# DecodeGenetics/BamQC

Hardware: AMD Instinct MI355X
Metric: BAM records/sec (and GB/s vs HBM roofline), 150 bp PE, 1/2/4/8 MI355X (higher is better)
Workload: dtype u8/u32/u64 integer

## Files before the change

### bamqc_amd/csrc/bqc_api.cpp

```cpp
#include <hip/hip_runtime.h>

#include <algorithm>
#include <climits>
#include <cmath>
#include <cstdarg>
#include <cstdio>
#include <cstdlib>
#include <cstring>
#include <string>
#include <chrono>
#include <condition_variable>
#include <mutex>
#include <thread>
#include <vector>

#include "bqc_ctx.h"
#include "../host/parallel.h"

extern "C" {
void bqc_launch_cov_final(const StateLayout&, uint64_t*, const uint32_t* carry, const uint32_t* parity, const uint8_t* started, const uint8_t* sel, uint32_t count_start, hipStream_t);
void bqc_launch_ref_nibbles(const uint8_t* dna5, uint64_t len, uint32_t* out, uint64_t n_dwords, hipStream_t);
uint32_t bqc_long_slots_cap(uint32_t max_read_len, uint32_t n_cu);
hipError_t bqc_long_init();
hipError_t bqc_short_init();
}

static thread_local char g_create_err[512];

int bqc_fail(bqc_ctx* c, int code, const char* fmt, ...)
{
    char buf[512];
    va_list ap;
    va_start(ap, fmt);
    vsnprintf(buf, sizeof buf, fmt, ap);
    va_end(ap);
    if (c) c->err = buf;
    else snprintf(g_create_err, sizeof g_create_err, "%s", buf);
    return code;
}
#define fail bqc_fail

extern "C" int bqc_abi_version(void) { return BQC_ABI_VERSION; }
extern "C" const char* bqc_last_error(const bqc_ctx* c) { return c ? c->err.c_str() : g_create_err; }

static int upload_ref_tables(bqc_ctx* c)
{
    HIPCHK(c, hipMemcpyAsync(c->d_ref_ptrs, c->d_ref.data(), sizeof(uint8_t*) * c->d_ref.size(), hipMemcpyHostToDevice, c->stream));
    HIPCHK(c, hipMemcpyAsync(c->d_ref_len, c->ref_len.data(), sizeof(uint64_t) * c->ref_len.size(), hipMemcpyHostToDevice, c->stream));
    HIPCHK(c, hipMemcpyAsync(c->d_refn_ptrs, c->d_refn.data(), sizeof(uint32_t*) * c->d_refn.size(), hipMemcpyHostToDevice, c->stream));
    HIPCHK(c, hipStreamSynchronize(c->stream));
    return 0;
}

static int reset_stream_records(bqc_ctx* c)
{
    ErrRec e{};
    e.first_key = BQC_ERRKEY_NONE;
    const int32_t cur[2] = {-1, -1};
    HIPCHK(c, hipMemcpyAsync(c->d_err0, &e, sizeof e, hipMemcpyHostToDevice, c->stream));
    HIPCHK(c, hipMemcpyAsync(c->d_cursor, cur, 8, hipMemcpyHostToDevice, c->stream));
    HIPCHK(c, hipStreamSynchronize(c->stream));
    return 0;
}

extern "C" int bqc_create(const bqc_options* opt, bqc_ctx** out)
{
    if (!opt || !out) return fail(nullptr, BQC_ERR_ARG, "bqc_create: null argument");
    if (opt->struct_size != sizeof(bqc_options)) return fail(nullptr, BQC_ERR_ARG, "bqc_create: struct_size mismatch");
    if (opt->n_lanes == 0 || opt->n_lanes > 256) return fail(nullptr, BQC_ERR_ARG, "bqc_create: n_lanes must be 1..256");
    if (opt->isize < 0) return fail(nullptr, BQC_ERR_ARG, "bqc_create: negative insert size");
    if (opt->max_read_len == 0 || opt->hist_cap == 0) return fail(nullptr, BQC_ERR_ARG, "bqc_create: zero capacity");
    if (opt->n_refs && !opt->main_chrom) return fail(nullptr, BQC_ERR_ARG, "bqc_create: main_chrom missing");
    int ndev = 0;
    if (hipGetDeviceCount(&ndev) != hipSuccess || ndev <= 0)
        return fail(nullptr, BQC_ERR_DEVICE, "bqc_create: no HIP device available (this library has no CPU fallback)");
    if (opt->device < 0 || opt->device >= ndev) return fail(nullptr, BQC_ERR_DEVICE, "bqc_create: device %d out of range", opt->device);
    bqc_ctx* c = new bqc_ctx();
    c->opt = *opt;
    c->device = opt->device;
    uint32_t nr = opt->n_refs ? opt->n_refs : 1;
    c->main_chrom.assign(nr, 0);
    if (opt->n_refs) memcpy(c->main_chrom.data(), opt->main_chrom, opt->n_refs);
    if (opt->fasta_index) c->fasta_index.assign(opt->fasta_index, opt->fasta_index + opt->n_refs);
    c->opt.main_chrom = c->main_chrom.data();
    c->opt.fasta_index = c->fasta_index.empty() ? nullptr : c->fasta_index.data();
    c->sl = make_state_layout(opt->n_lanes, opt->max_read_len, opt->hist_cap, (uint32_t)opt->isize + 1);
    c->cov.assign(opt->n_lanes, LaneCov());
    c->shard.tail = opt->shard_tail != 0;
    c->shard.pending.assign(opt->n_lanes, c->shard.tail ? 1 : 0);
    c->shard.has_prev.assign(opt->n_lanes, 0);
    c->shard.prev_rid.assign(opt->n_lanes, 0);
    c->shard.prev_bp.assign(opt->n_lanes, 0);
    c->d_ref.assign(nr, nullptr);
    c->d_refn.assign(nr, nullptr);
    c->ref_len.assign(nr, 0);
    const char* v = getenv("BQC_NO_FAST");
    c->no_fast = v && v[0] == '1';
#define CCHK(call)                                                                                            \
    do {                                                                                                      \
        hipError_t e_ = (call);                                                                               \
        if (e_ != hipSuccess) {                                                                               \
            fail(nullptr, BQC_ERR_DEVICE, "bqc_create: %s failed: %s", #call, hipGetErrorString(e_));         \
            bqc_destroy(c);                                                                                   \
            return BQC_ERR_DEVICE;                                                                            \
        }                                                                                                     \
    } while (0)
    const bool ctiming = getenv("BQC_TIMING") && getenv("BQC_TIMING")[0] == '1';
    const auto ct0 = std::chrono::steady_clock::now();
    double cts[10] = {0, 0, 0, 0, 0, 0, 0, 0, 0, 0};
    auto cstamp = [&](int k) { cts[k] = std::chrono::duration<double>(std::chrono::steady_clock::now() - ct0).count() * 1e3; };
    CCHK(hipSetDevice(c->device));
    hipDeviceProp_t prop;
    CCHK(hipGetDeviceProperties(&prop, c->device));
    c->n_cu = prop.multiProcessorCount > 0 ? (uint32_t)prop.multiProcessorCount : 256;
    cstamp(0);
    c->stream = bqc_pool_stream(c->device, 0);
    if (!c->stream) { fail(nullptr, BQC_ERR_DEVICE, "bqc_create: hipStreamCreate failed"); bqc_destroy(c); return BQC_ERR_DEVICE; }
    cstamp(1);
    CCHK(hipMalloc(&c->d_state, c->sl.words * 8));
    CCHK(hipMalloc(&c->d_err0, sizeof(ErrRec)));
    CCHK(hipMalloc(&c->d_cursor, 8));
    cstamp(6);
    if (!c->fasta_index.empty()) {
        CCHK(hipMalloc(&c->d_fasta_index, 4 * c->fasta_index.size()));
        CCHK(hipMemcpy(c->d_fasta_index, c->fasta_index.data(), 4 * c->fasta_index.size(), hipMemcpyHostToDevice));
    }
    cstamp(7);
    c->kl_slots_cap = bqc_long_slots_cap(opt->max_read_len, c->n_cu);
    c->t8_slots_cap = std::max(std::max(1024u, 4u * c->n_cu), c->kl_slots_cap);
    CCHK(hipMalloc(&c->d_t8rows, (size_t)c->t8_slots_cap * BQC_T8_SPW * 65536));
    CCHK(hipMalloc(&c->d_t8used, (size_t)c->t8_slots_cap * BQC_T8_USED * 4));
    cstamp(8);
    CCHK(hipMalloc(&c->d_kl_cyc, (size_t)c->kl_slots_cap * 2 * 6 * 1024 * 4));
    CCHK(hipMalloc(&c->d_kl_cyc_used, (size_t)c->kl_slots_cap * 4));
    CCHK(hipMalloc(&c->d_carry, (size_t)opt->n_lanes * 2 * 2000 * 4));
    CCHK(hipMalloc(&c->d_parity, ((size_t)opt->n_lanes + 1) * 4));
    CCHK(hipMalloc(&c->d_started, opt->n_lanes));
    CCHK(hipMalloc(&c->d_ref_ptrs, sizeof(uint8_t*) * nr));
    CCHK(hipMalloc(&c->d_ref_len, sizeof(uint64_t) * nr));
    CCHK(hipMalloc(&c->d_refn_ptrs, sizeof(uint32_t*) * nr));
    CCHK(hipMalloc(&c->d_main, nr));
    cstamp(9);
    CCHK(hipMemcpy(c->d_main, c->main_chrom.data(), nr, hipMemcpyHostToDevice));
    cstamp(2);
    CCHK(hipMemsetAsync(c->d_state, 0, c->sl.words * 8, c->stream));
    if (reset_stream_records(c)) { snprintf(g_create_err, sizeof g_create_err, "%s", c->err.c_str()); bqc_destroy(c); return BQC_ERR_DEVICE; }
    CCHK(hipMemsetAsync(c->d_carry, 0, (size_t)opt->n_lanes * 2 * 2000 * 4, c->stream));
    CCHK(hipMemsetAsync(c->d_parity, 0, ((size_t)opt->n_lanes + 1) * 4, c->stream));
    CCHK(hipMemsetAsync(c->d_started, 0, opt->n_lanes, c->stream));
    CCHK(hipStreamSynchronize(c->stream));
    if (upload_ref_tables(c)) { snprintf(g_create_err, sizeof g_create_err, "%s", c->err.c_str()); bqc_destroy(c); return BQC_ERR_DEVICE; }
    cstamp(3);
    if (opt->sketch.n_k && opt->sketch.n_q) {
        std::string e;
        c->sketch = sketch_create(opt->sketch, opt->n_lanes, c->stream, e);
        if (!c->sketch) { fail(nullptr, BQC_ERR_ARG, "bqc_create: sketch: %s", e.c_str()); bqc_destroy(c); return BQC_ERR_ARG; }
    }
    cstamp(4);
    for (int i = 0; i < 16; ++i) {
        hipEvent_t e;
        CCHK(hipEventCreate(&e));
        c->ev.push_back(e);
    }
    cstamp(5);
    if (ctiming) fprintf(stderr, "[timing] bqc_create: kernel attributes (code object load) at %.1f ms, compute stream %.1f, allocations %.1f (first three %.1f, FASTA index copied %.1f, 8-mer rows %.1f, the rest %.1f, then a copy), memsets + tables %.1f, sketch %.1f, events %.1f\n", cts[0], cts[1], cts[2], cts[6], cts[7], cts[8], cts[9], cts[3], cts[4], cts[5]);
    *out = c;
    return 0;
}

namespace {
struct StreamPool {
    std::mutex m;
    std::condition_variable cv;
    static const int kAhead = 4;
    hipStream_t made[kAhead] = {nullptr, nullptr, nullptr, nullptr};
    bool taken[kAhead] = {false, false, false, false};
    int device = -1;
    int n_made = 0;
    bool making = false;
};
StreamPool g_streams;
}
hipStream_t bqc_pool_stream(int device, int rank)
{
    {
        std::unique_lock<std::mutex> lk(g_streams.m);
        if (g_streams.device == device && rank >= 0 && rank < StreamPool::kAhead) {
            g_streams.cv.wait(lk, [&] { return g_streams.n_made > rank || !g_streams.making; });
            if (g_streams.n_made > rank && !g_streams.taken[rank]) { g_streams.taken[rank] = true; return g_streams.made[rank]; }
        }
    }
    hipStream_t s = nullptr;
    if (hipStreamCreateWithFlags(&s, hipStreamNonBlocking) != hipSuccess) { (void)hipGetLastError(); return nullptr; }
    return s;
}

extern "C" int bqc_warmup(int32_t device)
{
    {
        std::lock_guard<std::mutex> lk(g_streams.m);
        if (g_streams.device != -1) return g_streams.device == device ? 0 : BQC_ERR_ARG;
        g_streams.device = device;
        g_streams.making = true;
    }
    auto done = [](int rc) { { std::lock_guard<std::mutex> lk(g_streams.m); g_streams.making = false; } g_streams.cv.notify_all(); return rc; };
    if (hipSetDevice(device) != hipSuccess || hipFree(nullptr) != hipSuccess) return done(BQC_ERR_DEVICE);
    for (int k = 0; k < StreamPool::kAhead; ++k) {
        hipStream_t s = nullptr;
        if (hipStreamCreateWithFlags(&s, hipStreamNonBlocking) != hipSuccess) { (void)hipGetLastError(); return done(BQC_ERR_DEVICE); }
        { std::lock_guard<std::mutex> lk(g_streams.m); g_streams.made[k] = s; g_streams.n_made = k + 1; }
        g_streams.cv.notify_all();
    }
    return done(0);
}

extern "C" int bqc_set_fasta_index(bqc_ctx* c, const int32_t* idx)
{
    if (!c || !idx) return BQC_ERR_ARG;
    if (c->upload_counter) return bqc_fail(c, BQC_ERR_STATE, "bqc_set_fasta_index after the first batch");
    HIPCHK(c, hipSetDevice(c->device));
    const size_t n = c->opt.n_refs ? c->opt.n_refs : 1;
    c->fasta_index.assign(n, -1);
    for (uint32_t r = 0; r < c->opt.n_refs; ++r) c->fasta_index[r] = idx[r];
    c->opt.fasta_index = c->fasta_index.data();
    if (!c->d_fasta_index) HIPCHK(c, hipMalloc(&c->d_fasta_index, 4 * n));
    HIPCHK(c, hipMemcpy(c->d_fasta_index, c->fasta_index.data(), 4 * n, hipMemcpyHostToDevice));
    return 0;
}

extern "C" void bqc_destroy(bqc_ctx* c)
{
    if (!c) return;
    (void)hipSetDevice(c->device);
    if (c->copy_stream) (void)hipStreamSynchronize(c->copy_stream);
    if (c->stream) (void)hipStreamSynchronize(c->stream);
    bqc_pipeline_destroy(c);
    bqc_anchor_destroy(c);
    auto in_arena = [&](const void* p) { return c->ref_arena && (const uint8_t*)p >= c->ref_arena && (const uint8_t*)p < c->ref_arena + c->ref_arena_cap; };
    for (auto p : c->d_ref) if (p && !in_arena(p)) (void)hipFree(p);
    for (auto p : c->d_refn) if (p && !in_arena(p)) (void)hipFree(p);
    if (c->ref_arena) (void)hipFree(c->ref_arena);

    (void)hipFree(c->d_refn_ptrs);
    if (c->sketch) sketch_destroy(c->sketch);
    (void)hipFree(c->d_state); (void)hipFree(c->d_err0); (void)hipFree(c->d_cursor); (void)hipFree(c->d_fasta_index); (void)hipFree(c->d_t8rows); (void)hipFree(c->d_t8used); (void)hipFree(c->d_kl_cyc); (void)hipFree(c->d_kl_cyc_used); (void)hipFree(c->d_carry); (void)hipFree(c->d_parity);
    (void)hipFree(c->d_started); (void)hipFree(c->d_ref_ptrs); (void)hipFree(c->d_ref_len); (void)hipFree(c->d_main);
    for (auto e : c->ev) (void)hipEventDestroy(e);
    if (c->stream) (void)hipStreamDestroy(c->stream);
    if (c->copy_stream) (void)hipStreamDestroy(c->copy_stream);
    delete c;
}

extern "C" int bqc_reserve_references(bqc_ctx* c, uint64_t total_bases, uint32_t n_contigs)
{
    if (!c) return BQC_ERR_ARG;
    if (c->ref_arena) return 0;
    HIPCHK(c, hipSetDevice(c->device));
    const size_t cap = (size_t)total_bases + (size_t)total_bases / 2 + (size_t)n_contigs * (8 * BQC_FAST_NH + 1024) + 4096;
    if (hipMalloc((void**)&c->ref_arena, cap) != hipSuccess) { (void)hipGetLastError(); c->ref_arena = nullptr; return 0; }
    c->ref_arena_cap = cap;
    c->ref_arena_used = 0;
    return 0;
}

extern "C" int bqc_set_reference(bqc_ctx* c, int32_t rid, const uint8_t* dna5, uint64_t len)
{
    if (!c || rid < 0 || (uint32_t)rid >= c->opt.n_refs || (!dna5 && len)) return fail(c, BQC_ERR_ARG, "bqc_set_reference: bad argument");
    HIPCHK(c, hipSetDevice(c->device));
    auto in_arena = [&](const void* p) { return c->ref_arena && (const uint8_t*)p >= c->ref_arena && (const uint8_t*)p < c->ref_arena + c->ref_arena_cap; };
    if (c->d_ref[rid]) { if (!in_arena(c->d_ref[rid])) HIPCHK(c, hipFree(c->d_ref[rid])); c->d_ref[rid] = nullptr; }
    if (c->d_refn[rid]) { if (!in_arena(c->d_refn[rid])) HIPCHK(c, hipFree(c->d_refn[rid])); c->d_refn[rid] = nullptr; }
    const uint64_t nd8 = (len + 7) / 8;
    const size_t b1 = ((len ? len : 1) + 255) & ~(size_t)255, b2 = ((nd8 + 2 * BQC_FAST_NH) * 4 + 255) & ~(size_t)255;
    uint8_t* p = nullptr;
    uint32_t* pn = nullptr;
    if (c->ref_arena && c->ref_arena_used + b1 + b2 <= c->ref_arena_cap) {
        p = c->ref_arena + c->ref_arena_used;
        pn = (uint32_t*)(p + b1);
        c->ref_arena_used += b1 + b2;
    } else {
        HIPCHK(c, hipMalloc(&p, len ? len : 1));
        HIPCHK(c, hipMalloc(&pn, (nd8 + 2 * BQC_FAST_NH) * 4));
    }
    HIPCHK(c, hipMemcpy(p, dna5, len, hipMemcpyHostToDevice));
    bqc_launch_ref_nibbles(p, len, pn, nd8, c->stream);
    HIPCHK(c, hipStreamSynchronize(c->stream));
    c->d_ref[rid] = p;
    c->d_refn[rid] = pn;
    c->ref_len[rid] = len;
    return upload_ref_tables(c);
}

static int sync_and_check(bqc_ctx* c)
{
    HIPCHK(c, hipSetDevice(c->device));
    if (c->poisoned) return bqc_fail(c, BQC_ERR_STATE, "context is in an error state: %s", c->err.c_str());
    int rc = bqc_drain(c);
    if (rc) return rc;
    ErrRec e;
    HIPCHK(c, hipMemcpyAsync(&e, c->d_err0, sizeof e, hipMemcpyDeviceToHost, c->stream));
    HIPCHK(c, hipStreamSynchronize(c->stream));
    rc = bqc_report_errors(c, e);
    if (rc) { c->poisoned = true; c->poison_code = rc; }
    return rc;
}

extern "C" int bqc_sync(bqc_ctx* c)
{
    if (!c) return BQC_ERR_ARG;
    return sync_and_check(c);
}

extern "C" int bqc_reset(bqc_ctx* c)
{
    if (!c) return BQC_ERR_ARG;
    HIPCHK(c, hipSetDevice(c->device));
    (void)bqc_drain(c);
    bqc_state_ready(c);
    HIPCHK(c, hipMemsetAsync(c->d_state, 0, c->sl.words * 8, c->stream));
    if (reset_stream_records(c)) return BQC_ERR_DEVICE;
    HIPCHK(c, hipMemsetAsync(c->d_carry, 0, (size_t)c->opt.n_lanes * 2 * 2000 * 4, c->stream));
    HIPCHK(c, hipMemsetAsync(c->d_parity, 0, ((size_t)c->opt.n_lanes + 1) * 4, c->stream));
    HIPCHK(c, hipMemsetAsync(c->d_started, 0, c->opt.n_lanes, c->stream));
    if (c->sketch) sketch_reset(c->sketch, c->stream);
    HIPCHK(c, hipStreamSynchronize(c->stream));
    c->cov.assign(c->opt.n_lanes, LaneCov());
    if (c->anchor.d_state) HIPCHK(c, bqc_anchor_fresh_state(c));
    c->anchor.mode = 0;
    c->state_seq = 0;
    c->flushed = false;
    c->poisoned = false;
    c->poison_code = 0;
    return 0;
}

extern "C" int bqc_set_timing(bqc_ctx* c, int enable)
{
    if (!c) return BQC_ERR_ARG;
    c->timing = enable != 0;
    return 0;
}

extern "C" int bqc_last_timing(bqc_ctx* c, uint32_t* n, const char* const** names, const float** ms)
{
    if (!c || !n || !names || !ms) return BQC_ERR_ARG;
    HIPCHK(c, hipStreamSynchronize(c->stream));
    c->tms.assign(c->n_timed, 0.f);
    for (int i = 0; i < c->n_timed; ++i) (void)hipEventElapsedTime(&c->tms[i], c->ev[i], c->ev[i + 1]);
    *n = (uint32_t)c->n_timed;
    *names = c->tnames.data();
    *ms = c->tms.data();
    return 0;
}

extern "C" int bqc_flush(bqc_ctx* c)
{
    if (!c) return BQC_ERR_ARG;
    if (c->poisoned) return fail(c, BQC_ERR_STATE, "context is in an error state: %s", c->err.c_str());
    if (c->flushed) return 0;
    HIPCHK(c, hipSetDevice(c->device));
    int rc = sync_and_check(c);
    if (rc) return rc;
    bqc_state_ready(c);
    bqc_launch_cov_final(c->sl, c->d_state, c->d_carry, c->d_parity, c->d_started, nullptr, 1, c->stream);
    HIPCHK(c, hipGetLastError());
    HIPCHK(c, hipStreamSynchronize(c->stream));
    c->flushed = true;
    return 0;
}

extern "C" uint64_t bqc_state_words(const bqc_ctx* c) { return c ? c->sl.words + (c->sketch ? sketch_state_words(c->sketch) : 0) : 0; }

extern "C" int bqc_state_export(bqc_ctx* c, void* dst)
{
    if (!c || !dst) return BQC_ERR_ARG;
    int rc = bqc_flush(c);
    if (rc) return rc;
    bqc_state_ready(c);
    HIPCHK(c, hipMemcpyAsync(dst, c->d_state, c->sl.words * 8, hipMemcpyDeviceToDevice, c->stream));
    if (c->sketch) sketch_state_export(c->sketch, (uint64_t*)dst + c->sl.words, c->stream);
    HIPCHK(c, hipStreamSynchronize(c->stream));
    return 0;
}
extern "C" int bqc_state_import(bqc_ctx* c, const void* src)
{
    if (!c || !src) return BQC_ERR_ARG;
    HIPCHK(c, hipSetDevice(c->device));
    (void)bqc_drain(c);
    bqc_state_ready(c);
    HIPCHK(c, hipMemcpyAsync(c->d_state, src, c->sl.words * 8, hipMemcpyDeviceToDevice, c->stream));
    if (c->sketch) sketch_state_import(c->sketch, (const uint64_t*)src + c->sl.words, c->stream);
    HIPCHK(c, hipStreamSynchronize(c->stream));
    c->flushed = true;
    return 0;
}
extern "C" int bqc_state_export_host(bqc_ctx* c, uint64_t* dst)
{
    if (!c || !dst) return BQC_ERR_ARG;
    int rc = bqc_flush(c);
    if (rc) return rc;
    bqc_state_ready(c);
    HIPCHK(c, hipStreamSynchronize(c->stream));
    HIPCHK(c, hipMemcpy(dst, c->d_state, c->sl.words * 8, hipMemcpyDeviceToHost));
    if (c->sketch) {
        uint64_t* tmp = nullptr;
        const uint64_t w = sketch_state_words(c->sketch);
        HIPCHK(c, hipMalloc(&tmp, w * 8));
        sketch_state_export(c->sketch, tmp, c->stream);
        HIPCHK(c, hipStreamSynchronize(c->stream));
        HIPCHK(c, hipMemcpy(dst + c->sl.words, tmp, w * 8, hipMemcpyDeviceToHost));
        HIPCHK(c, hipFree(tmp));
    }
    return 0;
}
extern "C" int bqc_state_import_host(bqc_ctx* c, const uint64_t* src)
{
    if (!c || !src) return BQC_ERR_ARG;
    HIPCHK(c, hipSetDevice(c->device));
    (void)bqc_drain(c);
    bqc_state_ready(c);
    HIPCHK(c, hipStreamSynchronize(c->stream));
    HIPCHK(c, hipMemcpy(c->d_state, src, c->sl.words * 8, hipMemcpyHostToDevice));
    if (c->sketch) {
        uint64_t* tmp = nullptr;
        const uint64_t w = sketch_state_words(c->sketch);
        HIPCHK(c, hipMalloc(&tmp, w * 8));
        HIPCHK(c, hipMemcpy(tmp, src + c->sl.words, w * 8, hipMemcpyHostToDevice));
        sketch_state_import(c->sketch, tmp, c->stream);
        HIPCHK(c, hipStreamSynchronize(c->stream));
        HIPCHK(c, hipFree(tmp));
    }
    c->flushed = true;
    return 0;
}

static uint32_t last_nonzero_len(const uint64_t* p, uint32_t n)
{
    while (n > 0 && p[n - 1] == 0) --n;
    return n;
}

extern "C" int bqc_finalize(bqc_ctx* c, const bqc_counts** out)
{
    if (!c || !out) return BQC_ERR_ARG;
    int rc = bqc_flush(c);
    if (rc) return rc;
    const StateLayout& sl = c->sl;
    c->h_state.resize(sl.words);
    HIPCHK(c, hipMemcpy(c->h_state.data(), c->d_state, sl.words * 8, hipMemcpyDeviceToHost));
    c->arrays.clear();
    c->lanes.assign(sl.n_lanes, bqc_lane_counts{});
    c->sk_out.assign(sl.n_lanes, {});
    auto keep = [&](std::vector<uint64_t>&& v) -> const uint64_t* {
        c->arrays.push_back(std::move(v));
        return c->arrays.back().data();
    };
    auto u32copy = [&](const uint64_t* p, uint32_t n) {
        std::vector<uint64_t> v(n ? n : 1);
        for (uint32_t i = 0; i < n; ++i) v[i] = p[i] & 0xFFFFFFFFull;
        return v;
    };
    c->arrays.reserve(sl.n_lanes * 64);
    for (uint32_t l = 0; l < sl.n_lanes; ++l) {
        const uint64_t* S = c->h_state.data() + sl.lane_base(l);
        bqc_lane_counts& L = c->lanes[l];
        for (int i = 0; i < BQC_N_SCALARS; ++i)
            L.scalars[i] = i == BQC_S_TOTALBPS ? S[sl.o_scalars + i] : (S[sl.o_scalars + i] & 0xFFFFFFFFull);
        for (int i = 0; i <= BQC_COVSIZE; ++i) L.poscov[i] = S[sl.o_poscov + i];
        if (S[sl.o_covstart] == 0) L.poscov[0] += 2 * BQC_VSIZE;
        for (int i = 0; i <= BQC_COVSIZE; ++i) L.poscov[i] &= 0xFFFFFFFFull;
        L.eightmer = S + sl.o_eightmer;
        L.triplet = S + sl.o_triplet;
        for (uint32_t m = 0; m < 2; ++m) {
            const uint64_t* Mq = S + sl.o_mate[m];
            bqc_mate_counts& mc = L.mate[m];
            const uint32_t n_rl = last_nonzero_len(Mq + sl.m_readlen, sl.lcap + 1);
            const uint32_t ncyc = n_rl ? n_rl - 1 : 0;
            mc.n_cycles = ncyc;
            for (int j = 0; j < 5; ++j) mc.dnacount[j] = Mq + sl.m_dnacount + (uint64_t)j * sl.lcap;
            mc.qualcount = Mq + sl.m_qualcount;
            mc.qualcount_readnr = Mq[sl.m_readnr] & 0xFFFFFFFFull;
            {
                std::vector<uint64_t> v(ncyc ? ncyc : 1, 0);
                uint64_t run = 0;
                for (uint32_t j = sl.lcap + 1; j-- > 0;) {
                    if (j < ncyc) v[j] = run & 0xFFFFFFFFull;
                    run += Mq[sl.m_sc5hist + j];
                }
                mc.sc5 = keep(std::move(v));
            }
            {
                std::vector<uint64_t> v(ncyc ? ncyc : 1, 0);
                uint64_t run = 0;
                for (uint32_t j = 0; j < ncyc; ++j) { run += Mq[sl.m_sc3diff + j]; v[j] = run & 0xFFFFFFFFull; }
                mc.sc3 = keep(std::move(v));
            }
            mc.n_Ncount = n_rl; mc.Ncount = keep(u32copy(Mq + sl.m_ncount, n_rl));
            mc.n_GCcount = n_rl; mc.GCcount = Mq + sl.m_gccount;
            mc.n_averageQual = last_nonzero_len(Mq + sl.m_avgceil, 256);
            mc.averageQual = keep(u32copy(Mq + sl.m_avgqual, mc.n_averageQual));
            mc.n_insertSize = sl.icap; mc.insertSize = keep(u32copy(Mq + sl.m_insert, sl.icap));
            mc.n_mapQ = last_nonzero_len(Mq + sl.m_mapq, 256); mc.mapQ = keep(u32copy(Mq + sl.m_mapq, mc.n_mapQ));
            mc.n_readLength = n_rl; mc.readLength = keep(u32copy(Mq + sl.m_readlen, n_rl));
            mc.n_mismatch = last_nonzero_len(Mq + sl.m_mismatch, sl.hcap); mc.mismatch = keep(u32copy(Mq + sl.m_mismatch, mc.n_mismatch));
            mc.n_delhist = last_nonzero_len(Mq + sl.m_delhist, sl.hcap); mc.delhist = keep(u32copy(Mq + sl.m_delhist, mc.n_delhist));
            mc.n_inshist = last_nonzero_len(Mq + sl.m_inshist, sl.hcap); mc.inshist = keep(u32copy(Mq + sl.m_inshist, mc.n_inshist));
        }
        if (c->sketch) {
            std::string e;
            if (!sketch_finalize(c->sketch, l, c->sk_out[l], c->stream, e)) return fail(c, BQC_ERR_DEVICE, "sketch finalize: %s", e.c_str());
            L.n_sketch = (uint32_t)c->sk_out[l].size();
            L.sketch = c->sk_out[l].data();
        }
    }
    c->counts.n_lanes = sl.n_lanes;
    c->counts.lanes = c->lanes.data();
    *out = &c->counts;
    return 0;
}
```

### bamqc_amd/csrc/bqc_ctx.h

```cpp
#pragma once
#include <hip/hip_runtime.h>

#include <atomic>
#include <cstdarg>
#include <cstdio>
#include <deque>
#include <mutex>
#include <string>
#include <vector>

#include "../../include/bamqc.h"
#include "device_types.h"
#include "prep.h"
#include "anchor.h"
#include "sketch.h"
#include "../host/raw_vector.h"

struct LaneCov {
    bool first = true;
    int32_t id = 0;
    uint32_t shift = 0;
    uint64_t win = 0;
    uint64_t batch_base = 0;
};

struct HostPass {
    uint32_t n = 0;
    uint64_t seq_bytes = 0, qual_bytes = 0, cigar_words = 0;
    uint32_t n_slow = 0, max_len_slow = 0;
    uint32_t t8_lane = 0;
    bool multi_lane = false;
    raw_vector<CovEntry> cov;
    raw_vector<uint32_t> order;
    std::vector<SuperWindow> sws;
    std::vector<Stretch> stretches;
    std::vector<CovTile> tiles;
    std::vector<uint8_t> lane_mask, started_after;
    std::vector<uint64_t> add_idx, add_val;
    uint32_t n_pending = 0;
    std::vector<std::vector<uint32_t>> lane_first;
    std::vector<uint64_t> lane_count;
};

struct BatchMem {
    void* dmem = nullptr;
    size_t dcap = 0;
    DevBatch d{};
    PrepArgs prep{};
    uint8_t* d_lane_mask = nullptr;
    uint8_t* d_started_after = nullptr;
    uint64_t* d_add_idx = nullptr;
    uint64_t* d_add_val = nullptr;
    uint32_t n_add = 0;
    uint32_t* d_rsum = nullptr;
    uint32_t* d_order_tmp = nullptr;
    ErrRec* d_err = nullptr;
    uint64_t algo_bytes = 0;
    uint32_t n_slow = 0, max_len_slow = 0, n_chunks_slow_ub = 0, t8_lane = 0;
    uint64_t lane_bits[4] = {0, 0, 0, 0};
    bool processed = false;
    size_t h2d_begin = 0, h2d_end = 0;
    size_t o_col[13] = {0};
    size_t col_bytes[13] = {0};
    size_t o_xr = 0, o_xv = 0, o_cov_in = 0, o_order = 0, o_sws = 0, o_stretch = 0, o_tiles = 0, o_mask = 0, o_started = 0, o_aidx = 0, o_aval = 0;
};

struct PendBatch {
    std::vector<uint8_t> lane;
    std::vector<int32_t> rid;
    std::vector<uint32_t> bp;
    void* dmem = nullptr;
    uint32_t extra_cap = 0;
    uint32_t n() const { return (uint32_t)lane.size(); }
};
struct ShardCtx {
    bool tail = false, resolved = false, exported = false;
    std::vector<uint8_t> pending;
    std::vector<uint8_t> has_prev;
    std::vector<int32_t> prev_rid;
    std::vector<uint32_t> prev_bp;
    std::deque<PendBatch> batches;
};

struct bqc_dbatch {
    BatchMem m;
    std::vector<LaneCov> cov_after;
    uint64_t seq = 0;
};

struct Slot {
    BatchMem m;
    char* hmem = nullptr;
    size_t hcap = 0;
    ErrRec* h_err = nullptr;
    hipEvent_t ev_h2d = nullptr, ev_done = nullptr;
    bool busy = false;
    bool in_place = false;
    uint64_t ticket = 0;
};

struct bqc_anchored {
    AnchorSummary* h_sum = nullptr;
    AnchorLane* h_lanes = nullptr;
    uint32_t* h_bound = nullptr;
    std::vector<uint32_t> rest;
    std::vector<int32_t> pend_rid;
    std::vector<uint32_t> pend_bp;
    std::vector<uint8_t> pend_lane;
    const CovEntry* d_cov = nullptr;
    uint32_t n = 0;
    bool completed = false;
    bool released = false;
    static const uint32_t kInline = 1u << 17;
};
struct AnchorEngine {
    std::atomic<int> mode{0};
    AnchorState* d_state = nullptr;
    AnchorSummary* d_sum = nullptr;
    uint32_t* d_bound = nullptr;
    void* d_scratch = nullptr;
    const uint32_t* d_plog_bp = nullptr; const int32_t* d_plog_rid = nullptr; const uint8_t* d_plog_lane = nullptr;
    size_t cap_n = 0;
    std::mutex m;
    std::vector<bqc_anchored*> free_list, all;
    bqc_anchored* outstanding = nullptr;
    std::string err;
};

struct bqc_ctx {
    bqc_options opt{};
    std::vector<uint8_t> main_chrom;
    std::vector<int32_t> fasta_index;
    StateLayout sl{};
    int device = 0;
    hipStream_t stream = nullptr;
    hipStream_t copy_stream = nullptr;
    uint32_t n_cu = 256;
    uint64_t* d_state = nullptr;
    ErrRec* d_err0 = nullptr;
    int32_t* d_cursor = nullptr;
    int32_t* d_fasta_index = nullptr;
    uint32_t* d_t8rows = nullptr;
    uint32_t* d_t8used = nullptr;
    uint32_t* d_kl_cyc = nullptr;
    uint32_t* d_kl_cyc_used = nullptr;
    uint32_t kl_slots_cap = 0;
    uint32_t t8_slots_used = 0, t8_slots_cap = 0;
    uint64_t t8_lanes[4] = {0, 0, 0, 0};
    std::vector<std::pair<void*, size_t>> pool;
    uint32_t* d_carry = nullptr;
    uint32_t* d_parity = nullptr;
    uint8_t* d_started = nullptr;
    std::vector<uint8_t*> d_ref;
    uint8_t* ref_arena = nullptr;
    size_t ref_arena_cap = 0, ref_arena_used = 0;
    std::vector<uint32_t*> d_refn;
    std::vector<uint64_t> ref_len;
    uint8_t** d_ref_ptrs = nullptr;
    uint32_t** d_refn_ptrs = nullptr;
    bool no_fast = false;
    uint64_t* d_ref_len = nullptr;
    uint8_t* d_main = nullptr;
    std::vector<LaneCov> cov;
    bool flushed = false;
    bool poisoned = false;
    int poison_code = 0;
    uint64_t upload_counter = 0;
    uint64_t state_seq = 0;
    HostPass hp;
    ShardCtx shard;
    static const int kSlots = 3;
    Slot slots[kSlots];
    uint64_t next_ticket = 1;
    uint64_t checked_ticket = 0;
    AnchorEngine anchor;
    SketchDevice* sketch = nullptr;
    bool timing = false;
    std::vector<hipEvent_t> ev;
    std::vector<const char*> tnames;
    std::vector<float> tms;
    int n_timed = 0;
    std::vector<uint64_t> h_state;
    std::vector<std::vector<uint64_t>> arrays;
    std::vector<bqc_lane_counts> lanes;
    std::vector<std::vector<bqc_sketch_counts>> sk_out;
    bqc_counts counts{};
    std::string err;
};

int bqc_fail(bqc_ctx* c, int code, const char* fmt, ...);
#define HIPCHK(c, call)                                                                                         \
    do {                                                                                                        \
        hipError_t e_ = (call);                                                                                 \
        if (e_ != hipSuccess) return bqc_fail(c, BQC_ERR_DEVICE, "%s failed: %s", #call, hipGetErrorString(e_)); \
    } while (0)

hipStream_t bqc_pool_stream(int device, int rank);
int bqc_copy_stream(bqc_ctx* c);
int bqc_report_errors(bqc_ctx* c, const ErrRec& e);
int bqc_drain(bqc_ctx* c);
void bqc_pipeline_destroy(bqc_ctx* c);
hipError_t bqc_anchor_fresh_state(bqc_ctx* c);
void bqc_anchor_destroy(bqc_ctx* c);
void bqc_state_ready(bqc_ctx* c);
```

### bamqc_amd/csrc/bqc_pipeline.cpp

```cpp
#include "bqc_ctx.h"

#include <algorithm>
#include <chrono>
#include <climits>
#include <cstdlib>
#include <cstring>

#include "../host/parallel.h"

extern "C" {
void bqc_launch_reads_chunks(const DevBatch&, const StateLayout&, uint64_t*, const DevRefs&, uint32_t*, uint32_t grid, uint32_t fast_table, hipStream_t);
void bqc_launch_nm_extra(const DevBatch&, const StateLayout&, uint64_t*, const DevRefs&, uint32_t*, hipStream_t);
void bqc_launch_long(const DevBatch&, const StateLayout&, uint64_t*, const DevRefs&, uint32_t*, uint32_t*, uint32_t max_len_ub, uint32_t max_read_len, uint32_t, uint32_t, uint32_t* t8rows, uint32_t* t8_used, uint32_t t8_lane, uint32_t* cyc_tiles, uint32_t* cyc_used, uint32_t slot_cap, hipStream_t);
uint32_t bqc_long_slots(uint32_t max_len_ub, uint32_t max_read_len, uint32_t n_chunks_ub, uint32_t n_cu);
void bqc_launch_cov(const DevBatch&, const StateLayout&, uint64_t*, uint32_t* carry, uint32_t* parity, const uint8_t* lane_mask, uint8_t* started,
                    const uint8_t* started_after, uint32_t n_lanes, hipStream_t);
void bqc_launch_add_words(uint64_t* state, const uint64_t* idx, const uint64_t* val, uint32_t n, hipStream_t);
void bqc_launch_or_bytes(uint8_t* dst, const uint8_t* src, uint32_t n, hipStream_t);
void bqc_launch_short(const DevBatch&, const StateLayout&, uint64_t*, const DevRefs&, uint32_t*, uint32_t grid, uint32_t* t8rows, uint32_t* t8_used, hipStream_t);
uint32_t bqc_short_parts();
void bqc_launch_t8_fold(const uint32_t* t8rows, const uint32_t* t8_used, uint32_t n_slots, const StateLayout&, uint64_t* state, uint32_t lane, hipStream_t);
void bqc_launch_err_merge(ErrRec* dst, const ErrRec* src, hipStream_t);
void bqc_launch_cov_final(const StateLayout&, uint64_t*, const uint32_t* carry, const uint32_t* parity, const uint8_t* started, const uint8_t* sel, uint32_t count_start, hipStream_t);
}

using clk = std::chrono::steady_clock;
static double secs_since(clk::time_point a) { return std::chrono::duration<double>(clk::now() - a).count(); }
static int timing_level()
{
    static const int lv = [] { const char* e = getenv("BQC_TIMING"); return e ? atoi(e) : 0; }();
    return lv;
}

int bqc_copy_stream(bqc_ctx* c)
{
    if (c->copy_stream) return 0;
    c->copy_stream = bqc_pool_stream(c->device, 3);
    return c->copy_stream ? 0 : bqc_fail(c, BQC_ERR_DEVICE, "hipStreamCreate failed");
}

void bqc_state_ready(bqc_ctx* c)
{
    if (!c->t8_slots_used) return;
    for (uint32_t l = 0; l < c->opt.n_lanes; ++l)
        if (c->t8_lanes[l >> 6] >> (l & 63u) & 1ull) bqc_launch_t8_fold(c->d_t8rows, c->d_t8used, c->t8_slots_used, c->sl, c->d_state, l, c->stream);
    c->t8_lanes[0] = c->t8_lanes[1] = c->t8_lanes[2] = c->t8_lanes[3] = 0;
    c->t8_slots_used = 0;
}

namespace {
struct CovPlanner {
    bqc_ctx* c;
    HostPass& H;
    uint32_t n, nl;
    std::vector<uint8_t> started_before;
    std::vector<uint32_t> last_rel;
    CovPlanner(bqc_ctx* c_, HostPass& H_, uint32_t n_) : c(c_), H(H_), n(n_), nl(c_->opt.n_lanes), started_before(nl), last_rel(nl, 0)
    {
        H.lane_mask.assign(nl, 0);
        H.lane_first.resize(nl);
        for (uint32_t l = 0; l < nl; ++l) {
            started_before[l] = !c->cov[l].first;
            c->cov[l].batch_base = c->cov[l].win;
            H.lane_first[l].clear();
        }
    }
    void step(uint32_t i, uint32_t lane, int32_t rid, uint32_t beginpos, uint64_t& rel, uint32_t& pos)
    {
        LaneCov& s = c->cov[lane];
        pos = an_step(s.first, s.id, s.shift, s.win, rid, beginpos);
        rel = s.win - s.batch_base;
        if (rel > 0xFFFFFFF0ull) return;
        std::vector<uint32_t>& first = H.lane_first[lane];
        if (first.size() <= rel) first.resize((size_t)rel + 1, i);
        last_rel[lane] = (uint32_t)rel;
    }
    void finish()
    {
        H.tiles.clear(); H.add_idx.clear(); H.add_val.clear();
        for (uint32_t l = 0; l < nl; ++l) {
            const std::vector<uint32_t>& first = H.lane_first[l];
            if (first.empty()) continue;
            H.lane_mask[l] = 1;
            const uint32_t W1 = last_rel[l];
            auto first_at = [&](uint64_t k) { return k < first.size() ? first[k] : n; };
            uint32_t last_tile = 0xFFFFFFFFu;
            uint64_t covered_final = 0;
            auto push_tile = [&](uint32_t w) {
                const uint32_t t = w / BQC_COV_TILE_WINDOWS;
                if (last_tile != 0xFFFFFFFFu && t <= last_tile) return;
                last_tile = t;
                const uint32_t wlo = t * BQC_COV_TILE_WINDOWS;
                CovTile ct{};
                ct.lane = l; ct.win_lo = wlo; ct.win_final = W1; ct.mixed = H.multi_lane ? 1u : 0u;
                ct.list_begin = first_at(wlo == 0 ? 0 : wlo - 1);
                ct.list_end = first_at((uint64_t)wlo + BQC_COV_TILE_WINDOWS);
                H.tiles.push_back(ct);
                const uint64_t hi = std::min<uint64_t>((uint64_t)wlo + BQC_COV_TILE_WINDOWS, W1);
                if (hi > wlo) covered_final += hi - wlo;
            };
            if (started_before[l]) { push_tile(0); push_tile(1); }
            for (uint64_t w = 0; w < first.size(); ++w) {
                const bool present = w + 1 == first.size() || first[w] != first[w + 1];
                if (present) { push_tile((uint32_t)w); push_tile((uint32_t)w + 1); }
            }
            if (W1 > covered_final) {
                H.add_idx.push_back(c->sl.lane_base(l) + c->sl.o_poscov + 0);
                H.add_val.push_back((uint64_t)(W1 - covered_final) * BQC_VSIZE);
            }
            c->cov[l].batch_base = c->cov[l].win;
        }
        H.started_after.resize(nl);
        for (uint32_t l = 0; l < nl; ++l) H.started_after[l] = !c->cov[l].first;
    }
};
}

static uint64_t plan_read_groups(HostPass& H, uint32_t n, uint32_t nl)
{
    uint32_t lanes_present = 0;
    H.t8_lane = 0;
    for (uint32_t l = 0; l < nl; ++l) {
        if (H.lane_count[l]) ++lanes_present;
        if (H.lane_count[l] > H.lane_count[H.t8_lane]) H.t8_lane = l;
    }
    uint64_t in_lanes = 0;
    for (uint32_t l = 0; l < nl; ++l) in_lanes += H.lane_count[l];
    const uint64_t n_bad = n - in_lanes;
    H.multi_lane = lanes_present > 1 || (n_bad > 0 && in_lanes > 0);
    H.stretches.clear(); H.sws.clear();
    auto add_stretch = [&](uint32_t lane, uint32_t begin, uint32_t count) {
        if (!count) return;
        Stretch S{lane, (uint32_t)H.sws.size(), 0, 0};
        for (uint32_t p = 0; p < count; p += BQC_SW_READS)
            H.sws.push_back(SuperWindow{lane, begin + p, std::min<uint32_t>(BQC_SW_READS, count - p), (uint32_t)H.stretches.size()});
        S.sw_end = (uint32_t)H.sws.size();
        H.stretches.push_back(S);
    };
    if (!H.multi_lane) {
        uint32_t lane = 0;
        for (uint32_t l = 0; l < nl; ++l) if (H.lane_count[l]) lane = l;
        add_stretch(lane, 0, n);
    } else {
        uint64_t at = n_bad;
        for (uint32_t l = 0; l < nl; ++l) { add_stretch(l, (uint32_t)(l == 0 ? 0 : at), (uint32_t)(H.lane_count[l] + (l == 0 ? n_bad : 0))); at += H.lane_count[l]; }
    }
    return n_bad;
}

static int host_pass(bqc_ctx* c, const bqc_batch* b, HostPass& H)
{
    const uint32_t n = b->n_reads, nl = c->opt.n_lanes;
    H.n = n;
    const unsigned nt_max = std::min(16u, bqc_host_threads());
    struct Part { uint64_t s1 = 0, s2 = 0, s3 = 0; uint32_t n_slow = 0, max_slow = 0; std::vector<uint64_t> lanes; };
    std::vector<Part> part(nt_max);
    const unsigned nt = parallel_ranges(n, nt_max, 1 << 17, [&](unsigned t, size_t lo, size_t hi) {
        Part& P = part[t];
        P.lanes.assign(nl, 0);
        uint64_t s1 = 0, s2 = 0, s3 = 0;
        uint32_t ns = 0, ms = 0;
        for (size_t i = lo; i < hi; ++i) {
            const uint32_t L = b->l_seq[i], lane = b->lane[i];
            s1 += (L + 1) / 2; s2 += L; s3 += b->n_cigar[i];
            if (lane < nl) P.lanes[lane]++;
            if (c->no_fast || L > BQC_FAST_MAXLEN) { ++ns; ms = std::max(ms, L); }
        }
        P.s1 = s1; P.s2 = s2; P.s3 = s3; P.n_slow = ns; P.max_slow = ms;
    });
    H.seq_bytes = H.qual_bytes = H.cigar_words = 0;
    H.n_slow = H.max_len_slow = 0;
    H.lane_count.assign(nl, 0);
    for (unsigned t = 0; t < nt; ++t) {
        H.seq_bytes += part[t].s1; H.qual_bytes += part[t].s2; H.cigar_words += part[t].s3;
        H.n_slow += part[t].n_slow; H.max_len_slow = std::max(H.max_len_slow, part[t].max_slow);
        for (uint32_t l = 0; l < nl; ++l) H.lane_count[l] += part[t].lanes[l];
    }
    const uint64_t n_bad = plan_read_groups(H, n, nl);
    if (H.multi_lane) {
        std::vector<uint64_t> w(nl);
        uint64_t at = n_bad, w_bad = 0;
        for (uint32_t l = 0; l < nl; ++l) { w[l] = at; at += H.lane_count[l]; }
        { const size_t cap = H.order.capacity(); H.order.resize(n); if (H.order.capacity() != cap) advise_huge(H.order); }
        for (uint32_t i = 0; i < n; ++i) {
            const uint32_t lane = b->lane[i];
            if (lane < nl) H.order[w[lane]++] = i; else H.order[w_bad++] = i;
        }
    } else H.order.clear();
    { const size_t cap = H.cov.capacity(); H.cov.resize(n); if (H.cov.capacity() != cap) advise_huge(H.cov); }
    CovPlanner plan(c, H, n);
    ShardCtx& sh = c->shard;
    const bool set_aside = sh.tail && !sh.resolved;
    PendBatch* pb = nullptr;
    H.n_pending = 0;
    const uint32_t n_refs = c->opt.n_refs;
    const uint8_t* main_chrom = c->main_chrom.data();
    if (!set_aside) {
        const uint16_t* const flags = b->flag;
        const uint8_t* const lanes = b->lane;
        const int32_t* const rids = b->rid;
        const int32_t* const poss = b->pos;
        CovEntry* const out = H.cov.data();
        LaneCov* const cov = c->cov.data();
        std::vector<uint32_t>* const lane_first = H.lane_first.data();
        uint32_t* const last_rel = plan.last_rel.data();
        LaneCov local = cov[0];
        const bool one = nl == 1;
        bool too_many = false;
        for (uint32_t i = 0; i < n; ++i) {
            const uint32_t flag = flags[i], lane = lanes[i];
            const int32_t rid = rids[i];
            if (!an_is_candidate(flag, rid, n_refs, main_chrom, lane, nl)) { out[i] = CovEntry{BQC_COV_NONE, 0}; continue; }
            LaneCov& st = one ? local : cov[lane];
            const uint32_t pos = an_step(st.first, st.id, st.shift, st.win, rid, (uint32_t)poss[i]);
            const uint64_t rel = st.win - st.batch_base;
            if (rel > 0xFFFFFFF0ull) { too_many = true; break; }
            std::vector<uint32_t>& first = lane_first[lane];
            if (first.size() <= rel) first.resize((size_t)rel + 1, i);
            last_rel[lane] = (uint32_t)rel;
            out[i] = CovEntry{(uint32_t)rel, pos};
        }
        if (one) cov[0] = local;
        if (too_many) return bqc_fail(c, BQC_ERR_ARG, "batch spans too many coverage windows (split the batch)");
    } else
    for (uint32_t i = 0; i < n; ++i) {
        const uint32_t flag = b->flag[i], lane = b->lane[i];
        const int32_t rid = b->rid[i];
        if (!an_is_candidate(flag, rid, n_refs, main_chrom, lane, nl)) { H.cov[i] = CovEntry{BQC_COV_NONE, 0}; continue; }
        const uint32_t beginpos = (uint32_t)b->pos[i];
        if (set_aside && sh.pending[lane]) {
            const uint32_t d = beginpos - sh.prev_bp[lane];
            const bool certain = sh.has_prev[lane] && (rid != sh.prev_rid[lane] || (d > 2u * BQC_VSIZE && d <= 0xFFFFFFFFu - 2u * BQC_VSIZE));
            sh.has_prev[lane] = 1; sh.prev_rid[lane] = rid; sh.prev_bp[lane] = beginpos;
            if (!certain) {
                if (!pb) { sh.batches.emplace_back(); pb = &sh.batches.back(); }
                H.cov[i] = CovEntry{BQC_COV_PENDING, pb->n()};
                pb->lane.push_back((uint8_t)lane); pb->rid.push_back(rid); pb->bp.push_back(beginpos);
                continue;
            }
            sh.pending[lane] = 0;
        }
        uint64_t rel;
        uint32_t pos;
        plan.step(i, lane, rid, beginpos, rel, pos);
        if (rel > 0xFFFFFFF0ull) return bqc_fail(c, BQC_ERR_ARG, "batch spans too many coverage windows (split the batch)");
        H.cov[i] = CovEntry{(uint32_t)rel, pos};
    }
    H.n_pending = pb ? pb->n() : 0;
    plan.finish();
    for (uint32_t e = 0; e < b->n_nm_extra; ++e)
        if (b->nm_extra_read[e] >= n) return bqc_fail(c, BQC_ERR_ARG, "nm_extra_read out of range");
    return 0;
}

extern "C" void bqc_anchor_rule(uint32_t n, const uint16_t* flag, const int32_t* rid, const int32_t* pos, const uint8_t* lane, uint32_t n_refs,
                                const uint8_t* main_chrom, uint32_t n_lanes, AnchorState* states, uint64_t* win, uint32_t* off)
{
    for (uint32_t i = 0; i < n; ++i) {
        win[i] = ~0ull; off[i] = 0;
        if (!an_is_candidate(flag[i], rid[i], n_refs, main_chrom, lane[i], n_lanes)) continue;
        AnchorState& s = states[lane[i]];
        bool first = s.first != 0;
        off[i] = an_step(first, s.id, s.shift, s.win, rid[i], (uint32_t)pos[i]);
        s.first = first;
        win[i] = s.win;
    }
}

static int first_from_table(bqc_ctx* c, const bqc_anchored* a, size_t off, size_t total, std::vector<uint32_t>& first)
{
    if (off + total > bqc_anchored::kInline + a->rest.size()) return bqc_fail(c, BQC_ERR_DEVICE, "internal error: the anchors' window table is shorter than the last window");
    first.assign(total, AN_NO_READ);
    uint32_t cur = AN_NO_READ;
    for (size_t k = total; k-- > 0;) {
        const size_t at = off + k;
        const uint32_t v = at < bqc_anchored::kInline ? a->h_bound[at] : a->rest[at - bqc_anchored::kInline];
        if (v != AN_NO_READ) cur = v;
        first[k] = cur;
    }
    if (first[total - 1] == AN_NO_READ) return bqc_fail(c, BQC_ERR_DEVICE, "internal error: the anchors' window table does not end at the last window");
    return 0;
}

static bool lane_anchored(const AnchorLane* AL, uint32_t l) { return AL[l].n_cand > AL[l].n_pending; }
static void load_state(LaneCov& lc, const AnchorState& s) { lc.first = s.first != 0; lc.id = s.id; lc.shift = s.shift; lc.win = s.win; }

static int host_pass_anchored(bqc_ctx* c, uint32_t n, const bqc_anchored* a, HostPass& H)
{
    const AnchorSummary& S = *a->h_sum;
    const AnchorLane* AL = a->h_lanes;
    const uint32_t nl = c->opt.n_lanes;
    H.n = n;
    H.seq_bytes = S.seq_bytes; H.qual_bytes = S.qual_bytes; H.cigar_words = S.cigar_words;
    H.n_slow = S.n_slow; H.max_len_slow = S.max_len_slow;
    H.lane_count.assign(nl, 0);
    for (uint32_t l = 0; l < nl; ++l) H.lane_count[l] = AL[l].n_reads;
    if (plan_read_groups(H, n, nl) != S.n_bad) return bqc_fail(c, BQC_ERR_DEVICE, "internal error: the anchors' read counts do not add up");
    H.order.clear();
    H.n_pending = 0;
    if (S.n_pending) {
        ShardCtx& sh = c->shard;
        sh.batches.emplace_back();
        PendBatch& pb = sh.batches.back();
        if (nl > 1) pb.lane = a->pend_lane; else pb.lane.assign(S.n_pending, 0);
        pb.rid = a->pend_rid;
        pb.bp = a->pend_bp;
        H.n_pending = S.n_pending;
    }
    if (c->shard.tail)
        for (uint32_t l = 0; l < nl; ++l) {
            const AnchorState& A = AL[l].after;
            c->shard.pending[l] = A.pending ? 1 : 0; c->shard.has_prev[l] = A.has_prev ? 1 : 0; c->shard.prev_rid[l] = A.prev_rid; c->shard.prev_bp[l] = A.prev_bp;
        }
    for (uint32_t l = 0; l < nl; ++l) load_state(c->cov[l], AL[l].before);
    CovPlanner plan(c, H, n);
    for (uint32_t l = 0; l < nl; ++l) {
        if (!lane_anchored(AL, l)) continue;
        const int rc = first_from_table(c, a, AL[l].first_off, (size_t)AL[l].last_rel + 1, H.lane_first[l]);
        if (rc) return rc;
        plan.last_rel[l] = AL[l].last_rel;
    }
    for (uint32_t l = 0; l < nl; ++l) load_state(c->cov[l], AL[l].after);
    plan.finish();
    return 0;
}

namespace {
struct Carver {
    size_t off = 0;
    size_t take(size_t bytes) { size_t o = off; off += (bytes + 255) & ~(size_t)255; return o; }
};
}

static int layout_batch(bqc_ctx* c, BatchMem& m, const bqc_batch* b, const HostPass& H, bool from_pool, const CovEntry* in_place = nullptr, bool order_on_device = false)
{
    const uint64_t n = H.n;
    const uint32_t nl = c->opt.n_lanes;
    Carver cv;
    cv.take(256);
    m.h2d_begin = cv.off;
    const size_t cb[13] = {2 * n, n, n, 4 * n, 4 * n, 4 * n, 4 * n, 4 * n, 4 * n, 2 * n, H.seq_bytes, H.qual_bytes, 4 * H.cigar_words};
    for (int k = 0; k < 13; ++k) { m.col_bytes[k] = in_place ? 0 : cb[k]; m.o_col[k] = cv.take(in_place ? 0 : cb[k] + (k >= 10 ? 512 : 0)); }
    m.o_xr = cv.take(4ull * b->n_nm_extra); m.o_xv = cv.take(4ull * b->n_nm_extra);
    m.o_cov_in = cv.take(in_place ? 0 : sizeof(CovEntry) * n);
    m.o_order = cv.take(H.multi_lane ? 4 * n : 0);
    m.o_sws = cv.take(sizeof(SuperWindow) * H.sws.size());
    m.o_stretch = cv.take(sizeof(Stretch) * H.stretches.size());
    m.o_tiles = cv.take(sizeof(CovTile) * H.tiles.size());
    m.o_mask = cv.take(nl); m.o_started = cv.take(nl);
    m.o_aidx = cv.take(8 * H.add_idx.size()); m.o_aval = cv.take(8 * H.add_val.size());
    m.h2d_end = cv.off;
    const uint64_t nblk = (n + 1023) / 1024, n_sw = H.sws.size(), n_st = H.stretches.size();
    const uint64_t perm_cap = 3 * n + H.cigar_words + 128 * (n_sw + n_st + 1);
    const uint64_t cf_cap = (2 * n + 128 * n_sw) / 256 + H.cigar_words / 256 + 4 * n_st + 16;
    const uint64_t cs_cap = H.n_slow / BQC_CHUNK_READS + n_st + 4;
    const uint64_t cx_cap = H.cigar_words / 2 + 1;
    if (perm_cap > 0xFFFFFFF0ull) return bqc_fail(c, BQC_ERR_ARG, "batch too large (split the batch)");
    const size_t o_flag2 = cv.take(2 * n), o_soff = cv.take(4 * n), o_qoff = cv.take(4 * n), o_cgoff = cv.take(4 * n), o_cov = cv.take(sizeof(CovEntry) * n),
                 o_covx = cv.take(sizeof(CovExtra) * cx_cap), o_cls = cv.take(2 * n), o_segs = cv.take(sizeof(TripSeg) * (H.cigar_words + 1)),
                 o_perm = cv.take(4 * perm_cap), o_cf = cv.take(sizeof(Chunk) * cf_cap), o_cs = cv.take(sizeof(Chunk) * cs_cap),
                 o_desc = cv.take(sizeof(BatchDesc)), o_err = cv.take(sizeof(ErrRec)), o_cursave = cv.take(8), o_bsz = cv.take(24 * nblk), o_btgt = cv.take(8 * nblk),
                 o_bmf = cv.take(8 * nblk), o_swc = cv.take(sizeof(SwCounts) * n_sw), o_swp = cv.take(sizeof(SwPlan) * n_sw),
                 o_rsum = cv.take(H.n_slow ? 12 * n : 0), o_otmp = cv.take(order_on_device && H.multi_lane ? 4 * lane_order_tmp_words((uint32_t)n, nl) : 0);
    const size_t need = cv.off + 256;
    if (m.dcap < need) {
        if (m.dmem) { (void)hipFree(m.dmem); m.dmem = nullptr; m.dcap = 0; }
        if (from_pool)
            for (size_t k = 0; k < c->pool.size(); ++k)
                if (c->pool[k].second >= need && c->pool[k].second <= 2 * need + (64u << 20)) {
                    m.dmem = c->pool[k].first; m.dcap = c->pool[k].second;
                    c->pool.erase(c->pool.begin() + k);
                    break;
                }
        if (!m.dmem) {
            const size_t cap = need + need / 8;
            const hipError_t he = hipMalloc(&m.dmem, cap);
            if (he != hipSuccess) { m.dmem = nullptr; return bqc_fail(c, BQC_ERR_DEVICE, "hipMalloc(%zu) failed: %s", cap, hipGetErrorString(he)); }
            m.dcap = cap;
        }
    }
    char* base = (char*)m.dmem;
    DevBatch& d = m.d;
    d = DevBatch{};
    d.n_reads = (uint32_t)n;
    d.flag = (const uint16_t*)(base + o_flag2);
    d.mapq = (const uint8_t*)(base + m.o_col[1]); d.lane = (const uint8_t*)(base + m.o_col[2]);
    d.rid = (const int32_t*)(base + m.o_col[3]); d.pos = (const int32_t*)(base + m.o_col[4]); d.tlen = (const int32_t*)(base + m.o_col[5]);
    d.nm = (const int32_t*)(base + m.o_col[6]); d.as_ = (const int32_t*)(base + m.o_col[7]); d.l_seq = (const uint32_t*)(base + m.o_col[8]);
    d.n_cigar = (const uint16_t*)(base + m.o_col[9]);
    d.seq = (const uint8_t*)(base + m.o_col[10]); d.qual = (const uint8_t*)(base + m.o_col[11]); d.cigar = (const uint32_t*)(base + m.o_col[12]);
    d.seq_off = (const uint32_t*)(base + o_soff); d.qual_off = (const uint32_t*)(base + o_qoff); d.cigar_off = (const uint32_t*)(base + o_cgoff);
    d.order = H.multi_lane ? (const uint32_t*)(base + m.o_order) : nullptr;
    d.perm = (const uint32_t*)(base + o_perm);
    d.chunks = (const Chunk*)(base + o_cs); d.chunks_fast = (const Chunk*)(base + o_cf);
    d.desc = (const BatchDesc*)(base + o_desc);
    d.nm_extra_read = (const uint32_t*)(base + m.o_xr); d.nm_extra_val = (const int32_t*)(base + m.o_xv); d.n_nm_extra = b->n_nm_extra;
    d.cov = (const CovEntry*)(base + o_cov); d.cov_extra = (const CovExtra*)(base + o_covx);
    d.cov_tiles = (const CovTile*)(base + m.o_tiles); d.n_cov_tiles = (uint32_t)H.tiles.size();
    d.segs = (const TripSeg*)(base + o_segs);
    PrepArgs& p = m.prep;
    p = PrepArgs{};
    p.n = (uint32_t)n; p.n_lanes = nl; p.max_read_len = c->opt.max_read_len; p.no_fast = c->no_fast ? 1u : 0u; p.replay = 0;
    p.flag_in = (const uint16_t*)(base + m.o_col[0]); p.mapq = d.mapq; p.lane = d.lane; p.rid = d.rid; p.pos = d.pos; p.as_ = d.as_;
    p.l_seq = d.l_seq; p.n_cigar = d.n_cigar; p.qual = d.qual; p.cigar = d.cigar;
    p.cov_in = (const CovEntry*)(base + m.o_cov_in); p.order = d.order;
    p.sws = (const SuperWindow*)(base + m.o_sws); p.n_sw = (uint32_t)n_sw;
    p.stretches = (const Stretch*)(base + m.o_stretch); p.n_stretch = (uint32_t)n_st;
    p.fasta_index = c->d_fasta_index;
    p.flag_out = (uint16_t*)(base + o_flag2); p.seq_off = (uint32_t*)(base + o_soff); p.qual_off = (uint32_t*)(base + o_qoff);
    p.cigar_off = (uint32_t*)(base + o_cgoff); p.cov_out = (CovEntry*)(base + o_cov); p.cov_extra = (CovExtra*)(base + o_covx);
    p.cov_extra_cap = (uint32_t)std::min<uint64_t>(cx_cap, 0xFFFFFFFFull); p.cls = (uint16_t*)(base + o_cls); p.segs = (TripSeg*)(base + o_segs);
    p.perm = (uint32_t*)(base + o_perm); p.perm_cap = (uint32_t)perm_cap;
    p.chunks_fast = (Chunk*)(base + o_cf); p.chunks_fast_cap = (uint32_t)cf_cap;
    p.chunks_slow = (Chunk*)(base + o_cs); p.chunks_slow_cap = (uint32_t)cs_cap;
    p.desc = (BatchDesc*)(base + o_desc); p.err = (ErrRec*)(base + o_err);
    p.cursor = c->d_cursor; p.cursor_save = (int32_t*)(base + o_cursave);
    p.blk_sizes = (unsigned long long*)(base + o_bsz); p.blk_tgt = (uint32_t*)(base + o_btgt); p.blk_maxfast = (uint32_t*)(base + o_bmf);
    p.sw_counts = (SwCounts*)(base + o_swc); p.sw_plan = (SwPlan*)(base + o_swp);
    m.d_lane_mask = (uint8_t*)(base + m.o_mask); m.d_started_after = (uint8_t*)(base + m.o_started);
    m.d_add_idx = (uint64_t*)(base + m.o_aidx); m.d_add_val = (uint64_t*)(base + m.o_aval); m.n_add = (uint32_t)H.add_idx.size();
    m.d_rsum = H.n_slow ? (uint32_t*)(base + o_rsum) : nullptr;
    m.d_order_tmp = order_on_device && H.multi_lane ? (uint32_t*)(base + o_otmp) : nullptr;
    m.d_err = p.err;
    m.algo_bytes = 48ull * n + H.seq_bytes + H.qual_bytes + 4 * H.cigar_words;
    m.n_slow = H.n_slow; m.max_len_slow = H.max_len_slow; m.n_chunks_slow_ub = (uint32_t)cs_cap; m.t8_lane = H.t8_lane;
    m.lane_bits[0] = m.lane_bits[1] = m.lane_bits[2] = m.lane_bits[3] = 0;
    for (size_t l = 0; l < H.lane_count.size() && l < 256; ++l) if (H.lane_count[l]) m.lane_bits[l >> 6] |= 1ull << (l & 63);
    if (in_place) {
        d.mapq = b->mapq; d.lane = b->lane; d.rid = b->rid; d.pos = b->pos; d.tlen = b->tlen; d.nm = b->nm; d.as_ = b->as; d.l_seq = b->l_seq; d.n_cigar = b->n_cigar;
        d.seq = b->seq; d.qual = b->qual; d.cigar = b->cigar;
        p.flag_in = b->flag; p.mapq = d.mapq; p.lane = d.lane; p.rid = d.rid; p.pos = d.pos; p.as_ = d.as_; p.l_seq = d.l_seq; p.n_cigar = d.n_cigar; p.qual = d.qual; p.cigar = d.cigar;
        p.cov_in = in_place;
    }
    m.processed = false;
    return 0;
}

static void fill_tables(const BatchMem& m, const bqc_batch* b, const HostPass& H, char* img, size_t img_begin , bool anchors_on_device = false)
{
    auto at = [&](size_t off) { return img + (off - img_begin); };
    if (b->n_nm_extra) { memcpy(at(m.o_xr), b->nm_extra_read, 4ull * b->n_nm_extra); memcpy(at(m.o_xv), b->nm_extra_val, 4ull * b->n_nm_extra); }
    if (!anchors_on_device) memcpy(at(m.o_cov_in), H.cov.data(), sizeof(CovEntry) * (size_t)H.n);
    if (H.multi_lane && !anchors_on_device) memcpy(at(m.o_order), H.order.data(), 4ull * H.n);
    memcpy(at(m.o_sws), H.sws.data(), sizeof(SuperWindow) * H.sws.size());
    memcpy(at(m.o_stretch), H.stretches.data(), sizeof(Stretch) * H.stretches.size());
    if (!H.tiles.empty()) memcpy(at(m.o_tiles), H.tiles.data(), sizeof(CovTile) * H.tiles.size());
    memcpy(at(m.o_mask), H.lane_mask.data(), H.lane_mask.size());
    memcpy(at(m.o_started), H.started_after.data(), H.started_after.size());
    if (!H.add_idx.empty()) { memcpy(at(m.o_aidx), H.add_idx.data(), 8 * H.add_idx.size()); memcpy(at(m.o_aval), H.add_val.data(), 8 * H.add_val.size()); }
}

static const void* column_ptr(const bqc_batch* b, int k)
{
    switch (k) {
    case 0: return b->flag; case 1: return b->mapq; case 2: return b->lane; case 3: return b->rid; case 4: return b->pos; case 5: return b->tlen;
    case 6: return b->nm; case 7: return b->as; case 8: return b->l_seq; case 9: return b->n_cigar; case 10: return b->seq; case 11: return b->qual;
    default: return b->cigar;
    }
}

static void tick(bqc_ctx* c, const char* name)
{
    if (!c->timing || c->n_timed + 1 >= (int)c->ev.size()) return;
    (void)hipEventRecord(c->ev[c->n_timed + 1], c->stream);
    c->tnames.push_back(name);
    c->n_timed++;
}

static int enqueue_kernels(bqc_ctx* c, BatchMem& m)
{
    DevRefs refs{(const uint8_t* const*)c->d_ref_ptrs, c->d_ref_len, c->d_main, c->opt.n_refs, (const uint32_t* const*)c->d_refn_ptrs};
    uint32_t* err = &m.d_err->flags;
    const DevBatch& d = m.d;
    if (d.n_reads == 0) { if (c->timing) { c->n_timed = 0; c->tnames.clear(); } return 0; }
    if (c->timing) { c->n_timed = 0; c->tnames.clear(); (void)hipEventRecord(c->ev[0], c->stream); }
    m.prep.replay = m.processed ? 1u : 0u;
    bqc_launch_prep(m.prep, refs, c->stream);
    m.processed = true;
    tick(c, "k_prep");
    if (!d.n_cov_tiles) bqc_launch_or_bytes(c->d_started, m.d_started_after, c->opt.n_lanes, c->stream);
    if (d.n_reads > m.n_slow) {
        const uint32_t grid = c->n_cu;
        if (!(bqc_short_parts() & 8u)) {
            bqc_launch_reads_chunks(d, c->sl, c->d_state, refs, err, c->n_cu * 8, 1, c->stream);
            tick(c, "k_reads");
        }
        if (c->t8_slots_used + grid > c->t8_slots_cap) bqc_state_ready(c);
        for (int k = 0; k < 4; ++k) c->t8_lanes[k] |= m.lane_bits[k];
        bqc_launch_short(d, c->sl, c->d_state, refs, err, grid, c->d_t8rows + (size_t)c->t8_slots_used * BQC_T8_SPW * 16384u,
                         c->d_t8used + (size_t)c->t8_slots_used * BQC_T8_USED, c->stream);
        c->t8_slots_used += grid;
        tick(c, "k_short");
    }
    if (m.n_slow) {
        bqc_launch_reads_chunks(d, c->sl, c->d_state, refs, err, std::min(m.n_chunks_slow_ub, c->n_cu * 8), 0, c->stream);
        tick(c, "k_reads(generic)");
        HIPCHK(c, hipMemsetAsync(m.d_rsum, 0, 12ull * d.n_reads, c->stream));
        const uint32_t slots = bqc_long_slots(m.max_len_slow, c->opt.max_read_len, m.n_chunks_slow_ub, c->n_cu);
        if (slots > c->kl_slots_cap || slots > c->t8_slots_cap)
            return bqc_fail(c, BQC_ERR_DEVICE, "internal error: k_long needs %u scratch slots, the context has %u / %u", slots, c->kl_slots_cap, c->t8_slots_cap);
        if (c->t8_slots_used + slots > c->t8_slots_cap) bqc_state_ready(c);
        for (int k = 0; k < 4; ++k) c->t8_lanes[k] |= m.lane_bits[k];
        bqc_launch_long(d, c->sl, c->d_state, refs, err, m.d_rsum, m.max_len_slow, c->opt.max_read_len, m.n_chunks_slow_ub, c->n_cu,
                        c->d_t8rows + (size_t)c->t8_slots_used * BQC_T8_SPW * 16384u, c->d_t8used + (size_t)c->t8_slots_used * BQC_T8_USED, m.t8_lane, c->d_kl_cyc,
                        c->d_kl_cyc_used, std::min(c->kl_slots_cap, c->t8_slots_cap - c->t8_slots_used), c->stream);
        c->t8_slots_used += slots;
        tick(c, "k_long");
    }
    if (d.n_nm_extra) bqc_launch_nm_extra(d, c->sl, c->d_state, refs, err, c->stream);
    if (d.n_cov_tiles) bqc_launch_cov(d, c->sl, c->d_state, c->d_carry, c->d_parity, m.d_lane_mask, c->d_started, m.d_started_after, c->opt.n_lanes, c->stream);
    bqc_launch_add_words(c->d_state, m.d_add_idx, m.d_add_val, m.n_add, c->stream);
    tick(c, "k_cov");
    if (c->sketch) { sketch_process(c->sketch, d, c->stream); tick(c, "k_sketch"); }
    bqc_launch_err_merge(c->d_err0, m.d_err, c->stream);
    HIPCHK(c, hipGetLastError());
    return 0;
}

int bqc_report_errors(bqc_ctx* c, const ErrRec& e)
{
    if (e.first_key != BQC_ERRKEY_NONE) {
        const uint32_t i = (uint32_t)(e.first_key >> 3), order = (uint32_t)(e.first_key & 7u);
        switch (order) {
        case 1: return bqc_fail(c, BQC_ERR_RANGE, "read %u is %u bases long; max_read_len is %u", i, e.aux0, c->opt.max_read_len);
        case 2: return bqc_fail(c, BQC_ERR_ARG, "read %u: lane %u out of range", i, e.aux0);
        case 3: return bqc_fail(c, BQC_ERR_ARG, "batch too large: payload offsets exceed 32 bits (split the batch)");
        case 4: return bqc_fail(c, BQC_ERR_AS_TAG, "ERROR: read %u has no usable AS tag.", i);
        case 5: return bqc_fail(c, BQC_ERR_FASTA, "ERROR: Could not read fasta record for reference id %d (read %u)", (int32_t)e.aux0, i);
        default: return bqc_fail(c, BQC_ERR_NO_MATE_FLAG, "ERROR: No first or second flag in read %u", i);
        }
    }
    if (!e.flags) return 0;
    if (e.flags & BQC_DEVERR_INTERNAL) return bqc_fail(c, BQC_ERR_DEVICE, "internal error: kernel layout assumption violated");
    if (e.flags & BQC_DEVERR_MATE) return bqc_fail(c, BQC_ERR_NO_MATE_FLAG, "ERROR: No first or second flag in read");
    if (e.flags & BQC_DEVERR_RANGE) return bqc_fail(c, BQC_ERR_RANGE, "mismatch/deletion/insertion count exceeds hist_cap (or NM < D+I)");
    return bqc_fail(c, BQC_ERR_RANGE, "base quality above 222 cannot be represented by the reference (q+33 wraps)");
}
static int poison(bqc_ctx* c, int code) { c->poisoned = true; c->poison_code = code; return code; }

extern "C" void bqc_dbatch_free(bqc_ctx* c, bqc_dbatch* db)
{
    if (!db) return;
    if (c) { (void)hipSetDevice(c->device); (void)hipStreamSynchronize(c->stream); }
    if (c && db->m.dmem && c->pool.size() < 3) c->pool.emplace_back(db->m.dmem, db->m.dcap);
    else (void)hipFree(db->m.dmem);
    delete db;
}
extern "C" uint64_t bqc_dbatch_bytes(const bqc_dbatch* db) { return db ? db->m.algo_bytes : 0; }

static int check_batch_args(bqc_ctx* c, const bqc_batch* b, const char* who)
{
    if (!c || !b) return bqc_fail(c, BQC_ERR_ARG, "%s: null argument", who);
    if (c->poisoned) return bqc_fail(c, BQC_ERR_STATE, "context is in an error state: %s", c->err.c_str());
    if (c->flushed) return bqc_fail(c, BQC_ERR_STATE, "%s after bqc_flush/bqc_finalize (call bqc_reset first)", who);
    if (b->n_reads && (!b->flag || !b->mapq || !b->lane || !b->rid || !b->pos || !b->tlen || !b->nm || !b->as || !b->l_seq || !b->n_cigar))
        return bqc_fail(c, BQC_ERR_ARG, "%s: null column", who);
    if (b->n_nm_extra && (!b->nm_extra_read || !b->nm_extra_val)) return bqc_fail(c, BQC_ERR_ARG, "%s: null nm_extra column", who);
    return 0;
}

extern "C" int bqc_upload(bqc_ctx* c, const bqc_batch* b, bqc_dbatch** out)
{
    if (!out) return bqc_fail(c, BQC_ERR_ARG, "bqc_upload: null argument");
    int rc = check_batch_args(c, b, "bqc_upload");
    if (rc) return rc;
    if (c->shard.tail && !c->shard.resolved) return bqc_fail(c, BQC_ERR_STATE, "bqc_upload: resident batches are not available to a shard_tail context (use bqc_submit)");
    HIPCHK(c, hipSetDevice(c->device));
    c->anchor.mode = 2;
    const auto t0 = clk::now();
    HostPass& H = c->hp;
    if ((rc = host_pass(c, b, H))) return poison(c, rc);
    const double t_pass = secs_since(t0);
    bqc_dbatch* db = new bqc_dbatch();
    if ((rc = layout_batch(c, db->m, b, H, true))) { delete db; return poison(c, rc); }
    BatchMem& m = db->m;
    char* base = (char*)m.dmem;
    std::vector<char> img(m.h2d_end - m.o_xr);
    fill_tables(m, b, H, img.data(), m.o_xr);
    hipError_t he = hipSuccess;
    for (int k = 0; k < 13 && he == hipSuccess; ++k)
        if (m.col_bytes[k]) he = hipMemcpyAsync(base + m.o_col[k], column_ptr(b, k), m.col_bytes[k], hipMemcpyHostToDevice, c->stream);
    if (he == hipSuccess) he = hipMemcpyAsync(base + m.o_xr, img.data(), img.size(), hipMemcpyHostToDevice, c->stream);
    if (he == hipSuccess) he = hipStreamSynchronize(c->stream);
    if (he != hipSuccess) { bqc_dbatch_free(c, db); poison(c, BQC_ERR_DEVICE); return bqc_fail(c, BQC_ERR_DEVICE, "upload failed: %s", hipGetErrorString(he)); }
    if (timing_level() == 2)
        fprintf(stderr, "[timing] upload of %u reads: host pass %.4f s, H2D %.4f s (%.1f MB)\n", b->n_reads, t_pass, secs_since(t0) - t_pass, (m.h2d_end - m.h2d_begin) / 1e6);
    db->cov_after = c->cov;
    db->seq = ++c->upload_counter;
    c->state_seq = db->seq;
    *out = db;
    return 0;
}

extern "C" int bqc_process(bqc_ctx* c, bqc_dbatch* db)
{
    if (!c || !db) return bqc_fail(c, BQC_ERR_ARG, "bqc_process: null argument");
    if (c->poisoned) return bqc_fail(c, BQC_ERR_STATE, "context is in an error state: %s", c->err.c_str());
    if (c->flushed) return bqc_fail(c, BQC_ERR_STATE, "bqc_process after bqc_flush (call bqc_reset first)");
    HIPCHK(c, hipSetDevice(c->device));
    if (db->seq > c->state_seq) {
        c->cov = db->cov_after;
        c->state_seq = db->seq;
    }
    return enqueue_kernels(c, db->m);
}

static int retire_slot(bqc_ctx* c, Slot& s)
{
    if (!s.busy) return 0;
    HIPCHK(c, hipEventSynchronize(s.ev_done));
    s.busy = false;
    if (s.ticket > c->checked_ticket) c->checked_ticket = s.ticket;
    const int rc = bqc_report_errors(c, *s.h_err);
    return rc ? poison(c, rc) : 0;
}

int bqc_drain(bqc_ctx* c)
{
    int first = 0;
    for (uint64_t t = c->checked_ticket + 1; t < c->next_ticket; ++t) {
        Slot& s = c->slots[t % bqc_ctx::kSlots];
        if (!s.busy || s.ticket != t) continue;
        if (first) { (void)hipEventSynchronize(s.ev_done); s.busy = false; continue; }
        const int rc = retire_slot(c, s);
        if (rc) first = rc;
    }
    if (c->next_ticket) c->checked_ticket = c->next_ticket - 1;
    return first;
}

void bqc_pipeline_destroy(bqc_ctx* c)
{
    for (Slot& s : c->slots) {
        if (s.busy && s.ev_done) (void)hipEventSynchronize(s.ev_done);
        if (s.m.dmem) (void)hipFree(s.m.dmem);
        if (s.hmem) (void)hipHostFree(s.hmem);
        if (s.h_err) (void)hipHostFree(s.h_err);
        if (s.ev_h2d) (void)hipEventDestroy(s.ev_h2d);
        if (s.ev_done) (void)hipEventDestroy(s.ev_done);
        s = Slot();
    }
    for (auto& pb : c->pool) (void)hipFree(pb.first);
    c->pool.clear();
    for (PendBatch& pb : c->shard.batches) if (pb.dmem) (void)hipFree(pb.dmem);
    c->shard.batches.clear();
}

static int submit_impl(bqc_ctx* c, const bqc_batch* b, bool pinned_columns, uint64_t* ticket_out, const bqc_anchored* anchored = nullptr)
{
    int rc = check_batch_args(c, b, "bqc_submit");
    if (rc) return rc;
    HIPCHK(c, hipSetDevice(c->device));
    if (ticket_out) *ticket_out = 0;
    if (!anchored) c->anchor.mode = 2;
    if (b->n_reads == 0) return 0;
    if ((rc = bqc_copy_stream(c))) return rc;
    const uint64_t ticket = c->next_ticket;
    Slot& s = c->slots[ticket % bqc_ctx::kSlots];
    const auto t0 = clk::now();
    if ((rc = retire_slot(c, s))) return rc;
    const double t_wait = secs_since(t0);
    if (!s.ev_done) {
        HIPCHK(c, hipEventCreateWithFlags(&s.ev_h2d, hipEventDisableTiming));
        HIPCHK(c, hipEventCreateWithFlags(&s.ev_done, hipEventDisableTiming));
        HIPCHK(c, hipHostMalloc((void**)&s.h_err, sizeof(ErrRec), hipHostMallocDefault));
    }
    HostPass& H = c->hp;
    if ((rc = anchored ? host_pass_anchored(c, b->n_reads, anchored, H) : host_pass(c, b, H))) return poison(c, rc);
    const double t_pass = secs_since(t0) - t_wait;
    static const bool copy_anyway = getenv("BQC_ANCHORED_COPY") && getenv("BQC_ANCHORED_COPY")[0] == '1';
    const bool in_place = anchored && !copy_anyway;
    if ((rc = layout_batch(c, s.m, b, H, false, in_place ? anchored->d_cov : nullptr, anchored != nullptr))) return poison(c, rc);
    s.in_place = in_place;
    BatchMem& m = s.m;
    if (H.n_pending) {
        PendBatch& pb = c->shard.batches.back();
        pb.extra_cap = (uint32_t)std::min<uint64_t>(H.cigar_words / 2 + 1, 0xFFFFFFF0ull);
        const size_t bytes = sizeof(PendRun) * (size_t)pb.n() + 256 + sizeof(PendExtra) * (size_t)pb.extra_cap;
        const hipError_t he = hipMalloc(&pb.dmem, bytes);
        if (he != hipSuccess) { poison(c, BQC_ERR_DEVICE); return bqc_fail(c, BQC_ERR_DEVICE, "hipMalloc(%zu) failed: %s", bytes, hipGetErrorString(he)); }
        m.prep.pend = (PendRun*)pb.dmem;
        m.prep.pend_extra_n = (uint32_t*)((char*)pb.dmem + sizeof(PendRun) * (size_t)pb.n());
        m.prep.pend_extra = (PendExtra*)((char*)m.prep.pend_extra_n + 256);
        m.prep.pend_extra_cap = pb.extra_cap;
    }
    const size_t img_begin = pinned_columns ? m.o_xr : m.h2d_begin, img_bytes = m.h2d_end - img_begin;
    if (s.hcap < img_bytes) {
        if (s.hmem) (void)hipHostFree(s.hmem);
        s.hmem = nullptr; s.hcap = 0;
        const size_t cap = img_bytes + img_bytes / 8 + 4096;
        const hipError_t he = hipHostMalloc((void**)&s.hmem, cap, hipHostMallocDefault);
        if (he != hipSuccess) { poison(c, BQC_ERR_DEVICE); return bqc_fail(c, BQC_ERR_DEVICE, "hipHostMalloc(%zu) failed: %s", cap, hipGetErrorString(he)); }
        s.hcap = cap;
    }
    fill_tables(m, b, H, s.hmem, img_begin, anchored != nullptr);
    char* base = (char*)m.dmem;
    hipError_t he = hipSuccess;
    if (pinned_columns) {
        for (int k = 0; k < 13 && he == hipSuccess; ++k)
            if (m.col_bytes[k]) he = hipMemcpyAsync(base + m.o_col[k], column_ptr(b, k), m.col_bytes[k], hipMemcpyDefault, c->copy_stream);
    } else {
        struct Piece { char* dst; const char* src; size_t n; };
        Piece pc[13];
        size_t total = 0;
        for (int k = 0; k < 13; ++k) { pc[k] = Piece{s.hmem + (m.o_col[k] - m.h2d_begin), (const char*)column_ptr(b, k), m.col_bytes[k]}; total += m.col_bytes[k]; }
        parallel_ranges(total, std::min(8u, bqc_host_threads()), 16u << 20, [&](unsigned, size_t lo, size_t hi) {
            size_t at = 0;
            for (int k = 0; k < 13; ++k) {
                const size_t a = std::max(lo, at), z = std::min(hi, at + pc[k].n);
                if (a < z) memcpy(pc[k].dst + (a - at), pc[k].src + (a - at), z - a);
                at += pc[k].n;
            }
        });
    }
    if (anchored && !in_place) {
        const size_t n_cov = sizeof(CovEntry) * (size_t)b->n_reads, o_behind = m.o_cov_in + ((n_cov + 255) & ~(size_t)255);
        if (he == hipSuccess && m.o_cov_in > img_begin) he = hipMemcpyAsync(base + img_begin, s.hmem, m.o_cov_in - img_begin, hipMemcpyHostToDevice, c->copy_stream);
        if (he == hipSuccess && n_cov) he = hipMemcpyAsync(base + m.o_cov_in, anchored->d_cov, n_cov, hipMemcpyDeviceToDevice, c->copy_stream);
        if (he == hipSuccess && m.h2d_end > o_behind) he = hipMemcpyAsync(base + o_behind, s.hmem + (o_behind - img_begin), m.h2d_end - o_behind, hipMemcpyHostToDevice, c->copy_stream);
    } else
    if (he == hipSuccess) he = hipMemcpyAsync(base + img_begin, s.hmem, img_bytes, hipMemcpyHostToDevice, c->copy_stream);
    if (he == hipSuccess) he = hipEventRecord(s.ev_h2d, c->copy_stream);
    if (he == hipSuccess) he = hipStreamWaitEvent(c->stream, s.ev_h2d, 0);
    if (he != hipSuccess) { poison(c, BQC_ERR_DEVICE); return bqc_fail(c, BQC_ERR_DEVICE, "upload failed: %s", hipGetErrorString(he)); }
    if (m.d_order_tmp) bqc_launch_lane_order(m.d.lane, b->n_reads, c->opt.n_lanes, (uint32_t*)((char*)m.dmem + m.o_order), m.d_order_tmp, c->stream);
    if ((rc = enqueue_kernels(c, m))) return poison(c, rc);
    HIPCHK(c, hipMemcpyAsync(s.h_err, m.d_err, sizeof(ErrRec), hipMemcpyDeviceToHost, c->stream));
    HIPCHK(c, hipEventRecord(s.ev_done, c->stream));
    s.busy = true;
    s.ticket = ticket;
    c->next_ticket = ticket + 1;
    c->state_seq = ++c->upload_counter;
    if (ticket_out) *ticket_out = ticket;
    if (timing_level() == 2)
        fprintf(stderr, "[timing] submit of %u reads: waited %.4f s for the slot, host pass %.4f s, staging + enqueue %.4f s (%.1f MB to the device)\n", b->n_reads, t_wait,
                t_pass, secs_since(t0) - t_wait - t_pass, (m.h2d_end - m.h2d_begin) / 1e6);
    return 0;
}

static bool lives_on_device(const void* p)
{
    if (!p) return false;
    hipPointerAttribute_t a;
    if (hipPointerGetAttributes(&a, p) != hipSuccess) { (void)hipGetLastError(); return false; }
    return a.type == hipMemoryTypeDevice;
}
extern "C" int bqc_submit(bqc_ctx* c, const bqc_batch* b)
{
    if (c && b && b->n_reads && (lives_on_device(b->seq) || lives_on_device(b->qual) || lives_on_device(b->cigar)))
        return bqc_fail(c, BQC_ERR_ARG, "bqc_submit: payload columns in device memory need bqc_submit_async");
    return submit_impl(c, b, false, nullptr);
}
extern "C" int bqc_submit_async(bqc_ctx* c, const bqc_batch* b, uint64_t* ticket) { return submit_impl(c, b, true, ticket); }

static int anchor_fail(bqc_ctx* c, const char* what) { c->anchor.err = what; return -BQC_ERR_DEVICE; }
static void anchor_release_locked(AnchorEngine& E, bqc_anchored* a)
{
    if (E.outstanding == a) E.outstanding = nullptr;
    if (a->released) return;
    a->released = true;
    E.free_list.push_back(a);
}
static void anchor_release(AnchorEngine& E, bqc_anchored* a) { std::lock_guard<std::mutex> lk(E.m); anchor_release_locked(E, a); }
extern "C" const char* bqc_anchor_error(const bqc_ctx* c) { return c ? c->anchor.err.c_str() : ""; }

hipError_t bqc_anchor_fresh_state(bqc_ctx* c)
{
    AnchorState s0{};
    s0.first = 1;
    s0.pending = c->shard.tail && !c->shard.resolved ? 1u : 0u;
    const std::vector<AnchorState> s0s(c->opt.n_lanes, s0);
    return hipMemcpy(c->anchor.d_state, s0s.data(), sizeof(AnchorState) * s0s.size(), hipMemcpyHostToDevice);
}
static size_t anchor_first_extra(uint32_t nl) { return 2 * (size_t)nl + 16; }

extern "C" int bqc_anchor_enqueue(bqc_ctx* c, const bqc_batch* b, void* d_cov, void* stream, bqc_anchored** out)
{
    if (!c || !b || !out || (b->n_reads && !d_cov)) return -BQC_ERR_ARG;
    *out = nullptr;
    AnchorEngine& E = c->anchor;
    const uint32_t nl = c->opt.n_lanes;
    if ((c->shard.tail && c->shard.resolved) || E.mode.load() == 2) return 1;
    const bool log_groups = c->shard.tail && nl > 1;
    {
        std::lock_guard<std::mutex> lk(E.m);
        if (E.outstanding) { E.err = "bqc_anchor_enqueue: the batch enqueued before has not been completed or discarded"; return -BQC_ERR_STATE; }
    }
    if (hipSetDevice(c->device) != hipSuccess) return anchor_fail(c, "hipSetDevice failed");
    hipStream_t st = (hipStream_t)stream;
    const size_t n = b->n_reads;
    const size_t sum_bytes = sizeof(AnchorSummary) + sizeof(AnchorLane) * nl;
    if (!E.d_state) {
        if (hipMalloc((void**)&E.d_state, sizeof(AnchorState) * nl) != hipSuccess || hipMalloc((void**)&E.d_sum, sum_bytes) != hipSuccess) return anchor_fail(c, "out of device memory");
        if (bqc_anchor_fresh_state(c) != hipSuccess) return anchor_fail(c, "copy failed");
    }
    const size_t first_extra = anchor_first_extra(nl);
    if (E.cap_n < n) {
        if (hipStreamSynchronize(st) != hipSuccess) return anchor_fail(c, "stream failed");
        if (E.d_scratch) (void)hipFree(E.d_scratch);
        E.d_scratch = nullptr; E.cap_n = 0;
        const size_t cap = std::max<size_t>(n + n / 8, 1u << 20), nbk = cap / 1024 + 4;
        const size_t bytes = cap * 24 + 4 * first_extra + 64 + AN_MAX_BREAKS * (4 + sizeof(AnchorRun)) + nbk * (2 * 4 + sizeof(AnchorPart)) + 4096 +
                             (nl > 1 ? 4 * nbk * (2 * (size_t)nl + 1) + cap + 1024 : 0) + (log_groups ? 4 * (size_t)nl + 9 * cap + 1024 : 0);
        if (hipMalloc(&E.d_scratch, bytes) != hipSuccess) return anchor_fail(c, "out of device memory");
        E.cap_n = cap;
    }
    bqc_anchored* a = nullptr;
    {
        std::lock_guard<std::mutex> lk(E.m);
        if (!E.free_list.empty()) { a = E.free_list.back(); E.free_list.pop_back(); a->released = false; }
    }
    if (!a) {
        a = new bqc_anchored();
        if (hipHostMalloc((void**)&a->h_sum, sum_bytes, hipHostMallocDefault) != hipSuccess ||
            hipHostMalloc((void**)&a->h_bound, sizeof(uint32_t) * bqc_anchored::kInline, hipHostMallocDefault) != hipSuccess) {
            if (a->h_sum) (void)hipHostFree(a->h_sum);
            delete a;
            return anchor_fail(c, "out of page-locked memory");
        }
        a->h_lanes = (AnchorLane*)(a->h_sum + 1);
        std::lock_guard<std::mutex> lk(E.m);
        E.all.push_back(a);
    }
    a->rest.clear(); a->pend_rid.clear(); a->pend_bp.clear(); a->pend_lane.clear(); a->completed = false; a->n = (uint32_t)n; a->d_cov = (const CovEntry*)d_cov;
    AnchorArgs A{};
    A.n = (uint32_t)n; A.n_refs = c->opt.n_refs; A.n_lanes = nl; A.no_fast = c->no_fast ? 1u : 0u;
    A.flag = b->flag; A.lane = b->lane; A.rid = b->rid; A.pos = b->pos; A.l_seq = b->l_seq; A.n_cigar = b->n_cigar;
    A.main_chrom = c->d_main;
    A.cov_out = (CovEntry*)d_cov; A.state = E.d_state; A.sum = E.d_sum; A.lanes = (AnchorLane*)(E.d_sum + 1);
    char* q = (char*)E.d_scratch;
    const size_t cap = E.cap_n, nbk = cap / 1024 + 4;
    A.cpos = (uint32_t*)q; q += 4 * cap; A.crid = (int32_t*)q; q += 4 * cap; A.cidx = (uint32_t*)q; q += 4 * cap; A.crun = (uint32_t*)q; q += 4 * cap;
    A.first_of = (uint32_t*)q; q += 8 * cap + 4 * first_extra + 64; A.first_cap = (uint32_t)std::min<size_t>(2 * cap + first_extra, 0xFFFFFFFFu);
    A.bj = (uint32_t*)q; q += 4 * AN_MAX_BREAKS; A.runs = (AnchorRun*)q; q += sizeof(AnchorRun) * AN_MAX_BREAKS;
    q = (char*)(((uintptr_t)q + 255) & ~(uintptr_t)255);
    A.blk_a = (uint32_t*)q; q += 4 * (cap / 1024 + 4); A.blk_b = (uint32_t*)q; q += 4 * (cap / 1024 + 4);
    q = (char*)(((uintptr_t)q + 255) & ~(uintptr_t)255);
    A.parts = (AnchorPart*)q;
    if (nl > 1) {
        q += sizeof(AnchorPart) * nbk;
        q = (char*)(((uintptr_t)q + 255) & ~(uintptr_t)255);
        A.blk_c = (uint32_t*)q; q += 4 * nbk * nl; A.blk_r = (uint32_t*)q; q += 4 * nbk * ((size_t)nl + 1); A.clane = (uint8_t*)q;
    }
    E.d_plog_bp = A.cpos; E.d_plog_rid = A.crid; E.d_plog_lane = nullptr;
    if (log_groups) {
        q += cap;
        q = (char*)(((uintptr_t)q + 255) & ~(uintptr_t)255);
        A.set_aside = 1;
        A.lane_fc = (uint32_t*)q; q += 4 * (size_t)nl;
        q = (char*)(((uintptr_t)q + 255) & ~(uintptr_t)255);
        A.plog_bp = (uint32_t*)q; q += 4 * cap; A.plog_rid = (int32_t*)q; q += 4 * cap; A.plog_lane = (uint8_t*)q;
        E.d_plog_bp = A.plog_bp; E.d_plog_rid = A.plog_rid; E.d_plog_lane = A.plog_lane;
    }
    E.d_bound = A.first_of;
    const size_t n_first = std::min<size_t>(2 * n + first_extra, A.first_cap);
    if (hipMemsetAsync(A.first_of, 0xFF, 4 * n_first, st) != hipSuccess) { anchor_release(E, a); return anchor_fail(c, "memset failed"); }
    bqc_launch_anchor(A, st);
    if (hipMemcpyAsync(a->h_sum, E.d_sum, sum_bytes, hipMemcpyDeviceToHost, st) != hipSuccess ||
        hipMemcpyAsync(a->h_bound, A.first_of, sizeof(uint32_t) * std::min<size_t>(bqc_anchored::kInline, n_first), hipMemcpyDeviceToHost, st) != hipSuccess) {
        anchor_release(E, a);
        return anchor_fail(c, "copy failed");
    }
    {
        std::lock_guard<std::mutex> lk(E.m);
        E.outstanding = a;
    }
    E.mode = 1;
    *out = a;
    return 0;
}

extern "C" int bqc_anchor_complete(bqc_ctx* c, bqc_anchored* a, bqc_anchor_info* info)
{
    if (!c || !a) return -BQC_ERR_ARG;
    AnchorEngine& E = c->anchor;
    {
        std::lock_guard<std::mutex> lk(E.m);
        if (E.outstanding == a) E.outstanding = nullptr;
    }
    const AnchorSummary& S = *a->h_sum;
    if (info) { info->n_noqual = S.n_noqual; info->rid_min = S.rid_min; info->rid_max = S.rid_max; }
    if (S.flags & AN_FLAG_BOUND_OVERFLOW) return anchor_fail(c, "internal error: boundary list overflow");
    if (S.flags & AN_FLAG_TOO_MANY_BREAKS) {
        E.mode = 2;
        anchor_release(E, a);
        return 1;
    }
    const uint32_t nl = c->opt.n_lanes;
    const size_t K = bqc_anchored::kInline;
    size_t end = 0;
    for (uint32_t l = 0; l < nl; ++l)
        if (lane_anchored(a->h_lanes, l)) end = std::max(end, (size_t)a->h_lanes[l].first_off + a->h_lanes[l].last_rel + 1);
    if (end > 2 * E.cap_n + anchor_first_extra(nl)) return anchor_fail(c, "internal error: a window table lies outside the anchors' scratch");
    if (end > K) {
        a->rest.resize(end - K);
        if (hipSetDevice(c->device) != hipSuccess ||
            hipMemcpy(a->rest.data(), E.d_bound + K, sizeof(uint32_t) * a->rest.size(), hipMemcpyDeviceToHost) != hipSuccess) return anchor_fail(c, "copy failed");
    }
    if (S.n_pending) {
        if (S.n_pending > a->n) return anchor_fail(c, "internal error: more reads set aside than the batch holds");
        a->pend_rid.resize(S.n_pending); a->pend_bp.resize(S.n_pending);
        if (E.d_plog_lane) a->pend_lane.resize(S.n_pending);
        if (hipSetDevice(c->device) != hipSuccess || hipMemcpy(a->pend_bp.data(), E.d_plog_bp, 4ull * S.n_pending, hipMemcpyDeviceToHost) != hipSuccess ||
            hipMemcpy(a->pend_rid.data(), E.d_plog_rid, 4ull * S.n_pending, hipMemcpyDeviceToHost) != hipSuccess ||
            (E.d_plog_lane && hipMemcpy(a->pend_lane.data(), E.d_plog_lane, S.n_pending, hipMemcpyDeviceToHost) != hipSuccess)) return anchor_fail(c, "copy failed");
    }
    a->completed = true;
    return 0;
}

extern "C" void bqc_anchor_discard(bqc_ctx* c, bqc_anchored* a)
{
    if (!c || !a) return;
    c->anchor.mode = 2;
    anchor_release(c->anchor, a);
}

extern "C" int bqc_submit_anchored(bqc_ctx* c, const bqc_batch* b, bqc_anchored* a, uint64_t* ticket)
{
    if (!c || !b || !a || !a->completed || a->n != b->n_reads) return bqc_fail(c, BQC_ERR_ARG, "bqc_submit_anchored: bad argument");
    if (b->n_nm_extra) return bqc_fail(c, BQC_ERR_ARG, "bqc_submit_anchored: further NM values belong to batches decoded on the host");
    const int rc = submit_impl(c, b, true, ticket, a);
    anchor_release(c->anchor, a);
    return rc;
}

void bqc_anchor_destroy(bqc_ctx* c)
{
    AnchorEngine& E = c->anchor;
    for (bqc_anchored* a : E.all) { if (a->h_sum) (void)hipHostFree(a->h_sum); if (a->h_bound) (void)hipHostFree(a->h_bound); delete a; }
    E.all.clear(); E.free_list.clear(); E.outstanding = nullptr;
    if (E.d_state) (void)hipFree(E.d_state);
    if (E.d_sum) (void)hipFree(E.d_sum);
    if (E.d_scratch) (void)hipFree(E.d_scratch);
    E.d_state = nullptr; E.d_sum = nullptr; E.d_scratch = nullptr; E.cap_n = 0;
}

extern "C" int bqc_batch_uploaded(bqc_ctx* c, uint64_t ticket, int wait)
{
    if (!c) return -BQC_ERR_ARG;
    if (ticket == 0 || ticket >= c->next_ticket) return 1;
    Slot& s = c->slots[ticket % bqc_ctx::kSlots];
    if (!s.busy || s.ticket != ticket) return 1;
    hipEvent_t ev = s.in_place ? s.ev_done : s.ev_h2d;
    if (wait) return hipEventSynchronize(ev) == hipSuccess ? 1 : -BQC_ERR_DEVICE;
    const hipError_t q = hipEventQuery(ev);
    return q == hipSuccess ? 1 : q == hipErrorNotReady ? 0 : -BQC_ERR_DEVICE;
}

extern "C" int bqc_host_register(void* p, uint64_t bytes)
{
    if (!p || !bytes) return BQC_ERR_ARG;
    return hipHostRegister(p, (size_t)bytes, hipHostRegisterDefault) == hipSuccess ? 0 : BQC_ERR_DEVICE;
}
extern "C" int bqc_host_unregister(void* p) { return p && hipHostUnregister(p) == hipSuccess ? 0 : BQC_ERR_DEVICE; }

namespace {
struct LaneWire { uint8_t first, started, pad0, pad1; int32_t id, shift; };
}
static size_t shard_bytes(const bqc_ctx* c) { return 8 + (size_t)c->opt.n_lanes * (sizeof(LaneWire) + 2 * BQC_VSIZE * 4); }
extern "C" uint64_t bqc_shard_state_bytes(const bqc_ctx* c) { return c ? shard_bytes(c) : 0; }

extern "C" int bqc_shard_fasta_span(bqc_ctx* c, int32_t span[2])
{
    if (!c || !span) return BQC_ERR_ARG;
    HIPCHK(c, hipSetDevice(c->device));
    const int rc = c->poisoned ? 0 : bqc_sync(c);
    if (rc) return rc;
    int32_t cur[2];
    HIPCHK(c, hipMemcpy(cur, c->d_cursor, 8, hipMemcpyDeviceToHost));
    span[0] = cur[1]; span[1] = cur[0];
    return 0;
}

extern "C" int bqc_shard_export(bqc_ctx* c, void* out)
{
    if (!c || !out) return bqc_fail(c, BQC_ERR_ARG, "bqc_shard_export: null argument");
    if (c->poisoned) return bqc_fail(c, BQC_ERR_STATE, "context is in an error state: %s", c->err.c_str());
    if (c->shard.tail && !c->shard.resolved) return bqc_fail(c, BQC_ERR_STATE, "bqc_shard_export before bqc_shard_resolve");
    if (c->flushed && !c->shard.exported) return bqc_fail(c, BQC_ERR_STATE, "bqc_shard_export after bqc_flush");
    HIPCHK(c, hipSetDevice(c->device));
    int rc = bqc_sync(c);
    if (rc) return rc;
    const uint32_t nl = c->opt.n_lanes;
    std::vector<uint32_t> parity(nl + 1);
    std::vector<uint8_t> started(nl);
    int32_t cur[2];
    HIPCHK(c, hipMemcpy(parity.data(), c->d_parity, 4 * (size_t)nl, hipMemcpyDeviceToHost));
    HIPCHK(c, hipMemcpy(started.data(), c->d_started, nl, hipMemcpyDeviceToHost));
    HIPCHK(c, hipMemcpy(cur, c->d_cursor, 8, hipMemcpyDeviceToHost));
    char* w = (char*)out;
    const int32_t head[2] = {cur[1], cur[0]};
    memcpy(w, head, 8); w += 8;
    for (uint32_t l = 0; l < nl; ++l) {
        const LaneCov& s = c->cov[l];
        const LaneWire lw{(uint8_t)s.first, started[l], 0, 0, s.id, (int32_t)s.shift};
        memcpy(w, &lw, sizeof lw); w += sizeof lw;
        HIPCHK(c, hipMemcpy(w, c->d_carry + ((size_t)l * 2 + (parity[l] & 1u)) * 2 * BQC_VSIZE, 2 * BQC_VSIZE * 4, hipMemcpyDeviceToHost));
        w += 2 * BQC_VSIZE * 4;
    }
    c->shard.exported = true;
    c->flushed = true;
    return 0;
}

extern "C" int bqc_shard_resolve(bqc_ctx* c, const void* pred)
{
    if (!c || !pred) return bqc_fail(c, BQC_ERR_ARG, "bqc_shard_resolve: null argument");
    if (c->poisoned) return bqc_fail(c, BQC_ERR_STATE, "context is in an error state: %s", c->err.c_str());
    ShardCtx& sh = c->shard;
    if (!sh.tail || sh.resolved) return bqc_fail(c, BQC_ERR_STATE, "bqc_shard_resolve: not a shard_tail context, or resolved already");
    if (c->flushed) return bqc_fail(c, BQC_ERR_STATE, "bqc_shard_resolve after bqc_flush");
    HIPCHK(c, hipSetDevice(c->device));
    int rc = bqc_sync(c);
    if (rc) return rc;
    const uint32_t nl = c->opt.n_lanes;
    const size_t carry_lane = 2 * 2 * BQC_VSIZE;
    const std::vector<LaneCov> main_cov = c->cov;
    uint32_t* d_save = nullptr;
    const size_t save_bytes = carry_lane * 4 * nl + 4 * ((size_t)nl + 1) + nl;
    HIPCHK(c, hipMalloc(&d_save, save_bytes + 256));
    uint32_t* d_save_par = d_save + carry_lane * nl;
    uint8_t* d_save_started = (uint8_t*)(d_save_par + nl + 1);
    HIPCHK(c, hipMemcpyAsync(d_save, c->d_carry, carry_lane * 4 * nl, hipMemcpyDeviceToDevice, c->stream));
    HIPCHK(c, hipMemcpyAsync(d_save_par, c->d_parity, 4 * ((size_t)nl + 1), hipMemcpyDeviceToDevice, c->stream));
    HIPCHK(c, hipMemcpyAsync(d_save_started, c->d_started, nl, hipMemcpyDeviceToDevice, c->stream));
    const char* r = (const char*)pred + 8;
    std::vector<uint32_t> carry_in(carry_lane * nl, 0);
    std::vector<uint8_t> started_in(nl);
    for (uint32_t l = 0; l < nl; ++l) {
        LaneWire lw;
        memcpy(&lw, r, sizeof lw); r += sizeof lw;
        LaneCov s;
        s.first = lw.first != 0; s.id = lw.id; s.shift = (uint32_t)lw.shift; s.win = 0; s.batch_base = 0;
        c->cov[l] = s;
        started_in[l] = lw.started;
        memcpy(carry_in.data() + carry_lane * l, r, 2 * BQC_VSIZE * 4); r += 2 * BQC_VSIZE * 4;
    }
    HIPCHK(c, hipMemcpyAsync(c->d_carry, carry_in.data(), carry_lane * 4 * nl, hipMemcpyHostToDevice, c->stream));
    HIPCHK(c, hipMemsetAsync(c->d_parity, 0, 4 * ((size_t)nl + 1), c->stream));
    HIPCHK(c, hipMemcpyAsync(c->d_started, started_in.data(), nl, hipMemcpyHostToDevice, c->stream));
    HIPCHK(c, hipStreamSynchronize(c->stream));
    HostPass& H = c->hp;
    void* d_work = nullptr;
    size_t work_cap = 0;
    for (PendBatch& pb : sh.batches) {
        const uint32_t n = pb.n();
        H.n = n; H.multi_lane = nl > 1;
        H.cov.resize(n);
        CovPlanner plan(c, H, n);
        for (uint32_t i = 0; i < n; ++i) {
            uint64_t rel;
            uint32_t pos;
            plan.step(i, pb.lane[i], pb.rid[i], pb.bp[i], rel, pos);
            if (rel > 0xFFFFFFF0ull) { (void)hipFree(d_save); (void)hipFree(d_work); return poison(c, bqc_fail(c, BQC_ERR_ARG, "shard spans too many coverage windows")); }
            H.cov[i] = CovEntry{(uint32_t)rel, pos};
        }
        plan.finish();
        Carver cv;
        const size_t o_cin = cv.take(sizeof(CovEntry) * (size_t)n), o_lane = cv.take(n), o_tiles = cv.take(sizeof(CovTile) * H.tiles.size()), o_mask = cv.take(nl),
                     o_started = cv.take(nl), o_aidx = cv.take(8 * H.add_idx.size()), o_aval = cv.take(8 * H.add_val.size()), o_h2d_end = cv.off,
                     o_cov = cv.take(sizeof(CovEntry) * (size_t)n), o_covx = cv.take(sizeof(CovExtra) * ((size_t)pb.extra_cap + 1)), o_desc = cv.take(sizeof(BatchDesc));
        if (work_cap < cv.off) {
            if (d_work) (void)hipFree(d_work);
            d_work = nullptr;
            const hipError_t he = hipMalloc(&d_work, cv.off + cv.off / 4);
            if (he != hipSuccess) { (void)hipFree(d_save); return poison(c, bqc_fail(c, BQC_ERR_DEVICE, "hipMalloc failed: %s", hipGetErrorString(he))); }
            work_cap = cv.off + cv.off / 4;
        }
        std::vector<char> img(o_h2d_end);
        memcpy(img.data() + o_cin, H.cov.data(), sizeof(CovEntry) * (size_t)n);
        memcpy(img.data() + o_lane, pb.lane.data(), n);
        if (!H.tiles.empty()) memcpy(img.data() + o_tiles, H.tiles.data(), sizeof(CovTile) * H.tiles.size());
        memcpy(img.data() + o_mask, H.lane_mask.data(), nl);
        memcpy(img.data() + o_started, H.started_after.data(), nl);
        if (!H.add_idx.empty()) { memcpy(img.data() + o_aidx, H.add_idx.data(), 8 * H.add_idx.size()); memcpy(img.data() + o_aval, H.add_val.data(), 8 * H.add_val.size()); }
        char* base = (char*)d_work;
        HIPCHK(c, hipMemcpyAsync(base, img.data(), o_h2d_end, hipMemcpyHostToDevice, c->stream));
        const PendRun* pend = (const PendRun*)pb.dmem;
        const uint32_t* extra_n = (const uint32_t*)((const char*)pb.dmem + sizeof(PendRun) * (size_t)n);
        const PendExtra* extra = (const PendExtra*)((const char*)extra_n + 256);
        bqc_launch_pend_cov(n, (const CovEntry*)(base + o_cin), pend, extra, extra_n, pb.extra_cap, (const uint8_t*)(base + o_lane), (CovEntry*)(base + o_cov),
                            (CovExtra*)(base + o_covx), (BatchDesc*)(base + o_desc), c->stream);
        DevBatch d{};
        d.n_reads = n; d.lane = (const uint8_t*)(base + o_lane); d.cov = (const CovEntry*)(base + o_cov); d.cov_extra = (const CovExtra*)(base + o_covx);
        d.desc = (const BatchDesc*)(base + o_desc); d.cov_tiles = (const CovTile*)(base + o_tiles); d.n_cov_tiles = (uint32_t)H.tiles.size();
        if (!d.n_cov_tiles) bqc_launch_or_bytes(c->d_started, (const uint8_t*)(base + o_started), nl, c->stream);
        else bqc_launch_cov(d, c->sl, c->d_state, c->d_carry, c->d_parity, (const uint8_t*)(base + o_mask), c->d_started, (const uint8_t*)(base + o_started), nl, c->stream);
        bqc_launch_add_words(c->d_state, (const uint64_t*)(base + o_aidx), (const uint64_t*)(base + o_aval), (uint32_t)H.add_idx.size(), c->stream);
        HIPCHK(c, hipStreamSynchronize(c->stream));
        (void)hipFree(pb.dmem);
        pb.dmem = nullptr;
    }
    sh.batches.clear();
    std::vector<uint8_t> sel(nl, 0);
    bool any = false;
    for (uint32_t l = 0; l < nl; ++l) { sel[l] = sh.pending[l] ? 0 : 1; any |= sel[l] != 0; }
    if (any) {
        uint8_t* d_sel = (uint8_t*)d_save + save_bytes;
        HIPCHK(c, hipMemcpyAsync(d_sel, sel.data(), nl, hipMemcpyHostToDevice, c->stream));
        bqc_launch_cov_final(c->sl, c->d_state, c->d_carry, c->d_parity, c->d_started, d_sel, 0, c->stream);
        for (uint32_t l = 0; l < nl; ++l)
            if (sel[l]) {
                c->cov[l] = main_cov[l];
                HIPCHK(c, hipMemcpyAsync(c->d_carry + carry_lane * l, d_save + carry_lane * l, carry_lane * 4, hipMemcpyDeviceToDevice, c->stream));
                HIPCHK(c, hipMemcpyAsync(c->d_parity + l, d_save_par + l, 4, hipMemcpyDeviceToDevice, c->stream));
                HIPCHK(c, hipMemcpyAsync(c->d_started + l, d_save_started + l, 1, hipMemcpyDeviceToDevice, c->stream));
            }
    }
    HIPCHK(c, hipStreamSynchronize(c->stream));
    (void)hipFree(d_save);
    if (d_work) (void)hipFree(d_work);
    for (uint32_t l = 0; l < nl; ++l) sh.pending[l] = 0;
    sh.resolved = true;
    return 0;
}
```

### bamqc_amd/csrc/k_cov.hip

```cpp
#include "kernels_common.h"

#define KC_AT(p) ((p) + (((p) >> 6) << 2))
__global__ __launch_bounds__(256) void k_cov(DevBatch b, StateLayout sl, uint64_t* __restrict__ state,
                                                uint32_t* __restrict__ carry , uint32_t* parity ,
                                                const uint8_t* __restrict__ lane_mask, uint8_t* __restrict__ started,
                                                const uint8_t* __restrict__ started_after, uint32_t n_lanes)
{
    __shared__ __attribute__((aligned(16))) int32_t diff[4096 + 256];
    __shared__ uint32_t hist[BQC_COVSIZE + 1];
    __shared__ uint32_t wsum[4];
    for (uint32_t i = threadIdx.x; i <= BQC_COVSIZE; i += blockDim.x) hist[i] = 0;
    for (uint32_t i = threadIdx.x; i < 4096 + 256; i += blockDim.x) diff[i] = 0;
    uint32_t cur_lane = 0xFFFFFFFFu;
    CovTile t{};
    t.lane = 0xFFFFFFFFu;
    CovEntry e0{0, 0}, e1{0, 0};
    auto load = [&](const CovTile& tt, uint32_t i) {
        CovEntry e = b.cov[i];
        if (tt.mixed && b.lane[i] != tt.lane) e.off_len = 0;
        return e;
    };
    if (blockIdx.x < b.n_cov_tiles) {
        t = b.cov_tiles[blockIdx.x];
        const uint32_t i0 = t.list_begin + threadIdx.x, i1 = i0 + blockDim.x;
        if (i0 < t.list_end) e0 = load(t, i0);
        if (i1 < t.list_end) e1 = load(t, i1);
    }
    const uint32_t n_extra = b.desc->n_cov_extra;
    for (uint32_t ti = blockIdx.x;; ti += gridDim.x) {
        const bool done = ti >= b.n_cov_tiles;
        if (done) t.lane = 0xFFFFFFFFu;
        if (t.lane != cur_lane) {
            block_sync();
            if (cur_lane != 0xFFFFFFFFu)
                for (uint32_t i = threadIdx.x; i <= BQC_COVSIZE; i += blockDim.x)
                    if (hist[i]) { gadd(state + sl.lane_base(cur_lane) + sl.o_poscov + i, hist[i]); hist[i] = 0; }
            cur_lane = t.lane;
        }
        if (done) break;
        block_sync();
        const int64_t lo = (int64_t)t.win_lo * BQC_VSIZE;
        auto add = [&](const CovEntry& e) {
            const uint32_t len = e.off_len >> 16;
            if (!len) return;
            int64_t a = (int64_t)e.win * BQC_VSIZE + (e.off_len & 0xFFFFu) - lo, z = a + len;
            if (a < 0) a = 0;
            if (z > BQC_COV_TILE) z = BQC_COV_TILE;
            if (a < z) { atomicAdd(&diff[KC_AT((uint32_t)a)], 1); atomicAdd(&diff[KC_AT((uint32_t)z)], -1); }
        };
        add(e0); add(e1);
        for (uint32_t e = t.list_begin + 2 * blockDim.x + threadIdx.x; e < t.list_end; e += blockDim.x) add(load(t, e));
        for (uint32_t e = threadIdx.x; e < n_extra; e += blockDim.x) {
            const CovExtra x = b.cov_extra[e];
            if (x.lane == t.lane) add(CovEntry{x.win, x.off_len});
        }
        const CovTile tc = t;
        {
            const uint32_t tn = ti + gridDim.x;
            e0 = CovEntry{0, 0}; e1 = CovEntry{0, 0};
            if (tn < b.n_cov_tiles) {
                t = b.cov_tiles[tn];
                const uint32_t i0 = t.list_begin + threadIdx.x, i1 = i0 + blockDim.x;
                if (i0 < t.list_end) e0 = load(t, i0);
                if (i1 < t.list_end) e1 = load(t, i1);
            }
        }
        block_sync();
        const uint32_t s0 = threadIdx.x * 16u;
        int32_t d[16];
#pragma unroll
        for (int q = 0; q < 4; ++q) {
            const int4 v = *(const int4*)&diff[KC_AT(s0) + 4 * q];
            d[4 * q] = v.x; d[4 * q + 1] = v.y; d[4 * q + 2] = v.z; d[4 * q + 3] = v.w;
        }
        int32_t loc = 0;
#pragma unroll
        for (int j = 0; j < 16; ++j) loc += (s0 + j < BQC_COV_TILE) ? d[j] : 0;
        const int32_t inc = (int32_t)wave_scan_incl((uint32_t)loc);
        if (lane_id() == WAVE - 1) wsum[threadIdx.x >> 6] = (uint32_t)inc;
        block_sync();
#pragma unroll
        for (int q = 0; q < 4; ++q) *(int4*)&diff[KC_AT(s0) + 4 * q] = make_int4(0, 0, 0, 0);
        int32_t off = inc - loc;
        for (uint32_t w = 0; w < (threadIdx.x >> 6); ++w) off += (int32_t)wsum[w];
        const uint32_t par = parity[tc.lane] & 1u;
        const uint32_t* cin = carry + ((uint64_t)tc.lane * 2 + par) * 2000;
        uint32_t* cout = carry + ((uint64_t)tc.lane * 2 + (par ^ 1u)) * 2000;
        int32_t run = off;
        uint32_t run_bin = 0xFFFFFFFFu, run_n = 0;
        if (lo >= 2 * BQC_VSIZE && tc.win_lo + BQC_COV_TILE_WINDOWS <= tc.win_final) {
#pragma unroll
            for (int j = 0; j < 16; ++j) {
                if (s0 + j >= BQC_COV_TILE) continue;
                run += d[j];
                const uint32_t bin = min((uint32_t)run, (uint32_t)BQC_COVSIZE);
                if (bin == run_bin) ++run_n;
                else { if (run_n) atomicAdd(&hist[run_bin], run_n); run_bin = bin; run_n = 1; }
            }
        } else
#pragma unroll
        for (int j = 0; j < 16; ++j) {
            const uint32_t p = s0 + j;
            if (p >= BQC_COV_TILE) continue;
            run += d[j];
            const int64_t vp = lo + p;
            uint32_t depth = (uint32_t)run;
            if (vp < 2 * BQC_VSIZE) depth += cin[vp];
            const uint32_t win = tc.win_lo + p / BQC_VSIZE;
            if (win < tc.win_final) {
                const uint32_t bin = depth > BQC_COVSIZE ? BQC_COVSIZE : depth;
                if (bin == run_bin) ++run_n;
                else { if (run_n) atomicAdd(&hist[run_bin], run_n); run_bin = bin; run_n = 1; }
            } else if (win < tc.win_final + 2) cout[(win - tc.win_final) * BQC_VSIZE + p % BQC_VSIZE] = depth;
        }
        if (run_n) atomicAdd(&hist[run_bin], run_n);
    }
    block_sync();
    if (threadIdx.x == 0) wsum[0] = atomicAdd(parity + n_lanes, 1u) == gridDim.x - 1u ? 1u : 0u;
    block_sync();
    if (wsum[0]) {
        for (uint32_t l = threadIdx.x; l < n_lanes; l += blockDim.x) {
            if (lane_mask[l]) parity[l] ^= 1u;
            if (started_after[l]) started[l] = 1;
        }
        if (threadIdx.x == 0) parity[n_lanes] = 0u;
    }
}

__global__ __launch_bounds__(256) void k_cov_final(StateLayout sl, uint64_t* __restrict__ state, const uint32_t* __restrict__ carry,
                                                      const uint32_t* __restrict__ parity, const uint8_t* __restrict__ started, const uint8_t* __restrict__ sel,
                                                      uint32_t count_start)
{
    __shared__ uint32_t hist[BQC_COVSIZE + 1];
    const uint32_t lane = blockIdx.x;
    if (!started[lane] || (sel && !sel[lane])) return;
    for (uint32_t i = threadIdx.x; i <= BQC_COVSIZE; i += blockDim.x) hist[i] = 0;
    block_sync();
    const uint32_t* c = carry + ((uint64_t)lane * 2 + (parity[lane] & 1u)) * 2000;
    for (uint32_t i = threadIdx.x; i < 2000; i += blockDim.x) {
        const uint32_t d = c[i];
        atomicAdd(&hist[d > BQC_COVSIZE ? BQC_COVSIZE : d], 1u);
    }
    block_sync();
    for (uint32_t i = threadIdx.x; i <= BQC_COVSIZE; i += blockDim.x)
        if (hist[i]) gadd(state + sl.lane_base(lane) + sl.o_poscov + i, hist[i]);
    if (threadIdx.x == 0 && count_start) gadd(state + sl.lane_base(lane) + sl.o_covstart, 1);
}

__global__ void k_or_bytes(uint8_t* __restrict__ dst, const uint8_t* __restrict__ src, uint32_t n)
{
    const uint32_t i = blockIdx.x * blockDim.x + threadIdx.x;
    if (i < n && src[i]) dst[i] = 1;
}

__global__ void k_add_words(uint64_t* __restrict__ state, const uint64_t* __restrict__ idx, const uint64_t* __restrict__ val, uint32_t n)
{
    const uint32_t i = blockIdx.x * blockDim.x + threadIdx.x;
    if (i < n) gadd(state + idx[i], val[i]);
}

__global__ void k_err_merge(ErrRec* __restrict__ dst, const ErrRec* __restrict__ src)
{
    if (dst->first_key == BQC_ERRKEY_NONE && dst->flags == 0 && (src->first_key != BQC_ERRKEY_NONE || src->flags != 0)) *dst = *src;
}
extern "C" void bqc_launch_err_merge(ErrRec* dst, const ErrRec* src, hipStream_t s) { hipLaunchKernelGGL(k_err_merge, dim3(1), dim3(1), 0, s, dst, src); }

extern "C" void bqc_launch_cov(const DevBatch& b, const StateLayout& sl, uint64_t* state, uint32_t* carry, uint32_t* parity, const uint8_t* lane_mask,
                               uint8_t* started, const uint8_t* started_after, uint32_t n_lanes, hipStream_t s)
{
    if (b.n_cov_tiles == 0) return;
    const uint32_t grid = b.n_cov_tiles < 2048u ? b.n_cov_tiles : 2048u;
    hipLaunchKernelGGL(k_cov, dim3(grid), dim3(256), 0, s, b, sl, state, carry, parity, lane_mask, started, started_after, n_lanes);
}

extern "C" void bqc_launch_cov_final(const StateLayout& sl, uint64_t* state, const uint32_t* carry, const uint32_t* parity,
                                     const uint8_t* started, const uint8_t* sel, uint32_t count_start, hipStream_t s)
{
    hipLaunchKernelGGL(k_cov_final, dim3(sl.n_lanes), dim3(256), 0, s, sl, state, carry, parity, started, sel, count_start);
}

extern "C" void bqc_launch_add_words(uint64_t* state, const uint64_t* idx, const uint64_t* val, uint32_t n, hipStream_t s)
{
    if (n) hipLaunchKernelGGL(k_add_words, dim3((n + 255) / 256), dim3(256), 0, s, state, idx, val, n);
}

extern "C" void bqc_launch_or_bytes(uint8_t* dst, const uint8_t* src, uint32_t n, hipStream_t s)
{
    if (n) hipLaunchKernelGGL(k_or_bytes, dim3((n + 255) / 256), dim3(256), 0, s, dst, src, n);
}

__global__ void k_calib_read4(const uint32_t* __restrict__ p, uint64_t n_dwords, uint32_t* __restrict__ out)
{
    uint32_t acc = 0;
    for (uint64_t i = (uint64_t)blockIdx.x * blockDim.x + threadIdx.x; i < n_dwords; i += (uint64_t)gridDim.x * blockDim.x) acc ^= p[i];
    if (acc == 0x12345678u) out[0] = acc;
}
__global__ void k_calib_read8(const uint2* __restrict__ p, uint64_t n, uint32_t* __restrict__ out)
{
    uint32_t acc = 0;
    for (uint64_t i = (uint64_t)blockIdx.x * blockDim.x + threadIdx.x; i < n; i += (uint64_t)gridDim.x * blockDim.x) { const uint2 v = p[i]; acc ^= v.x ^ v.y; }
    if (acc == 0x12345678u) out[0] = acc;
}
extern "C" int bqc_calib_read4(uint64_t bytes, int repeat)
{
    uint32_t* p = nullptr;
    uint32_t* o = nullptr;
    if (hipMalloc(&p, bytes) != hipSuccess || hipMalloc(&o, 64) != hipSuccess) return 2;
    (void)hipMemset(p, 1, bytes);
    for (int r = 0; r < repeat; ++r) hipLaunchKernelGGL(k_calib_read4, dim3(256 * 8), dim3(256), 0, 0, p, bytes / 4, o);
    for (int r = 0; r < repeat; ++r) hipLaunchKernelGGL(k_calib_read8, dim3(256 * 8), dim3(256), 0, 0, (const uint2*)p, bytes / 8, o);
    (void)hipDeviceSynchronize();
    (void)hipFree(p); (void)hipFree(o);
    return 0;
}
```

### bamqc_amd/csrc/k_prep.hip

```cpp
#include <algorithm>
#include "kernels_common.h"
#include "prep.h"

#define PR_THREADS 256
#define PR_PER_THREAD 4
#define PR_BLOCK (PR_THREADS * PR_PER_THREAD)

__device__ __forceinline__ uint32_t wave_scan_incl_max(uint32_t v)
{
    v = max(v, (uint32_t)__builtin_amdgcn_update_dpp(0, (int)v, 0x111, 0xF, 0xF, true));
    v = max(v, (uint32_t)__builtin_amdgcn_update_dpp(0, (int)v, 0x112, 0xF, 0xF, true));
    v = max(v, (uint32_t)__builtin_amdgcn_update_dpp(0, (int)v, 0x114, 0xF, 0xF, true));
    v = max(v, (uint32_t)__builtin_amdgcn_update_dpp(0, (int)v, 0x118, 0xF, 0xF, true));
    v = max(v, (uint32_t)__builtin_amdgcn_update_dpp(0, (int)v, 0x142, 0xA, 0xF, false));
    v = max(v, (uint32_t)__builtin_amdgcn_update_dpp(0, (int)v, 0x143, 0xC, 0xF, false));
    return v;
}
__device__ __forceinline__ uint32_t block_scan_excl(uint32_t v, uint32_t* sh, uint32_t* total)
{
    const uint32_t inc = wave_scan_incl(v), w = threadIdx.x >> 6, nw = blockDim.x >> 6;
    block_sync();
    if (lane_id() == WAVE - 1) sh[w] = inc;
    block_sync();
    uint32_t base = 0, tot = 0;
    for (uint32_t k = 0; k < nw; ++k) { const uint32_t x = sh[k]; if (k < w) base += x; tot += x; }
    *total = tot;
    return base + inc - v;
}
__device__ __forceinline__ uint32_t block_scan_excl_max(uint32_t v, uint32_t* sh, uint32_t* total)
{
    const uint32_t inc = wave_scan_incl_max(v), w = threadIdx.x >> 6, nw = blockDim.x >> 6;
    block_sync();
    if (lane_id() == WAVE - 1) sh[w] = inc;
    block_sync();
    uint32_t base = 0, tot = 0;
    for (uint32_t k = 0; k < nw; ++k) { const uint32_t x = sh[k]; if (k < w) base = max(base, x); tot = max(tot, x); }
    *total = tot;
    const uint32_t prev = (uint32_t)__builtin_amdgcn_update_dpp(0, (int)inc, 0x138 , 0xF, 0xF, true);
    return max(base, prev);
}
__device__ __forceinline__ void err_key(ErrRec* e, uint32_t read, uint32_t order)
{
    atomicMin(&e->first_key, ((unsigned long long)read << 3) | order);
}

__global__ __launch_bounds__(PR_THREADS) void k_prep_sizes(PrepArgs a)
{
    __shared__ unsigned long long sh[3 * (PR_THREADS / 64)];
    if (blockIdx.x == 0 && threadIdx.x == 0) {
        a.err->first_key = BQC_ERRKEY_NONE; a.err->flags = 0; a.err->aux0 = a.err->aux1 = 0;
        a.desc->n_cov_extra = 0;
        if (a.pend_extra_n) *a.pend_extra_n = 0;
        if (a.replay) *a.cursor = *a.cursor_save; else *a.cursor_save = *a.cursor;
    }
    for (uint32_t k = blockIdx.x * PR_THREADS + threadIdx.x; k < a.n_sw; k += gridDim.x * PR_THREADS) a.sw_counts[k] = SwCounts{0, 0, 0, 0};
    const uint32_t b0 = blockIdx.x * PR_BLOCK;
    unsigned long long s1 = 0, s2 = 0, s3 = 0;
#pragma unroll
    for (int j = 0; j < PR_PER_THREAD; ++j) {
        const uint32_t i = b0 + j * PR_THREADS + threadIdx.x;
        if (i < a.n) { const uint32_t L = a.l_seq[i]; s1 += (L + 1) / 2; s2 += L; s3 += a.n_cigar[i]; }
    }
#pragma unroll
    for (int o = 32; o > 0; o >>= 1) { s1 += __shfl_xor(s1, o); s2 += __shfl_xor(s2, o); s3 += __shfl_xor(s3, o); }
    if (lane_id() == 0) { const uint32_t w = threadIdx.x >> 6; sh[3 * w] = s1; sh[3 * w + 1] = s2; sh[3 * w + 2] = s3; }
    block_sync();
    if (threadIdx.x < 3) {
        unsigned long long t = 0;
        for (uint32_t w = 0; w < PR_THREADS / 64; ++w) t += sh[3 * w + threadIdx.x];
        a.blk_sizes[3ull * blockIdx.x + threadIdx.x] = t;
    }
}

__global__ __launch_bounds__(1024) void k_prep_scan(PrepArgs a)
{
    __shared__ unsigned long long sh[3 * 1024];
    const uint32_t nblk = (a.n + PR_BLOCK - 1) / PR_BLOCK;
    const uint32_t per = (nblk + blockDim.x - 1) / blockDim.x;
    const uint32_t lo = min(nblk, threadIdx.x * per), hi = min(nblk, lo + per);
    unsigned long long t[3] = {0, 0, 0};
    for (uint32_t b = lo; b < hi; ++b)
        for (int k = 0; k < 3; ++k) t[k] += a.blk_sizes[3ull * b + k];
    for (int k = 0; k < 3; ++k) sh[3 * threadIdx.x + k] = t[k];
    block_sync();
    for (uint32_t d = 1; d < blockDim.x; d <<= 1) {
        unsigned long long v[3] = {0, 0, 0};
        if (threadIdx.x >= d) for (int k = 0; k < 3; ++k) v[k] = sh[3 * (threadIdx.x - d) + k];
        block_sync();
        for (int k = 0; k < 3; ++k) sh[3 * threadIdx.x + k] += v[k];
        block_sync();
    }
    unsigned long long run[3];
    for (int k = 0; k < 3; ++k) run[k] = sh[3 * threadIdx.x + k] - t[k];
    for (uint32_t b = lo; b < hi; ++b) {
        bool over = false;
        for (int k = 0; k < 3; ++k) {
            const unsigned long long s = a.blk_sizes[3ull * b + k];
            a.blk_sizes[3ull * b + k] = run[k];
            run[k] += s;
            over |= run[k] > 0xFFFFFFFFull;
        }
        if (over) err_key(a.err, b * PR_BLOCK, 3);
    }
}

struct CigarView {
    uint32_t w[4];
    const uint32_t* cg;
    __device__ __forceinline__ uint32_t at(uint32_t k) const
    {
        if (k < 4u) return k == 0u ? w[0] : k == 1u ? w[1] : k == 2u ? w[2] : w[3];
        return cg[k];
    }
};
__device__ __forceinline__ int triplet_eligible(uint32_t flag, uint32_t mapq, int32_t as, const CigarView& cv, uint32_t ncig)
{
    if (!(flag & 0x1) || !(flag & 0x2) || (flag & 0x4) || (flag & 0x8) || (flag & 0x100)) return 0;
    if (mapq < 60) return 0;
    if (as == BQC_AS_ABSENT || as < 0) return -1;
    if (as < 50) return 0;
    uint32_t clipped = 0;
    for (uint32_t k = 0; k < ncig; ++k) {
        const uint32_t wd = cv.at(k), op = wd & 15u;
        if (op == 4u || op == 5u) clipped += wd >> 4;
    }
    return clipped > 0 ? 0 : 1;
}

struct ReadIn { uint32_t L, nc, flag, lane, mapq; int32_t rid, pos, as; CovEntry ce; };
struct ReadOut { uint32_t flag, cls, tgt1; CovEntry ce; };
__device__ __forceinline__ ReadOut prep_one(const PrepArgs& a, const DevRefs& refs, uint32_t i, const ReadIn& in, uint32_t co, bool offsets_ok,
                                            const CigarView& cv, bool ref_loaded , int32_t target_in )
{
    ReadOut o;
    uint32_t flag = in.flag & (0x0FFFu | BQC_FLAG_MATE_MAIN | BQC_FLAG_NO_QUAL);
    const uint32_t L = in.L, lane = in.lane;
    uint32_t nc = in.nc;
    o.tgt1 = 0;
    if (L > a.max_read_len) err_key(a.err, i, 1);
    else if (lane >= a.n_lanes) err_key(a.err, i, 2);
    if (!offsets_ok) nc = 0;
    const bool fast = !a.no_fast && L <= BQC_FAST_MAXLEN;
    uint32_t nseg = 0;
    CovEntry ce = in.ce;
    if (!(flag & 0x900u)) {
        const bool dup = flag & 0x400u, qcf = flag & 0x200u;
        if (!dup && !qcf) {
            const int e = triplet_eligible(flag, in.mapq, in.as, cv, nc);
            if (e < 0) err_key(a.err, i, 4);
            if (e > 0) {
                const int32_t target = target_in;
                if (target < 0 || !ref_loaded) err_key(a.err, i, 5);
                else { o.tgt1 = (uint32_t)target + 1u; flag |= BQC_FLAG_TRIPLET; }
            }
        }
        if (!(flag & 0xC0u)) err_key(a.err, i, 6);
    }
    if (ce.win != BQC_COV_NONE) {
        flag |= BQC_FLAG_COV;
        const bool rc = flag & 0x10u;
        const bool pending = ce.win == BQC_COV_PENDING;
        const uint32_t pend_idx = ce.off_len;
        const int64_t pos = pending ? 0 : (int64_t)ce.off_len;
        uint32_t cc = 0;
        int64_t run_a = -1, run_z = -1;
        bool first = true;
        ce.off_len = 0;
        auto emit = [&](int64_t lo, int64_t hi) {
            if (pending) {
                if (lo < 0 || lo >= 2 * BQC_VSIZE || lo >= hi) return;
                const uint32_t len = (uint32_t)(hi - lo < 2 * BQC_VSIZE ? hi - lo : 2 * BQC_VSIZE);
                if (first) { a.pend[pend_idx] = PendRun{(uint32_t)lo, len}; first = false; return; }
                const uint32_t k = atomicAdd(a.pend_extra_n, 1u);
                if (k < a.pend_extra_cap) a.pend_extra[k] = PendExtra{pend_idx, (uint32_t)lo, len, 0};
                else atomicOr(&a.err->flags, BQC_DEVERR_INTERNAL);
                return;
            }
            hi = hi < 2 * BQC_VSIZE ? hi : 2 * BQC_VSIZE;
            if (lo < 0 || lo >= hi) return;
            const uint32_t v = (uint32_t)lo | ((uint32_t)(hi - lo) << 16);
            if (first) { ce.off_len = v; first = false; return; }
            const uint32_t k = atomicAdd(&a.desc->n_cov_extra, 1u);
            if (k < a.cov_extra_cap) a.cov_extra[k] = CovExtra{ce.win, v, lane, 0};
            else atomicOr(&a.err->flags, BQC_DEVERR_INTERNAL);
        };
        if (nc == 1u) {
            const uint32_t w = cv.w[0], op = w & 15u, nn = w >> 4;
            if (op == 0u || op == 2u) emit(pos, pos + nn);
        } else {
            for (uint32_t k = 0; k < nc; ++k) {
                const uint32_t w = cv.at(rc ? nc - 1 - k : k), op = w & 15u, nn = w >> 4;
                if (op == 4u) cc += nn;
                if (op == 0u || op == 2u) {
                    const int64_t lo = pos + (int64_t)cc, hi = lo + nn;
                    if (run_z == lo) run_z = hi;
                    else { if (run_a >= 0) emit(run_a, run_z); run_a = lo; run_z = hi; }
                    cc += nn;
                }
            }
            if (run_a >= 0) emit(run_a, run_z);
        }
        if (pending) { if (first) a.pend[pend_idx] = PendRun{0, 0}; ce = CovEntry{BQC_COV_NONE, 0}; }
    } else ce.off_len = 0;
    if (fast && (flag & BQC_FLAG_TRIPLET) && nc > 1 && L >= 3) {
        const uint32_t n0 = cv.w[0] >> 4;
        if (n0 != 0) {
            uint64_t rp = n0;
            int64_t cpos = (int64_t)in.pos + n0;
            for (uint32_t k2 = 1; k2 < nc && rp < L; ++k2) {
                const uint32_t wk = cv.at(k2), op = wk & 15u, nn = wk >> 4;
                if (op == 2u || op == 3u || op == 5u || op == 6u) cpos += nn;
                else if (op == 4u || op == 1u) rp += nn;
                else {
                    const uint64_t ia = rp > 1 ? rp : 1, ib = rp + nn < (uint64_t)L - 1 ? rp + nn : (uint64_t)L - 1;
                    const int64_t posv = cpos - (int64_t)rp;
                    if (ia < ib && posv > INT32_MIN / 2 && posv < INT32_MAX / 2) {
                        a.segs[co + nseg] = TripSeg{i, (int32_t)posv, (uint32_t)ia | ((uint32_t)ib << 8), 0};
                        ++nseg;
                    }
                    rp += nn; cpos += nn;
                }
            }
        }
    }
    o.flag = flag;
    o.ce = ce;
    o.cls = ((fast ? ((flag & 0x40u) ? 0u : 1u) : 2u) << 8) | nseg;
    return o;
}

#ifndef PR_WAVES_PER_EU
#define PR_WAVES_PER_EU 4
#endif
__global__ __launch_bounds__(PR_THREADS) __attribute__((amdgpu_waves_per_eu(PR_WAVES_PER_EU, PR_WAVES_PER_EU))) void k_prep_reads(PrepArgs a, DevRefs refs)
{
    __shared__ uint32_t sh[2 * (PR_THREADS / 64)];
    __shared__ uint32_t red[8];
    const uint32_t i0 = blockIdx.x * PR_BLOCK + 4u * threadIdx.x;
    const unsigned long long gs = a.blk_sizes[3ull * blockIdx.x], gq = a.blk_sizes[3ull * blockIdx.x + 1], gc = a.blk_sizes[3ull * blockIdx.x + 2];
    if (threadIdx.x < 8) red[threadIdx.x] = threadIdx.x == 0 ? 0xFFFFFFFFu : 0u;
    ReadIn in[4];
    const uint32_t nlive = i0 >= a.n ? 0u : min(4u, a.n - i0);
    if (nlive == 4u) {
        const uint4 vl = *(const uint4*)(a.l_seq + i0);
        const uint2 vc = *(const uint2*)(a.n_cigar + i0), vf = *(const uint2*)(a.flag_in + i0);
        const uint32_t vlane = *(const uint32_t*)(a.lane + i0), vmq = *(const uint32_t*)(a.mapq + i0);
        const int4 vr = *(const int4*)(a.rid + i0), vp = *(const int4*)(a.pos + i0), va = *(const int4*)(a.as_ + i0);
        const uint4 c01 = *(const uint4*)(a.cov_in + i0), c23 = *(const uint4*)(a.cov_in + i0 + 2);
        const uint32_t Ls[4] = {vl.x, vl.y, vl.z, vl.w}, ncs[4] = {vc.x & 0xFFFFu, vc.x >> 16, vc.y & 0xFFFFu, vc.y >> 16};
        const uint32_t fs[4] = {vf.x & 0xFFFFu, vf.x >> 16, vf.y & 0xFFFFu, vf.y >> 16};
        const int32_t rs[4] = {vr.x, vr.y, vr.z, vr.w}, ps[4] = {vp.x, vp.y, vp.z, vp.w}, as[4] = {va.x, va.y, va.z, va.w};
        const CovEntry cs[4] = {{c01.x, c01.y}, {c01.z, c01.w}, {c23.x, c23.y}, {c23.z, c23.w}};
#pragma unroll
        for (int j = 0; j < 4; ++j) in[j] = ReadIn{Ls[j], ncs[j], fs[j], (vlane >> (8 * j)) & 0xFFu, (vmq >> (8 * j)) & 0xFFu, rs[j], ps[j], as[j], cs[j]};
    } else {
#pragma unroll
        for (int j = 0; j < 4; ++j) {
            in[j] = ReadIn{0, 0, 0x900u, 0, 0, -1, 0, 0, CovEntry{BQC_COV_NONE, 0}};
            if ((uint32_t)j < nlive) { const uint32_t i = i0 + j; in[j] = ReadIn{a.l_seq[i], a.n_cigar[i], a.flag_in[i], a.lane[i], a.mapq[i], a.rid[i], a.pos[i], a.as_[i], a.cov_in[i]}; }
        }
    }
    uint32_t ls[4], lq[4], lc[4], ts = 0, tq = 0, tc = 0;
#pragma unroll
    for (int j = 0; j < 4; ++j) { ls[j] = ts; lq[j] = tq; lc[j] = tc; ts += (in[j].L + 1) / 2; tq += in[j].L; tc += in[j].nc; }
    uint32_t tot;
    const unsigned long long bs = gs + block_scan_excl(ts, sh, &tot), bq = gq + block_scan_excl(tq, sh, &tot), bc = gc + block_scan_excl(tc, sh, &tot);
    ReadOut out[4];
    CigarView cv[4];
    bool ref_loaded[4];
    int32_t target[4];
    unsigned long long cos[4];
    bool oks[4];
#pragma unroll
    for (int j = 0; j < 4; ++j) {
        const unsigned long long so = bs + ls[j], qo = bq + lq[j], co = bc + lc[j];
        cos[j] = co;
        oks[j] = so + (in[j].L + 1) / 2 <= 0xFFFFFFFFull && qo + in[j].L <= 0xFFFFFFFFull && co + in[j].nc <= 0xFFFFFFFFull;
        const bool live = (uint32_t)j < nlive && oks[j];
        cv[j].cg = a.cigar + (uint32_t)co;
#pragma unroll
        for (uint32_t k = 0; k < 4u; ++k) cv[j].w[k] = live && k < in[j].nc ? cv[j].cg[k] : 0u;
        const int32_t rid = in[j].rid;
        const bool rid_ok = (uint32_t)j < nlive && rid >= 0 && (uint32_t)rid < refs.n_refs;
        ref_loaded[j] = rid_ok && refs.ref[rid] != nullptr;
        target[j] = rid_ok ? (a.fasta_index ? a.fasta_index[rid] : rid) : -1;
    }
    uint32_t tmax = 0, tmin = 0xFFFFFFFFu, maxfast = 0, maxlong = 0, cnt[4] = {0, 0, 0, 0};
    bool local_bad[4] = {false, false, false, false};
#pragma unroll
    for (int j = 0; j < 4; ++j) {
        out[j] = ReadOut{0x900u, 2u << 8, 0, CovEntry{BQC_COV_NONE, 0}};
        if ((uint32_t)j >= nlive) continue;
        out[j] = prep_one(a, refs, i0 + j, in[j], (uint32_t)cos[j], oks[j], cv[j], ref_loaded[j], target[j]);
        if (out[j].tgt1) { local_bad[j] = out[j].tgt1 < tmax; tmax = max(tmax, out[j].tgt1); tmin = min(tmin, out[j].tgt1); }
        const uint32_t cl = out[j].cls >> 8;
        if (cl == 2u) maxlong = max(maxlong, in[j].L); else maxfast = max(maxfast, in[j].L);
        cnt[cl] += 1; cnt[3] += out[j].cls & 0xFFu;
    }
    if (nlive == 4u) {
        *(uint4*)(a.seq_off + i0) = make_uint4((uint32_t)bs + ls[0], (uint32_t)bs + ls[1], (uint32_t)bs + ls[2], (uint32_t)bs + ls[3]);
        *(uint4*)(a.qual_off + i0) = make_uint4((uint32_t)bq + lq[0], (uint32_t)bq + lq[1], (uint32_t)bq + lq[2], (uint32_t)bq + lq[3]);
        *(uint4*)(a.cigar_off + i0) = make_uint4((uint32_t)bc + lc[0], (uint32_t)bc + lc[1], (uint32_t)bc + lc[2], (uint32_t)bc + lc[3]);
        *(uint2*)(a.flag_out + i0) = make_uint2(out[0].flag | (out[1].flag << 16), out[2].flag | (out[3].flag << 16));
        *(uint2*)(a.cls + i0) = make_uint2(out[0].cls | (out[1].cls << 16), out[2].cls | (out[3].cls << 16));
        *(uint4*)(a.cov_out + i0) = make_uint4(out[0].ce.win, out[0].ce.off_len, out[1].ce.win, out[1].ce.off_len);
        *(uint4*)(a.cov_out + i0 + 2) = make_uint4(out[2].ce.win, out[2].ce.off_len, out[3].ce.win, out[3].ce.off_len);
    } else {
        for (uint32_t j = 0; j < nlive; ++j) {
            const uint32_t i = i0 + j;
            a.seq_off[i] = (uint32_t)bs + ls[j]; a.qual_off[i] = (uint32_t)bq + lq[j]; a.cigar_off[i] = (uint32_t)bc + lc[j];
            a.flag_out[i] = (uint16_t)out[j].flag; a.cls[i] = (uint16_t)out[j].cls; a.cov_out[i] = out[j].ce;
        }
    }
    uint32_t blk_max;
    const uint32_t before = block_scan_excl_max(tmax, sh, &blk_max);
#pragma unroll
    for (int j = 0; j < 4; ++j)
        if (out[j].tgt1 && (local_bad[j] || out[j].tgt1 < before)) err_key(a.err, i0 + j, 5);
    if (tmin != 0xFFFFFFFFu) atomicMin(&red[0], tmin);
    if (maxfast) atomicMax(&red[1], maxfast);
    if (maxlong) atomicMax(&red[2], maxlong);
    if (!a.order) {
#pragma unroll
        for (int k = 0; k < 4; ++k) { const uint32_t v = wave_sum(cnt[k]); if (lane_id() == 0 && v) atomicAdd(&red[4 + k], v); }
    }
    block_sync();
    if (threadIdx.x == 0) {
        a.blk_tgt[2ull * blockIdx.x] = blk_max;
        a.blk_tgt[2ull * blockIdx.x + 1] = red[0];
        a.blk_maxfast[2ull * blockIdx.x] = red[1];
        a.blk_maxfast[2ull * blockIdx.x + 1] = red[2];
    }
    if (!a.order && threadIdx.x < 4 && red[4 + threadIdx.x])
        atomicAdd((uint32_t*)&a.sw_counts[blockIdx.x / (BQC_SW_READS / PR_BLOCK)] + threadIdx.x, red[4 + threadIdx.x]);
}

__device__ __forceinline__ uint32_t read_class(const PrepArgs& a, uint32_t r, uint32_t* nseg)
{
    const uint32_t v = a.cls[r];
    *nseg = v & 0xFFu;
    return v >> 8;
}

__global__ __launch_bounds__(PR_THREADS) void k_build_count(PrepArgs a)
{
    __shared__ uint32_t sh[4 * (PR_THREADS / 64)];
    const SuperWindow sw = a.sws[blockIdx.x];
    uint32_t c[4] = {0, 0, 0, 0};
    for (uint32_t p = threadIdx.x; p < sw.count; p += PR_THREADS) {
        const uint32_t r = a.order ? a.order[sw.begin + p] : sw.begin + p;
        uint32_t ns;
        const uint32_t cl = read_class(a, r, &ns);
        c[cl] += 1;
        c[3] += ns;
    }
    for (int k = 0; k < 4; ++k) c[k] = wave_sum(c[k]);
    if (lane_id() == 0) for (int k = 0; k < 4; ++k) sh[4 * (threadIdx.x >> 6) + k] = c[k];
    block_sync();
    if (threadIdx.x < 4) {
        uint32_t t = 0;
        for (uint32_t w = 0; w < PR_THREADS / 64; ++w) t += sh[4 * w + threadIdx.x];
        ((uint32_t*)&a.sw_counts[blockIdx.x])[threadIdx.x] = t;
    }
}

__global__ __launch_bounds__(1024) void k_build_plan(PrepArgs a)
{
    __shared__ uint32_t sh[2 * 16 + 8];
    __shared__ uint32_t s_fast_w, s_first_bad, s_gmin;
    const uint32_t nblk = (a.n + PR_BLOCK - 1) / PR_BLOCK;
    {
        uint32_t carry = (uint32_t)(*a.cursor + 1);
        uint32_t mf = 0, gmin = 0xFFFFFFFFu;
        if (threadIdx.x == 0) { s_first_bad = 0xFFFFFFFFu; s_gmin = 0xFFFFFFFFu; }
        for (uint32_t b0 = 0; b0 < nblk; b0 += blockDim.x) {
            const uint32_t b = b0 + threadIdx.x;
            const uint32_t mx = b < nblk ? a.blk_tgt[2ull * b] : 0u, mn = b < nblk ? a.blk_tgt[2ull * b + 1] : 0xFFFFFFFFu;
            if (b < nblk) mf = max(mf, a.blk_maxfast[2ull * b]);
            uint32_t tot;
            const uint32_t before = max(carry, block_scan_excl_max(mx, sh, &tot));
            gmin = min(gmin, mn);
            if (mn < before) atomicMin(&s_first_bad, b);
            carry = max(carry, tot);
        }
        if (gmin != 0xFFFFFFFFu) atomicMin(&s_gmin, gmin);
        block_sync();
        const uint32_t bad = s_first_bad;
        if (bad != 0xFFFFFFFFu) {
            uint32_t before = (uint32_t)(*a.cursor + 1);
            for (uint32_t b = threadIdx.x; b < bad; b += blockDim.x) before = max(before, a.blk_tgt[2ull * b]);
            uint32_t tot;
            (void)block_scan_excl_max(before, sh, &tot);
            for (uint32_t i = bad * PR_BLOCK + threadIdx.x; i < min(a.n, (bad + 1) * PR_BLOCK); i += blockDim.x)
                if (a.flag_out[i] & BQC_FLAG_TRIPLET) {
                    const int32_t rid = a.rid[i];
                    const uint32_t t1 = (uint32_t)(a.fasta_index ? a.fasta_index[rid] : rid) + 1u;
                    if (t1 < tot) err_key(a.err, i, 5);
                }
        }
        for (int o = 32; o > 0; o >>= 1) mf = max(mf, (uint32_t)__shfl_xor((int)mf, o));
        block_sync();
        if (lane_id() == 0) sh[threadIdx.x >> 6] = mf;
        block_sync();
        if (threadIdx.x == 0) {
            uint32_t m = 0;
            for (uint32_t w = 0; w < blockDim.x / 64; ++w) m = max(m, sh[w]);
            s_fast_w = max(1u, (m + 8 * BQC_FAST_NH - 1) / (8 * BQC_FAST_NH));
            *a.cursor = (int32_t)carry - 1;
            if (a.cursor[1] < 0 && s_gmin != 0xFFFFFFFFu) a.cursor[1] = (int32_t)s_gmin - 1;
        }
        block_sync();
    }
    const uint32_t fast_w = s_fast_w, rpw = 64u / fast_w, h0 = (rpw + 1) / 2, h1 = rpw / 2;
    const uint32_t groups_cap = BQC_FAST_WAVES * (64u / rpw);
    const uint32_t seg_cap = groups_cap * rpw;
    uint32_t run_g = 0, run_q = 0, run_s = 0;
    for (uint32_t s0 = 0; s0 < a.n_sw; s0 += blockDim.x) {
        const uint32_t s = s0 + threadIdx.x;
        uint32_t g = 0, q = 0, sl = 0;
        if (s < a.n_sw) {
            const SwCounts c = a.sw_counts[s];
            g = max((c.n0 + h0 - 1) / h0, (c.n1 + h1 - 1) / h1);
            q = c.n_seg; sl = c.n_slow;
        }
        uint32_t tg, tq, ts;
        const uint32_t eg = run_g + block_scan_excl(g, sh, &tg), eq = run_q + block_scan_excl(q, sh, &tq), es = run_s + block_scan_excl(sl, sh, &ts);
        if (s < a.n_sw) a.sw_plan[s] = SwPlan{eg, g, eq, es};
        run_g += tg; run_q += tq; run_s += ts;
    }
    __threadfence_block();
    block_sync();
    __shared__ uint32_t s_pb, s_cf, s_cs, s_g0, s_q0, s_s0, s_ng, s_nq, s_ns, s_lane, s_sw0, s_sw1, s_longest;
    if (threadIdx.x == 0) { s_pb = 0; s_cf = 0; s_cs = 0; }
    block_sync();
    for (uint32_t st = 0; st < a.n_stretch; ++st) {
        if (threadIdx.x == 0) {
            const Stretch S = a.stretches[st];
            const SwPlan p0 = a.sw_plan[S.sw_begin];
            const SwPlan pl = a.sw_plan[S.sw_end - 1];
            const SwCounts cl = a.sw_counts[S.sw_end - 1];
            s_g0 = p0.group_base; s_q0 = p0.seg_base; s_s0 = p0.slow_base;
            s_ng = pl.group_base + pl.n_groups - p0.group_base;
            s_nq = pl.seg_base + cl.n_seg - p0.seg_base;
            s_ns = pl.slow_base + cl.n_slow - p0.slow_base;
            s_lane = S.lane; s_sw0 = S.sw_begin; s_sw1 = S.sw_end;
        }
        block_sync();
        const uint32_t pb = s_pb, ng = s_ng, nq = s_nq, ns = s_ns, lane = s_lane;
        const uint32_t nq_pad = (nq + rpw - 1) / rpw * rpw;
        const uint32_t seg0 = pb + ng * rpw, slow0 = seg0 + nq_pad;
        for (uint32_t s = s_sw0 + threadIdx.x; s < s_sw1; s += blockDim.x) {
            SwPlan p = a.sw_plan[s];
            p.group_base = pb + (p.group_base - s_g0) * rpw;
            p.seg_base = seg0 + (p.seg_base - s_q0);
            p.slow_base = slow0 + (p.slow_base - s_s0);
            a.sw_plan[s] = p;
        }
        for (uint32_t k = nq + threadIdx.x; k < nq_pad; k += blockDim.x) a.perm[seg0 + k] = 0xFFFFFFFFu;
        const uint32_t n_rc = (ng + groups_cap - 1) / groups_cap, n_sc = (nq_pad + seg_cap - 1) / seg_cap, n_lc = (ns + BQC_CHUNK_READS - 1) / BQC_CHUNK_READS;
        const uint32_t cf = s_cf, cs = s_cs;
        for (uint32_t k = threadIdx.x; k < n_rc; k += blockDim.x) {
            const uint32_t g = min(groups_cap, ng - k * groups_cap);
            if (cf + k < a.chunks_fast_cap) a.chunks_fast[cf + k] = Chunk{pb + k * groups_cap * rpw, g * rpw, lane, g * rpw, 0, 0, 0, 0};
        }
        for (uint32_t k = threadIdx.x; k < n_sc; k += blockDim.x) {
            const uint32_t e = min(seg_cap, nq_pad - k * seg_cap);
            if (cf + n_rc + k < a.chunks_fast_cap) a.chunks_fast[cf + n_rc + k] = Chunk{seg0 + k * seg_cap, e, lane, 0, 0, 0, 0, 0};
        }
        for (uint32_t k = threadIdx.x; k < n_lc; k += blockDim.x) {
            const uint32_t e = min((uint32_t)BQC_CHUNK_READS, ns - k * BQC_CHUNK_READS);
            if (cs + k < a.chunks_slow_cap) a.chunks_slow[cs + k] = Chunk{slow0 + k * BQC_CHUNK_READS, e, lane, 0, 0, 0, 0, 0};
        }
        block_sync();
        if (threadIdx.x == 0) { s_pb = slow0 + ns; s_cf = cf + n_rc + n_sc; s_cs = cs + n_lc; }
        block_sync();
    }
    uint32_t longest = 0;
    for (uint32_t b = threadIdx.x; b < nblk; b += blockDim.x) longest = max(longest, a.blk_maxfast[2ull * b + 1]);
    for (int o = 32; o > 0; o >>= 1) longest = max(longest, (uint32_t)__shfl_xor((int)longest, o));
    if (threadIdx.x == 0) s_longest = 0;
    block_sync();
    if (lane_id() == 0) atomicMax(&s_longest, longest);
    block_sync();
    if (threadIdx.x == 0) {
        if (s_pb > a.perm_cap || s_cf > a.chunks_fast_cap || s_cs > a.chunks_slow_cap) atomicOr(&a.err->flags, BQC_DEVERR_INTERNAL);
        const bool fatal = a.err->first_key != BQC_ERRKEY_NONE || (a.err->flags & BQC_DEVERR_INTERNAL);
        a.desc->fatal = fatal ? 1u : 0u;
        a.desc->n_chunks_fast = fatal ? 0u : min(s_cf, a.chunks_fast_cap);
        a.desc->n_chunks_slow = fatal ? 0u : min(s_cs, a.chunks_slow_cap);
        a.desc->fast_w = fast_w;
        a.desc->n_perm = s_pb;
        a.desc->long_max_len = s_longest;
        if (a.desc->n_cov_extra > a.cov_extra_cap) a.desc->n_cov_extra = a.cov_extra_cap;
        const unsigned long long key = a.err->first_key;
        if (key != BQC_ERRKEY_NONE) {
            const uint32_t i = (uint32_t)(key >> 3), order = (uint32_t)key & 7u;
            if (i < a.n) { a.err->aux0 = order == 1 ? a.l_seq[i] : order == 2 ? a.lane[i] : (uint32_t)a.rid[i]; a.err->aux1 = a.lane[i]; }
        }
    }
}

__device__ __forceinline__ void block_scan_excl4(uint32_t v[4], uint32_t* sh, uint32_t tot[4])
{
    const uint32_t w = threadIdx.x >> 6, nw = blockDim.x >> 6;
    uint32_t inc[4];
#pragma unroll
    for (int k = 0; k < 4; ++k) inc[k] = wave_scan_incl(v[k]);
    block_sync();
    if (lane_id() == WAVE - 1) {
#pragma unroll
        for (int k = 0; k < 4; ++k) sh[4 * w + k] = inc[k];
    }
    block_sync();
#pragma unroll
    for (int k = 0; k < 4; ++k) {
        uint32_t base = 0, t = 0;
        for (uint32_t q = 0; q < nw; ++q) { const uint32_t x = sh[4 * q + k]; if (q < w) base += x; t += x; }
        tot[k] = t;
        v[k] = base + inc[k] - v[k];
    }
}

#define SC_PER (BQC_SW_READS / PR_THREADS)
#define SC_ENT (3 * BQC_SW_READS + 128)
__global__ __launch_bounds__(PR_THREADS) void k_build_scatter(PrepArgs a)
{
    __shared__ uint32_t ent[SC_ENT];
    __shared__ uint32_t sh[4 * (PR_THREADS / 64)];
    const SuperWindow sw = a.sws[blockIdx.x];
    const SwPlan pl = a.sw_plan[blockIdx.x];
    const uint32_t fast_w = a.desc->fast_w, rpw = 64u / fast_w, h0 = (rpw + 1) / 2, h1 = rpw / 2;
    const uint32_t n_ent = pl.n_groups * rpw;
    if (n_ent > SC_ENT) { if (threadIdx.x == 0) atomicOr(&a.err->flags, BQC_DEVERR_INTERNAL); return; }
    for (uint32_t k = threadIdx.x; k < n_ent; k += PR_THREADS) ent[k] = 0xFFFFFFFFu;
    uint32_t r[SC_PER], v[SC_PER];
    const uint32_t p0 = SC_PER * threadIdx.x;
    if (!a.order && p0 + SC_PER <= sw.count && ((sw.begin + p0) & 7u) == 0u) {
        const uint4 x = *(const uint4*)(a.cls + sw.begin + p0), y = *(const uint4*)(a.cls + sw.begin + p0 + 8);
        const uint32_t wd[8] = {x.x, x.y, x.z, x.w, y.x, y.y, y.z, y.w};
#pragma unroll
        for (int k = 0; k < SC_PER; ++k) { r[k] = sw.begin + p0 + k; v[k] = (wd[k >> 1] >> (16 * (k & 1))) & 0xFFFFu; }
    } else {
#pragma unroll
        for (int k = 0; k < SC_PER; ++k) { const uint32_t p = p0 + k; r[k] = p < sw.count ? (a.order ? a.order[sw.begin + p] : sw.begin + p) : 0xFFFFFFFFu; }
#pragma unroll
        for (int k = 0; k < SC_PER; ++k) v[k] = r[k] != 0xFFFFFFFFu ? a.cls[r[k]] : 3u << 8;
    }
    uint32_t c[4] = {0, 0, 0, 0};
#pragma unroll
    for (int k = 0; k < SC_PER; ++k) {
        const uint32_t cl = v[k] >> 8;
        c[0] += cl == 0u; c[1] += cl == 1u; c[2] += cl == 2u; c[3] += cl < 3u ? v[k] & 0xFFu : 0u;
    }
    uint32_t co[SC_PER];
#pragma unroll
    for (int k = 0; k < SC_PER; ++k) co[k] = (v[k] >> 8) < 3u && (v[k] & 0xFFu) ? a.cigar_off[r[k]] : 0u;
    uint32_t tot[4];
    block_scan_excl4(c, sh, tot);
    uint32_t k0 = c[0], k1 = c[1], k2 = c[2], k3 = c[3];
#pragma unroll
    for (int k = 0; k < SC_PER; ++k) {
        const uint32_t cl = v[k] >> 8, ns = v[k] & 0xFFu;
        if (cl == 0u) { ent[(k0 / h0) * rpw + k0 % h0] = r[k]; ++k0; }
        else if (cl == 1u) { ent[(k1 / h1) * rpw + h0 + k1 % h1] = r[k]; ++k1; }
        else if (cl == 2u) a.perm[pl.slow_base + k2++] = r[k];
        if (cl < 3u && ns) { for (uint32_t j = 0; j < ns; ++j) a.perm[pl.seg_base + k3 + j] = BQC_ENTRY_SEG | (co[k] + j); k3 += ns; }
    }
    block_sync();
    for (uint32_t k = threadIdx.x; k < n_ent; k += PR_THREADS) a.perm[pl.group_base + k] = ent[k];
}

extern "C" void bqc_launch_prep(const PrepArgs& a, const DevRefs& refs, hipStream_t s)
{
    if (a.n == 0) return;
    const uint32_t nblk = (a.n + PR_BLOCK - 1) / PR_BLOCK;
    hipLaunchKernelGGL(k_prep_sizes, dim3(nblk), dim3(PR_THREADS), 0, s, a);
    hipLaunchKernelGGL(k_prep_scan, dim3(1), dim3(1024), 0, s, a);
    hipLaunchKernelGGL(k_prep_reads, dim3(nblk), dim3(PR_THREADS), 0, s, a, refs);
    if (a.order) hipLaunchKernelGGL(k_build_count, dim3(a.n_sw), dim3(PR_THREADS), 0, s, a);
    hipLaunchKernelGGL(k_build_plan, dim3(1), dim3(1024), 0, s, a);
    hipLaunchKernelGGL(k_build_scatter, dim3(a.n_sw), dim3(PR_THREADS), 0, s, a);
}

__device__ __forceinline__ uint32_t pend_interval(uint32_t pos, uint32_t c0, uint32_t len)
{
    const uint32_t lo = pos + c0;
    if (!len || lo >= 2u * BQC_VSIZE) return 0u;
    const uint32_t hi = min(lo + len, 2u * BQC_VSIZE);
    return lo | ((hi - lo) << 16);
}
__global__ __launch_bounds__(256) void k_pend_cov(uint32_t n, const CovEntry* __restrict__ cov_in, const PendRun* __restrict__ pend, const PendExtra* __restrict__ extra,
                                                     const uint32_t* __restrict__ extra_n, uint32_t extra_cap, const uint8_t* __restrict__ lane,
                                                     CovEntry* __restrict__ cov_out, CovExtra* __restrict__ cov_extra, BatchDesc* __restrict__ desc)
{
    const uint32_t ne = min(*extra_n, extra_cap);
    for (uint32_t i = blockIdx.x * blockDim.x + threadIdx.x; i < n; i += gridDim.x * blockDim.x) {
        const CovEntry ce = cov_in[i];
        const PendRun r = pend[i];
        cov_out[i] = CovEntry{ce.win, pend_interval(ce.off_len, r.c0, r.len)};
    }
    for (uint32_t e = blockIdx.x * blockDim.x + threadIdx.x; e < ne; e += gridDim.x * blockDim.x) {
        const PendExtra x = extra[e];
        const CovEntry ce = cov_in[x.idx];
        cov_extra[e] = CovExtra{ce.win, pend_interval(ce.off_len, x.c0, x.len), lane[x.idx], 0};
    }
    if (blockIdx.x == 0 && threadIdx.x == 0) { desc->n_cov_extra = ne; desc->fatal = 0; }
}
extern "C" void bqc_launch_pend_cov(uint32_t n, const CovEntry* cov_in, const PendRun* pend, const PendExtra* extra, const uint32_t* extra_n, uint32_t extra_cap,
                                    const uint8_t* lane, CovEntry* cov_out, CovExtra* cov_extra, BatchDesc* desc, hipStream_t s)
{
    if (!n) return;
    hipLaunchKernelGGL(k_pend_cov, dim3(std::min<uint32_t>((n + 255) / 256, 4096u)), dim3(256), 0, s, n, cov_in, pend, extra, extra_n, extra_cap, lane, cov_out, cov_extra, desc);
}
```

### bamqc_amd/csrc/prep.h

```cpp
#pragma once
#include <stdint.h>
#include "device_types.h"

struct Stretch {
    uint32_t lane, sw_begin, sw_end, pad;
};

struct PrepArgs {
    uint32_t n;
    uint32_t n_lanes, max_read_len;
    uint32_t no_fast;
    uint32_t replay;
    const uint16_t* flag_in;
    const uint8_t* mapq;
    const uint8_t* lane;
    const int32_t* rid;
    const int32_t* pos;
    const int32_t* as_;
    const uint32_t* l_seq;
    const uint16_t* n_cigar;
    const uint8_t* qual;
    const uint32_t* cigar;
    const CovEntry* cov_in;
    const uint32_t* order;
    const SuperWindow* sws;
    uint32_t n_sw;
    const Stretch* stretches;
    uint32_t n_stretch;
    const int32_t* fasta_index;
    uint16_t* flag_out;
    uint32_t* seq_off;
    uint32_t* qual_off;
    uint32_t* cigar_off;
    CovEntry* cov_out;
    CovExtra* cov_extra;
    uint32_t cov_extra_cap;
    PendRun* pend;
    PendExtra* pend_extra;
    uint32_t* pend_extra_n;
    uint32_t pend_extra_cap;
    uint16_t* cls;
    TripSeg* segs;
    uint32_t* perm;
    uint32_t perm_cap;
    Chunk* chunks_fast;
    uint32_t chunks_fast_cap;
    Chunk* chunks_slow;
    uint32_t chunks_slow_cap;
    BatchDesc* desc;
    ErrRec* err;
    int32_t* cursor;
    int32_t* cursor_save;
    unsigned long long* blk_sizes;
    uint32_t* blk_tgt;
    uint32_t* blk_maxfast;
    SwCounts* sw_counts;
    SwPlan* sw_plan;
};

extern "C" void bqc_launch_prep(const PrepArgs& a, const DevRefs& refs, hipStream_t s);
extern "C" void bqc_launch_pend_cov(uint32_t n, const CovEntry* cov_in, const PendRun* pend, const PendExtra* extra, const uint32_t* extra_n, uint32_t extra_cap,
                                    const uint8_t* lane, CovEntry* cov_out, CovExtra* cov_extra, BatchDesc* desc, hipStream_t s);
```

Before: 4.428 billion.

## Run coverage on low-priority side stream and drop separate prep scan kernel

Coverage and add-words kernels now fork onto a separate low-priority stream right after k_prep_reads, overlapping with the build/short/long kernels, and join back before error merge. The prep size pass is restructured into grouped blocks with vectorised loads, and the single-block scan kernel is removed: each prep_reads block computes its base offsets from per-group totals. This adds cross-stream event sync and relies on coverage not conflicting with concurrent state updates. It also clamps n_cov_extra to its capacity in k_cov.

```diff
diff --git a/bamqc_amd/csrc/bqc_api.cpp b/bamqc_amd/csrc/bqc_api.cpp
--- a/bamqc_amd/csrc/bqc_api.cpp
+++ b/bamqc_amd/csrc/bqc_api.cpp
@@ -96,6 +96,8 @@
     c->ref_len.assign(nr, 0);
     const char* v = getenv("BQC_NO_FAST");
     c->no_fast = v && v[0] == '1';
+    const char* cs = getenv("BQC_COV_STREAM");
+    c->cov_side = !(cs && cs[0] == '0');
 #define CCHK(call)                                                                                            \
     do {                                                                                                      \
         hipError_t e_ = (call);                                                                               \
@@ -191,6 +193,12 @@
         }
     }
     hipStream_t s = nullptr;
+    if (rank == BQC_STREAM_RANK_COV) {
+        int least = 0, greatest = 0;
+        if (hipDeviceGetStreamPriorityRange(&least, &greatest) != hipSuccess) { (void)hipGetLastError(); least = 0; }
+        if (hipStreamCreateWithPriority(&s, hipStreamNonBlocking, least) != hipSuccess) { (void)hipGetLastError(); return nullptr; }
+        return s;
+    }
     if (hipStreamCreateWithFlags(&s, hipStreamNonBlocking) != hipSuccess) { (void)hipGetLastError(); return nullptr; }
     return s;
 }
@@ -233,6 +241,7 @@
     if (!c) return;
     (void)hipSetDevice(c->device);
     if (c->copy_stream) (void)hipStreamSynchronize(c->copy_stream);
+    if (c->cov_stream) (void)hipStreamSynchronize(c->cov_stream);
     if (c->stream) (void)hipStreamSynchronize(c->stream);
     bqc_pipeline_destroy(c);
     bqc_anchor_destroy(c);
@@ -248,6 +257,9 @@
     for (auto e : c->ev) (void)hipEventDestroy(e);
     if (c->stream) (void)hipStreamDestroy(c->stream);
     if (c->copy_stream) (void)hipStreamDestroy(c->copy_stream);
+    if (c->cov_stream) (void)hipStreamDestroy(c->cov_stream);
+    if (c->ev_cov_fork) (void)hipEventDestroy(c->ev_cov_fork);
+    if (c->ev_cov_join) (void)hipEventDestroy(c->ev_cov_join);
     delete c;
 }
 
diff --git a/bamqc_amd/csrc/bqc_ctx.h b/bamqc_amd/csrc/bqc_ctx.h
--- a/bamqc_amd/csrc/bqc_ctx.h
+++ b/bamqc_amd/csrc/bqc_ctx.h
@@ -135,6 +135,9 @@
     int device = 0;
     hipStream_t stream = nullptr;
     hipStream_t copy_stream = nullptr;
+    hipStream_t cov_stream = nullptr;
+    bool cov_side = true;
+    hipEvent_t ev_cov_fork = nullptr, ev_cov_join = nullptr;
     uint32_t n_cu = 256;
     uint64_t* d_state = nullptr;
     ErrRec* d_err0 = nullptr;
@@ -195,6 +198,7 @@
         if (e_ != hipSuccess) return bqc_fail(c, BQC_ERR_DEVICE, "%s failed: %s", #call, hipGetErrorString(e_)); \
     } while (0)
 
+#define BQC_STREAM_RANK_COV 4
 hipStream_t bqc_pool_stream(int device, int rank);
 int bqc_copy_stream(bqc_ctx* c);
 int bqc_report_errors(bqc_ctx* c, const ErrRec& e);
diff --git a/bamqc_amd/csrc/bqc_pipeline.cpp b/bamqc_amd/csrc/bqc_pipeline.cpp
--- a/bamqc_amd/csrc/bqc_pipeline.cpp
+++ b/bamqc_amd/csrc/bqc_pipeline.cpp
@@ -14,7 +14,7 @@
 void bqc_launch_long(const DevBatch&, const StateLayout&, uint64_t*, const DevRefs&, uint32_t*, uint32_t*, uint32_t max_len_ub, uint32_t max_read_len, uint32_t, uint32_t, uint32_t* t8rows, uint32_t* t8_used, uint32_t t8_lane, uint32_t* cyc_tiles, uint32_t* cyc_used, uint32_t slot_cap, hipStream_t);
 uint32_t bqc_long_slots(uint32_t max_len_ub, uint32_t max_read_len, uint32_t n_chunks_ub, uint32_t n_cu);
 void bqc_launch_cov(const DevBatch&, const StateLayout&, uint64_t*, uint32_t* carry, uint32_t* parity, const uint8_t* lane_mask, uint8_t* started,
-                    const uint8_t* started_after, uint32_t n_lanes, hipStream_t);
+                    const uint8_t* started_after, uint32_t n_lanes, uint32_t cov_extra_cap, hipStream_t);
 void bqc_launch_add_words(uint64_t* state, const uint64_t* idx, const uint64_t* val, uint32_t n, hipStream_t);
 void bqc_launch_or_bytes(uint8_t* dst, const uint8_t* src, uint32_t n, hipStream_t);
 void bqc_launch_short(const DevBatch&, const StateLayout&, uint64_t*, const DevRefs&, uint32_t*, uint32_t grid, uint32_t* t8rows, uint32_t* t8_used, hipStream_t);
@@ -359,7 +359,7 @@
     const size_t o_flag2 = cv.take(2 * n), o_soff = cv.take(4 * n), o_qoff = cv.take(4 * n), o_cgoff = cv.take(4 * n), o_cov = cv.take(sizeof(CovEntry) * n),
                  o_covx = cv.take(sizeof(CovExtra) * cx_cap), o_cls = cv.take(2 * n), o_segs = cv.take(sizeof(TripSeg) * (H.cigar_words + 1)),
                  o_perm = cv.take(4 * perm_cap), o_cf = cv.take(sizeof(Chunk) * cf_cap), o_cs = cv.take(sizeof(Chunk) * cs_cap),
-                 o_desc = cv.take(sizeof(BatchDesc)), o_err = cv.take(sizeof(ErrRec)), o_cursave = cv.take(8), o_bsz = cv.take(24 * nblk), o_btgt = cv.take(8 * nblk),
+                 o_desc = cv.take(sizeof(BatchDesc)), o_err = cv.take(sizeof(ErrRec)), o_cursave = cv.take(8), o_bsz = cv.take(24 * nblk), o_gsz = cv.take(24 * ((nblk + PR_GROUP - 1) / PR_GROUP)), o_btgt = cv.take(8 * nblk),
                  o_bmf = cv.take(8 * nblk), o_swc = cv.take(sizeof(SwCounts) * n_sw), o_swp = cv.take(sizeof(SwPlan) * n_sw),
                  o_rsum = cv.take(H.n_slow ? 12 * n : 0), o_otmp = cv.take(order_on_device && H.multi_lane ? 4 * lane_order_tmp_words((uint32_t)n, nl) : 0);
     const size_t need = cv.off + 256;
@@ -415,7 +415,7 @@
     p.chunks_slow = (Chunk*)(base + o_cs); p.chunks_slow_cap = (uint32_t)cs_cap;
     p.desc = (BatchDesc*)(base + o_desc); p.err = (ErrRec*)(base + o_err);
     p.cursor = c->d_cursor; p.cursor_save = (int32_t*)(base + o_cursave);
-    p.blk_sizes = (unsigned long long*)(base + o_bsz); p.blk_tgt = (uint32_t*)(base + o_btgt); p.blk_maxfast = (uint32_t*)(base + o_bmf);
+    p.blk_sizes = (unsigned long long*)(base + o_bsz); p.grp_sizes = (unsigned long long*)(base + o_gsz); p.blk_tgt = (uint32_t*)(base + o_btgt); p.blk_maxfast = (uint32_t*)(base + o_bmf);
     p.sw_counts = (SwCounts*)(base + o_swc); p.sw_plan = (SwPlan*)(base + o_swp);
     m.d_lane_mask = (uint8_t*)(base + m.o_mask); m.d_started_after = (uint8_t*)(base + m.o_started);
     m.d_add_idx = (uint64_t*)(base + m.o_aidx); m.d_add_val = (uint64_t*)(base + m.o_aval); m.n_add = (uint32_t)H.add_idx.size();
@@ -467,18 +467,45 @@
     c->n_timed++;
 }
 
-static int enqueue_kernels(bqc_ctx* c, BatchMem& m)
+static void launch_coverage(bqc_ctx* c, BatchMem& m, hipStream_t s)
+{
+    const DevBatch& d = m.d;
+    if (!d.n_cov_tiles) bqc_launch_or_bytes(c->d_started, m.d_started_after, c->opt.n_lanes, s);
+    else bqc_launch_cov(d, c->sl, c->d_state, c->d_carry, c->d_parity, m.d_lane_mask, c->d_started, m.d_started_after, c->opt.n_lanes, m.prep.cov_extra_cap, s);
+    bqc_launch_add_words(c->d_state, m.d_add_idx, m.d_add_val, m.n_add, s);
+}
+
+static int cov_join(bqc_ctx* c, bool& forked)
+{
+    if (!forked) return 0;
+    forked = false;
+    HIPCHK(c, hipEventRecord(c->ev_cov_join, c->cov_stream));
+    HIPCHK(c, hipStreamWaitEvent(c->stream, c->ev_cov_join, 0));
+    return 0;
+}
+
+static int enqueue_batch(bqc_ctx* c, BatchMem& m, bool& forked)
 {
     DevRefs refs{(const uint8_t* const*)c->d_ref_ptrs, c->d_ref_len, c->d_main, c->opt.n_refs, (const uint32_t* const*)c->d_refn_ptrs};
     uint32_t* err = &m.d_err->flags;
     const DevBatch& d = m.d;
-    if (d.n_reads == 0) { if (c->timing) { c->n_timed = 0; c->tnames.clear(); } return 0; }
+    const bool side = c->cov_side && (d.n_cov_tiles || m.n_add);
+    if (side && !c->ev_cov_join) {
+        if (!c->cov_stream) c->cov_stream = bqc_pool_stream(c->device, BQC_STREAM_RANK_COV);
+        if (!c->cov_stream) return bqc_fail(c, BQC_ERR_DEVICE, "hipStreamCreate failed");
+        if (!c->ev_cov_fork) HIPCHK(c, hipEventCreateWithFlags(&c->ev_cov_fork, hipEventDisableTiming));
+        HIPCHK(c, hipEventCreateWithFlags(&c->ev_cov_join, hipEventDisableTiming));
+    }
     if (c->timing) { c->n_timed = 0; c->tnames.clear(); (void)hipEventRecord(c->ev[0], c->stream); }
     m.prep.replay = m.processed ? 1u : 0u;
-    bqc_launch_prep(m.prep, refs, c->stream);
+    bqc_launch_prep(m.prep, refs, c->stream, side ? c->ev_cov_fork : nullptr);
     m.processed = true;
     tick(c, "k_prep");
-    if (!d.n_cov_tiles) bqc_launch_or_bytes(c->d_started, m.d_started_after, c->opt.n_lanes, c->stream);
+    if (side) {
+        HIPCHK(c, hipStreamWaitEvent(c->cov_stream, c->ev_cov_fork, 0));
+        forked = true;
+        launch_coverage(c, m, c->cov_stream);
+    } else if (!d.n_cov_tiles) bqc_launch_or_bytes(c->d_started, m.d_started_after, c->opt.n_lanes, c->stream);
     if (d.n_reads > m.n_slow) {
         const uint32_t grid = c->n_cu;
         if (!(bqc_short_parts() & 8u)) {
@@ -508,13 +535,29 @@
         tick(c, "k_long");
     }
     if (d.n_nm_extra) bqc_launch_nm_extra(d, c->sl, c->d_state, refs, err, c->stream);
-    if (d.n_cov_tiles) bqc_launch_cov(d, c->sl, c->d_state, c->d_carry, c->d_parity, m.d_lane_mask, c->d_started, m.d_started_after, c->opt.n_lanes, c->stream);
-    bqc_launch_add_words(c->d_state, m.d_add_idx, m.d_add_val, m.n_add, c->stream);
-    tick(c, "k_cov");
+    if (!side) {
+        if (d.n_cov_tiles) launch_coverage(c, m, c->stream);
+        else bqc_launch_add_words(c->d_state, m.d_add_idx, m.d_add_val, m.n_add, c->stream);
+        tick(c, "k_cov");
+    }
     if (c->sketch) { sketch_process(c->sketch, d, c->stream); tick(c, "k_sketch"); }
+    if (side) {
+        const int rc = cov_join(c, forked);
+        if (rc) return rc;
+        tick(c, "k_cov");
+    }
     bqc_launch_err_merge(c->d_err0, m.d_err, c->stream);
     HIPCHK(c, hipGetLastError());
     return 0;
+}
+
+static int enqueue_kernels(bqc_ctx* c, BatchMem& m)
+{
+    if (m.d.n_reads == 0) { if (c->timing) { c->n_timed = 0; c->tnames.clear(); } return 0; }
+    bool forked = false;
+    const int rc = enqueue_batch(c, m, forked);
+    if (forked) (void)cov_join(c, forked);
+    return rc;
 }
 
 int bqc_report_errors(bqc_ctx* c, const ErrRec& e)
@@ -1086,7 +1129,7 @@
         d.n_reads = n; d.lane = (const uint8_t*)(base + o_lane); d.cov = (const CovEntry*)(base + o_cov); d.cov_extra = (const CovExtra*)(base + o_covx);
         d.desc = (const BatchDesc*)(base + o_desc); d.cov_tiles = (const CovTile*)(base + o_tiles); d.n_cov_tiles = (uint32_t)H.tiles.size();
         if (!d.n_cov_tiles) bqc_launch_or_bytes(c->d_started, (const uint8_t*)(base + o_started), nl, c->stream);
-        else bqc_launch_cov(d, c->sl, c->d_state, c->d_carry, c->d_parity, (const uint8_t*)(base + o_mask), c->d_started, (const uint8_t*)(base + o_started), nl, c->stream);
+        else bqc_launch_cov(d, c->sl, c->d_state, c->d_carry, c->d_parity, (const uint8_t*)(base + o_mask), c->d_started, (const uint8_t*)(base + o_started), nl, pb.extra_cap, c->stream);
         bqc_launch_add_words(c->d_state, (const uint64_t*)(base + o_aidx), (const uint64_t*)(base + o_aval), (uint32_t)H.add_idx.size(), c->stream);
         HIPCHK(c, hipStreamSynchronize(c->stream));
         (void)hipFree(pb.dmem);
diff --git a/bamqc_amd/csrc/k_cov.hip b/bamqc_amd/csrc/k_cov.hip
--- a/bamqc_amd/csrc/k_cov.hip
+++ b/bamqc_amd/csrc/k_cov.hip
@@ -4,7 +4,7 @@
 __global__ __launch_bounds__(256) void k_cov(DevBatch b, StateLayout sl, uint64_t* __restrict__ state,
                                                 uint32_t* __restrict__ carry , uint32_t* parity ,
                                                 const uint8_t* __restrict__ lane_mask, uint8_t* __restrict__ started,
-                                                const uint8_t* __restrict__ started_after, uint32_t n_lanes)
+                                                const uint8_t* __restrict__ started_after, uint32_t n_lanes, uint32_t cov_extra_cap)
 {
     __shared__ __attribute__((aligned(16))) int32_t diff[4096 + 256];
     __shared__ uint32_t hist[BQC_COVSIZE + 1];
@@ -26,7 +26,7 @@
         if (i0 < t.list_end) e0 = load(t, i0);
         if (i1 < t.list_end) e1 = load(t, i1);
     }
-    const uint32_t n_extra = b.desc->n_cov_extra;
+    const uint32_t n_extra = min(b.desc->n_cov_extra, cov_extra_cap);
     for (uint32_t ti = blockIdx.x;; ti += gridDim.x) {
         const bool done = ti >= b.n_cov_tiles;
         if (done) t.lane = 0xFFFFFFFFu;
@@ -166,11 +166,11 @@
 extern "C" void bqc_launch_err_merge(ErrRec* dst, const ErrRec* src, hipStream_t s) { hipLaunchKernelGGL(k_err_merge, dim3(1), dim3(1), 0, s, dst, src); }
 
 extern "C" void bqc_launch_cov(const DevBatch& b, const StateLayout& sl, uint64_t* state, uint32_t* carry, uint32_t* parity, const uint8_t* lane_mask,
-                               uint8_t* started, const uint8_t* started_after, uint32_t n_lanes, hipStream_t s)
+                               uint8_t* started, const uint8_t* started_after, uint32_t n_lanes, uint32_t cov_extra_cap, hipStream_t s)
 {
     if (b.n_cov_tiles == 0) return;
     const uint32_t grid = b.n_cov_tiles < 2048u ? b.n_cov_tiles : 2048u;
-    hipLaunchKernelGGL(k_cov, dim3(grid), dim3(256), 0, s, b, sl, state, carry, parity, lane_mask, started, started_after, n_lanes);
+    hipLaunchKernelGGL(k_cov, dim3(grid), dim3(256), 0, s, b, sl, state, carry, parity, lane_mask, started, started_after, n_lanes, cov_extra_cap);
 }
 
 extern "C" void bqc_launch_cov_final(const StateLayout& sl, uint64_t* state, const uint32_t* carry, const uint32_t* parity,
diff --git a/bamqc_amd/csrc/k_prep.hip b/bamqc_amd/csrc/k_prep.hip
--- a/bamqc_amd/csrc/k_prep.hip
+++ b/bamqc_amd/csrc/k_prep.hip
@@ -1,4 +1,5 @@
 #include <algorithm>
+#include <vector>
 #include "kernels_common.h"
 #include "prep.h"
 
@@ -39,68 +40,67 @@
     const uint32_t prev = (uint32_t)__builtin_amdgcn_update_dpp(0, (int)inc, 0x138 , 0xF, 0xF, true);
     return max(base, prev);
 }
+__device__ __forceinline__ unsigned long long uniform64(unsigned long long v)
+{
+    return (unsigned long long)__builtin_amdgcn_readfirstlane((uint32_t)v) | (unsigned long long)__builtin_amdgcn_readfirstlane((uint32_t)(v >> 32)) << 32;
+}
 __device__ __forceinline__ void err_key(ErrRec* e, uint32_t read, uint32_t order)
 {
     atomicMin(&e->first_key, ((unsigned long long)read << 3) | order);
 }
 
-__global__ __launch_bounds__(PR_THREADS) void k_prep_sizes(PrepArgs a)
-{
-    __shared__ unsigned long long sh[3 * (PR_THREADS / 64)];
+#define PS_THREADS 1024
+#define PS_PER (PR_GROUP / (PS_THREADS / 64))
+__global__ __launch_bounds__(PS_THREADS) void k_prep_sizes(PrepArgs a)
+{
+    __shared__ unsigned long long sh[3 * PR_GROUP];
     if (blockIdx.x == 0 && threadIdx.x == 0) {
         a.err->first_key = BQC_ERRKEY_NONE; a.err->flags = 0; a.err->aux0 = a.err->aux1 = 0;
         a.desc->n_cov_extra = 0;
         if (a.pend_extra_n) *a.pend_extra_n = 0;
         if (a.replay) *a.cursor = *a.cursor_save; else *a.cursor_save = *a.cursor;
     }
-    for (uint32_t k = blockIdx.x * PR_THREADS + threadIdx.x; k < a.n_sw; k += gridDim.x * PR_THREADS) a.sw_counts[k] = SwCounts{0, 0, 0, 0};
-    const uint32_t b0 = blockIdx.x * PR_BLOCK;
-    unsigned long long s1 = 0, s2 = 0, s3 = 0;
-#pragma unroll
-    for (int j = 0; j < PR_PER_THREAD; ++j) {
-        const uint32_t i = b0 + j * PR_THREADS + threadIdx.x;
-        if (i < a.n) { const uint32_t L = a.l_seq[i]; s1 += (L + 1) / 2; s2 += L; s3 += a.n_cigar[i]; }
-    }
-#pragma unroll
-    for (int o = 32; o > 0; o >>= 1) { s1 += __shfl_xor(s1, o); s2 += __shfl_xor(s2, o); s3 += __shfl_xor(s3, o); }
-    if (lane_id() == 0) { const uint32_t w = threadIdx.x >> 6; sh[3 * w] = s1; sh[3 * w + 1] = s2; sh[3 * w + 2] = s3; }
-    block_sync();
-    if (threadIdx.x < 3) {
+    for (uint32_t k = blockIdx.x * PS_THREADS + threadIdx.x; k < a.n_sw; k += gridDim.x * PS_THREADS) a.sw_counts[k] = SwCounts{0, 0, 0, 0};
+    const uint32_t nblk = (a.n + PR_BLOCK - 1) / PR_BLOCK, bg0 = blockIdx.x * PR_GROUP, nb = min((uint32_t)PR_GROUP, nblk - bg0);
+    const uint32_t w = threadIdx.x >> 6, l = lane_id();
+    uint4 vl[PS_PER][4];
+    uint2 vc[PS_PER][4];
+#pragma unroll
+    for (int q = 0; q < PS_PER; ++q) {
+        const uint32_t bl = w + (PS_THREADS / 64) * q;
+        const unsigned long long i0 = (unsigned long long)(bg0 + bl) * PR_BLOCK;
+        const bool whole = bl < nb && i0 + PR_BLOCK <= a.n;
+#pragma unroll
+        for (int j = 0; j < 4; ++j) {
+            vl[q][j] = make_uint4(0, 0, 0, 0); vc[q][j] = make_uint2(0, 0);
+            if (whole) { const uint32_t i = (uint32_t)i0 + 256u * j + 4u * l; vl[q][j] = *(const uint4*)(a.l_seq + i); vc[q][j] = *(const uint2*)(a.n_cigar + i); }
+        }
+    }
+#pragma unroll
+    for (int q = 0; q < PS_PER; ++q) {
+        const uint32_t bl = w + (PS_THREADS / 64) * q;
+        const unsigned long long i0 = (unsigned long long)(bg0 + bl) * PR_BLOCK;
+        unsigned long long s1 = 0, s2 = 0, s3 = 0;
+#pragma unroll
+        for (int j = 0; j < 4; ++j) {
+            const uint4 v = vl[q][j];
+            s1 += (unsigned long long)((v.x + 1) / 2) + (v.y + 1) / 2 + (v.z + 1) / 2 + (v.w + 1) / 2;
+            s2 += (unsigned long long)v.x + v.y + v.z + v.w;
+            s3 += (vc[q][j].x & 0xFFFFu) + (vc[q][j].x >> 16) + (vc[q][j].y & 0xFFFFu) + (vc[q][j].y >> 16);
+        }
+        if (bl < nb && i0 + PR_BLOCK > a.n)
+            for (unsigned long long i = i0 + l; i < a.n; i += WAVE) { const uint32_t L = a.l_seq[i]; s1 += (L + 1) / 2; s2 += L; s3 += a.n_cigar[i]; }
+#pragma unroll
+        for (int o = 32; o > 0; o >>= 1) { s1 += __shfl_xor(s1, o); s2 += __shfl_xor(s2, o); s3 += __shfl_xor(s3, o); }
+        if (l == 0) { sh[3 * bl] = s1; sh[3 * bl + 1] = s2; sh[3 * bl + 2] = s3; }
+    }
+    block_sync();
+    if (threadIdx.x < 3 * PR_GROUP) {
+        const uint32_t bl = threadIdx.x / 3, k = threadIdx.x % 3;
         unsigned long long t = 0;
-        for (uint32_t w = 0; w < PR_THREADS / 64; ++w) t += sh[3 * w + threadIdx.x];
-        a.blk_sizes[3ull * blockIdx.x + threadIdx.x] = t;
-    }
-}
-
-__global__ __launch_bounds__(1024) void k_prep_scan(PrepArgs a)
-{
-    __shared__ unsigned long long sh[3 * 1024];
-    const uint32_t nblk = (a.n + PR_BLOCK - 1) / PR_BLOCK;
-    const uint32_t per = (nblk + blockDim.x - 1) / blockDim.x;
-    const uint32_t lo = min(nblk, threadIdx.x * per), hi = min(nblk, lo + per);
-    unsigned long long t[3] = {0, 0, 0};
-    for (uint32_t b = lo; b < hi; ++b)
-        for (int k = 0; k < 3; ++k) t[k] += a.blk_sizes[3ull * b + k];
-    for (int k = 0; k < 3; ++k) sh[3 * threadIdx.x + k] = t[k];
-    block_sync();
-    for (uint32_t d = 1; d < blockDim.x; d <<= 1) {
-        unsigned long long v[3] = {0, 0, 0};
-        if (threadIdx.x >= d) for (int k = 0; k < 3; ++k) v[k] = sh[3 * (threadIdx.x - d) + k];
-        block_sync();
-        for (int k = 0; k < 3; ++k) sh[3 * threadIdx.x + k] += v[k];
-        block_sync();
-    }
-    unsigned long long run[3];
-    for (int k = 0; k < 3; ++k) run[k] = sh[3 * threadIdx.x + k] - t[k];
-    for (uint32_t b = lo; b < hi; ++b) {
-        bool over = false;
-        for (int k = 0; k < 3; ++k) {
-            const unsigned long long s = a.blk_sizes[3ull * b + k];
-            a.blk_sizes[3ull * b + k] = run[k];
-            run[k] += s;
-            over |= run[k] > 0xFFFFFFFFull;
-        }
-        if (over) err_key(a.err, b * PR_BLOCK, 3);
+        for (uint32_t j = 0; j < bl; ++j) t += sh[3 * j + k];
+        if (bl < nb) a.blk_sizes[3ull * (bg0 + bl) + k] = t;
+        if (bl == PR_GROUP - 1) a.grp_sizes[3ull * blockIdx.x + k] = t + sh[3 * bl + k];
     }
 }
 
@@ -236,17 +236,46 @@
 {
     __shared__ uint32_t sh[2 * (PR_THREADS / 64)];
     __shared__ uint32_t red[8];
+    __shared__ unsigned long long gsum[3 * (PR_THREADS / 64) + 6];
     const uint32_t i0 = blockIdx.x * PR_BLOCK + 4u * threadIdx.x;
-    const unsigned long long gs = a.blk_sizes[3ull * blockIdx.x], gq = a.blk_sizes[3ull * blockIdx.x + 1], gc = a.blk_sizes[3ull * blockIdx.x + 2];
     if (threadIdx.x < 8) red[threadIdx.x] = threadIdx.x == 0 ? 0xFFFFFFFFu : 0u;
+    const uint32_t grp = blockIdx.x / PR_GROUP, nblk = gridDim.x;
+    unsigned long long grp_before[3] = {0, 0, 0}, grp_more[3] = {0, 0, 0}, in_grp = 0;
+    for (uint32_t g = threadIdx.x + 2 * PR_THREADS; g < grp; g += PR_THREADS) {
+        const unsigned long long* p = (const unsigned long long*)((const char*)a.grp_sizes + 24u * g);
+        for (int k = 0; k < 3; ++k) grp_before[k] += p[k];
+    }
+    if (threadIdx.x < grp) {
+        const unsigned long long* p = (const unsigned long long*)((const char*)a.grp_sizes + 24u * threadIdx.x);
+        for (int k = 0; k < 3; ++k) grp_before[k] += p[k];
+    }
+    if (threadIdx.x + PR_THREADS < grp) {
+        const unsigned long long* p = (const unsigned long long*)((const char*)a.grp_sizes + 24u * (threadIdx.x + PR_THREADS));
+        for (int k = 0; k < 3; ++k) grp_more[k] = p[k];
+    }
+    if (threadIdx.x < 6) {
+        const bool grp_last = (blockIdx.x + 1) % PR_GROUP == 0 || blockIdx.x + 1 == nblk;
+        const unsigned long long* incl_p = grp_last ? a.grp_sizes + 3ull * grp : a.blk_sizes + 3ull * (blockIdx.x + 1);
+        in_grp = threadIdx.x < 3 ? a.blk_sizes[3ull * blockIdx.x + threadIdx.x] : incl_p[threadIdx.x - 3];
+    }
+    auto sum_groups = [&] {
+        for (int k = 0; k < 3; ++k) grp_before[k] += grp_more[k];
+#pragma unroll
+        for (int o = 32; o > 0; o >>= 1)
+            for (int k = 0; k < 3; ++k) grp_before[k] += __shfl_xor(grp_before[k], o);
+        if (lane_id() == 0) for (int k = 0; k < 3; ++k) gsum[3 * (threadIdx.x >> 6) + k] = grp_before[k];
+        if (threadIdx.x < 6) gsum[3 * (PR_THREADS / 64) + threadIdx.x] = in_grp;
+    };
     ReadIn in[4];
     const uint32_t nlive = i0 >= a.n ? 0u : min(4u, a.n - i0);
-    if (nlive == 4u) {
+    if ((unsigned long long)(blockIdx.x + 1) * PR_BLOCK <= a.n) {
         const uint4 vl = *(const uint4*)(a.l_seq + i0);
         const uint2 vc = *(const uint2*)(a.n_cigar + i0), vf = *(const uint2*)(a.flag_in + i0);
         const uint32_t vlane = *(const uint32_t*)(a.lane + i0), vmq = *(const uint32_t*)(a.mapq + i0);
         const int4 vr = *(const int4*)(a.rid + i0), vp = *(const int4*)(a.pos + i0), va = *(const int4*)(a.as_ + i0);
         const uint4 c01 = *(const uint4*)(a.cov_in + i0), c23 = *(const uint4*)(a.cov_in + i0 + 2);
+        asm volatile("" : "+v"(grp_before[0]), "+v"(grp_before[1]), "+v"(grp_before[2]));
+        sum_groups();
         const uint32_t Ls[4] = {vl.x, vl.y, vl.z, vl.w}, ncs[4] = {vc.x & 0xFFFFu, vc.x >> 16, vc.y & 0xFFFFu, vc.y >> 16};
         const uint32_t fs[4] = {vf.x & 0xFFFFu, vf.x >> 16, vf.y & 0xFFFFu, vf.y >> 16};
         const int32_t rs[4] = {vr.x, vr.y, vr.z, vr.w}, ps[4] = {vp.x, vp.y, vp.z, vp.w}, as[4] = {va.x, va.y, va.z, va.w};
@@ -254,6 +283,7 @@
 #pragma unroll
         for (int j = 0; j < 4; ++j) in[j] = ReadIn{Ls[j], ncs[j], fs[j], (vlane >> (8 * j)) & 0xFFu, (vmq >> (8 * j)) & 0xFFu, rs[j], ps[j], as[j], cs[j]};
     } else {
+        sum_groups();
 #pragma unroll
         for (int j = 0; j < 4; ++j) {
             in[j] = ReadIn{0, 0, 0x900u, 0, 0, -1, 0, 0, CovEntry{BQC_COV_NONE, 0}};
@@ -264,7 +294,16 @@
 #pragma unroll
     for (int j = 0; j < 4; ++j) { ls[j] = ts; lq[j] = tq; lc[j] = tc; ts += (in[j].L + 1) / 2; tq += in[j].L; tc += in[j].nc; }
     uint32_t tot;
-    const unsigned long long bs = gs + block_scan_excl(ts, sh, &tot), bq = gq + block_scan_excl(tq, sh, &tot), bc = gc + block_scan_excl(tc, sh, &tot);
+    const uint32_t xs = block_scan_excl(ts, sh, &tot), xq = block_scan_excl(tq, sh, &tot), xc = block_scan_excl(tc, sh, &tot);
+    unsigned long long excl[3], incl[3];
+    for (int k = 0; k < 3; ++k) {
+        unsigned long long t = 0;
+        for (uint32_t w = 0; w < PR_THREADS / 64; ++w) t += gsum[3 * w + k];
+        grp_before[k] = uniform64(t); excl[k] = uniform64(gsum[3 * (PR_THREADS / 64) + k]); incl[k] = uniform64(gsum[3 * (PR_THREADS / 64) + 3 + k]);
+    }
+    unsigned long long base[3];
+    if (prep_block_bases(grp_before, excl, incl, base) && threadIdx.x == 0) err_key(a.err, blockIdx.x * PR_BLOCK, 3);
+    const unsigned long long bs = base[0] + xs, bq = base[1] + xq, bc = base[2] + xc;
     ReadOut out[4];
     CigarView cv[4];
     bool ref_loaded[4];
@@ -570,16 +609,41 @@
     for (uint32_t k = threadIdx.x; k < n_ent; k += PR_THREADS) a.perm[pl.group_base + k] = ent[k];
 }
 
-extern "C" void bqc_launch_prep(const PrepArgs& a, const DevRefs& refs, hipStream_t s)
+extern "C" void bqc_launch_prep(const PrepArgs& a, const DevRefs& refs, hipStream_t s, hipEvent_t after_reads)
 {
     if (a.n == 0) return;
     const uint32_t nblk = (a.n + PR_BLOCK - 1) / PR_BLOCK;
-    hipLaunchKernelGGL(k_prep_sizes, dim3(nblk), dim3(PR_THREADS), 0, s, a);
-    hipLaunchKernelGGL(k_prep_scan, dim3(1), dim3(1024), 0, s, a);
+    hipLaunchKernelGGL(k_prep_sizes, dim3((nblk + PR_GROUP - 1) / PR_GROUP), dim3(PS_THREADS), 0, s, a);
     hipLaunchKernelGGL(k_prep_reads, dim3(nblk), dim3(PR_THREADS), 0, s, a, refs);
+    if (after_reads) (void)hipEventRecord(after_reads, s);
     if (a.order) hipLaunchKernelGGL(k_build_count, dim3(a.n_sw), dim3(PR_THREADS), 0, s, a);
     hipLaunchKernelGGL(k_build_plan, dim3(1), dim3(1024), 0, s, a);
     hipLaunchKernelGGL(k_build_scatter, dim3(a.n_sw), dim3(PR_THREADS), 0, s, a);
+}
+
+extern "C" uint32_t bqc_prep_group(void) { return PR_GROUP; }
+extern "C" uint32_t bqc_prep_bases(const uint64_t* blk_totals, uint32_t n_blocks, uint64_t* bases)
+{
+    const uint32_t n_groups = (n_blocks + PR_GROUP - 1) / PR_GROUP;
+    std::vector<unsigned long long> blk(3ull * n_blocks), grp(3ull * n_groups);
+    for (uint32_t g = 0; g < n_groups; ++g)
+        for (int k = 0; k < 3; ++k) {
+            unsigned long long t = 0;
+            for (uint32_t b = g * PR_GROUP; b < std::min(n_blocks, (g + 1) * PR_GROUP); ++b) { blk[3ull * b + k] = t; t += blk_totals[3ull * b + k]; }
+            grp[3ull * g + k] = t;
+        }
+    uint32_t first_bad = 0xFFFFFFFFu;
+    for (uint32_t b = 0; b < n_blocks; ++b) {
+        const uint32_t g = b / PR_GROUP;
+        const bool grp_last = (b + 1) % PR_GROUP == 0 || b + 1 == n_blocks;
+        const unsigned long long* incl = grp_last ? &grp[3ull * g] : &blk[3ull * (b + 1)];
+        unsigned long long before[3] = {0, 0, 0}, base[3];
+        for (uint32_t g2 = 0; g2 < g; ++g2)
+            for (int k = 0; k < 3; ++k) before[k] += grp[3ull * g2 + k];
+        if (prep_block_bases(before, &blk[3ull * b], incl, base)) first_bad = std::min(first_bad, b);
+        for (int k = 0; k < 3; ++k) bases[3ull * b + k] = base[k];
+    }
+    return first_bad;
 }
 
 __device__ __forceinline__ uint32_t pend_interval(uint32_t pos, uint32_t c0, uint32_t len)
diff --git a/bamqc_amd/csrc/prep.h b/bamqc_amd/csrc/prep.h
--- a/bamqc_amd/csrc/prep.h
+++ b/bamqc_amd/csrc/prep.h
@@ -1,6 +1,23 @@
 #pragma once
+#include <hip/hip_runtime.h>
 #include <stdint.h>
 #include "device_types.h"
+
+#ifndef PR_GROUP
+#define PR_GROUP 32
+#endif
+static_assert(PR_GROUP >= 16 && (PR_GROUP & (PR_GROUP - 1)) == 0, "PR_GROUP: a power of two, 16 or more");
+
+__host__ __device__ inline bool prep_block_bases(const unsigned long long before[3], const unsigned long long excl[3], const unsigned long long incl[3],
+                                                 unsigned long long base[3])
+{
+    bool over = false;
+    for (int k = 0; k < 3; ++k) {
+        base[k] = before[k] + excl[k];
+        over |= before[k] + incl[k] > 0xFFFFFFFFull;
+    }
+    return over;
+}
 
 struct Stretch {
     uint32_t lane, sw_begin, sw_end, pad;
@@ -52,12 +69,15 @@
     int32_t* cursor;
     int32_t* cursor_save;
     unsigned long long* blk_sizes;
+    unsigned long long* grp_sizes;
     uint32_t* blk_tgt;
     uint32_t* blk_maxfast;
     SwCounts* sw_counts;
     SwPlan* sw_plan;
 };
 
-extern "C" void bqc_launch_prep(const PrepArgs& a, const DevRefs& refs, hipStream_t s);
+extern "C" void bqc_launch_prep(const PrepArgs& a, const DevRefs& refs, hipStream_t s, hipEvent_t after_reads);
+extern "C" uint32_t bqc_prep_bases(const uint64_t* blk_totals, uint32_t n_blocks, uint64_t* bases);
+extern "C" uint32_t bqc_prep_group(void);
 extern "C" void bqc_launch_pend_cov(uint32_t n, const CovEntry* cov_in, const PendRun* pend, const PendExtra* extra, const uint32_t* extra_n, uint32_t extra_cap,
                                     const uint8_t* lane, CovEntry* cov_out, CovExtra* cov_extra, BatchDesc* desc, hipStream_t s);
```

Result: faster. 4.557 billion (median of 6 runs) (+2.9%).
